# yondonfu/ai-rtc-agent

Measured on NVIDIA H100. Metric: frames/sec at 512x512 SD-Turbo img2img (1-step, stream-batch 1), higher is better.
Workload: dtype f16

## Files before the change

ai-rtc-agent_b200/csrc/capi.cu:

```cuda
#include "../../include/b200sd.h"

#include "attention.cuh"
#include "codec.cuh"
#include "elementwise.cuh"
#include "igemm.cuh"
#include "tconv.cuh"

using namespace b2;

extern "C" {

const char* b2sd_last_error(void) { return b2_last_error(); }
int b2sd_version(void) { return 1; }

static ActView to_view(const b2sd_act_view& v) {
    ActView a;
    a.ptr = reinterpret_cast<const __half*>(v.ptr);
    a.N = v.n; a.H = v.h; a.W = v.w; a.C = v.c; a.ld = v.ld;
    return a;
}

static void to_igemm_desc(const b2sd_igemm_desc* d, IgemmDesc& g) {
    g.nseg = d->nseg;
    for (int s = 0; s < d->nseg && s < IG_MAX_SRC; ++s) {
        g.src[s] = to_view(d->src[s]);
        g.ntap[s] = d->ntap[s];
    }
    g.w = reinterpret_cast<const __half*>(d->w);
    g.w_rows = d->w_rows;
    g.w_ld = d->w_ld;
    g.stride = d->stride;
    g.Nb = d->nb; g.Ho = d->ho; g.Wo = d->wo;
    g.BN = d->bn;
    g.swap = d->swap;
    g.pair = (d->flags & B2SD_IG_PAIR) ? 1 : 0;
    g.splits = d->splits;
    g.partial = nullptr;
    g.dbg_ts = reinterpret_cast<unsigned long long*>(d->partial);
    g.epi.out = reinterpret_cast<__half*>(d->out);
    g.epi.ldc = d->ldc;
    g.epi.colbias = d->colbias;
    g.epi.colbias_bstride = d->colbias_bstride;
    g.epi.res = reinterpret_cast<const __half*>(d->res);
    g.epi.ldr = d->ldr;
    g.epi.acc_scale = d->acc_scale;
    g.epi.res_scale = d->res_scale;
    g.epi.flags = d->flags & (IG_RELU | IG_GEGLU | IG_SILU | IG_PAD0);
    g.epi.n_valid = d->n_valid;
    g.epi.rowstat_out = static_cast<unsigned long long*>(d->rowstat_out);
    g.epi.rowstat_in = static_cast<const unsigned long long*>(d->rowstat_in);
    g.epi.colsum = d->colsum;
    g.epi.ln_inv_c = d->ln_c > 0 ? 1.f / (float)d->ln_c : 0.f;
    g.epi.ln_eps = d->ln_eps;
    g.epi.out2 = reinterpret_cast<__half*>(d->out2);
    g.epi.ld2 = d->ld2;
    g.epi.col2 = d->col2;
}

int b2sd_op_igemm(const b2sd_igemm_desc* d, void* stream) {
    if (!d) {
        b2_set_error("b2sd_op_igemm: null desc");
        return -1;
    }
    IgemmDesc g{};
    to_igemm_desc(d, g);
    if (d->flags & B2SD_IG_TCONV) {
        if (d->flags & B2SD_IG_PAD0) {
            b2_set_error("b2sd_op_igemm: the halo-tile kernel has no tap-origin-0 variant");
            return -1;
        }
        TconvPlan tp;
        if (tconv_plan(g, &tp)) return -1;
        return tconv_launch(tp, reinterpret_cast<cudaStream_t>(stream));
    }
    IgemmPlan plan;
    if (igemm_plan(g, &plan)) return -1;
    return igemm_launch(plan, reinterpret_cast<cudaStream_t>(stream));
}

int b2sd_igemm_plan_dry(const b2sd_igemm_desc* d, int autotile, int allow_swap, b2sd_igemm_plan_info* out) {
    if (!d || !out) {
        b2_set_error("b2sd_igemm_plan_dry: null argument");
        return -1;
    }
    IgemmDesc g{};
    to_igemm_desc(d, g);
    g.dbg_ts = nullptr;
    IgemmPlan plan;
    if (autotile == 2) {
        g.max_splits = 4; g.pair_auto = 1; g.pair_splits = 1;
    }
    igemm_set_dry_run(true);
    const int rc = autotile ? igemm_autotile(g, allow_swap != 0, &plan) : igemm_plan(g, &plan);
    igemm_set_dry_run(false);
    if (rc) return -1;
    out->mode = plan.mode;
    out->swap = plan.p.swap;
    out->bn = plan.p.BN;
    out->splits = plan.splits;
    out->grid_x = (int)plan.grid.x; out->grid_y = (int)plan.grid.y; out->grid_z = (int)plan.grid.z;
    out->num_stages = plan.p.num_stages;
    out->acc_bufs = plan.p.acc_bufs;
    out->total_kb = plan.p.total_kb;
    out->kb_per_split = plan.p.kb_per_split;
    out->tmem_cols = (int)plan.p.tmem_cols;
    out->m_tiles = plan.p.tiles_w * plan.p.tiles_h * plan.p.tiles_n;
    out->smem_bytes = (int64_t)plan.smem;
    out->rows_total = plan.rows_total;
    return 0;
}

int b2sd_groupnorm_plan_dry(int ca, int cb, int groups, int hw, int* cluster, int* threads, int* pixels_per_cta) {
    GroupNormArgs a{};
    a.ca = ca; a.cb = cb; a.lda = ca; a.ldb = cb; a.ldy = ca + cb; a.groups = groups; a.hw = hw; a.nb = 1;
    if (groups <= 0 || hw <= 0 || ca <= 0 || !cluster) {
        b2_set_error("b2sd_groupnorm_plan_dry: bad arguments");
        return -1;
    }
    *cluster = groupnorm_plan(a, threads, pixels_per_cta);
    return 0;
}

uint64_t b2sd_igemm_partial_floats(int splits, int64_t rows_total, int n_valid) {
    return igemm_partial_floats(splits, rows_total, n_valid);
}

int b2sd_op_nv12_to_rgb(const void* y, int y_pitch, const void* uv, int uv_pitch, void* rgb_nhwc, int h, int w, int flags, void* stream) {
    return nv12_to_rgb_u8_launch(static_cast<const uint8_t*>(y), y_pitch, static_cast<const uint8_t*>(uv), uv_pitch,
                                 static_cast<uint8_t*>(rgb_nhwc), h, w, flags, reinterpret_cast<cudaStream_t>(stream));
}
int b2sd_op_rgb_to_nv12(const void* rgb_nchw, void* y, int y_pitch, void* uv, int uv_pitch, int h, int w, int flags, void* stream) {
    return rgb_u8_to_nv12_launch(static_cast<const uint8_t*>(rgb_nchw), static_cast<uint8_t*>(y), y_pitch, static_cast<uint8_t*>(uv),
                                 uv_pitch, h, w, flags, reinterpret_cast<cudaStream_t>(stream));
}
int b2sd_codec_probe(void) { return codec_probe(); }

int b2sd_op_attention(const b2sd_attn_desc* d, void* stream) {
    AttnDesc a{};
    a.q = reinterpret_cast<const __half*>(d->q); a.ldq = d->ldq;
    a.k = reinterpret_cast<const __half*>(d->k); a.ldk = d->ldk; a.k_bstride = d->k_bstride; a.k_rows = d->k_rows;
    a.vt = reinterpret_cast<const __half*>(d->vt); a.ldvt = d->ldvt; a.vt_bstride = d->vt_bstride; a.vt_cols = d->vt_cols;
    a.out = reinterpret_cast<__half*>(d->out); a.ldo = d->ldo;
    a.nb = d->nb; a.heads = d->heads; a.sq = d->sq; a.skv = d->skv; a.d_real = d->d_real; a.dp = d->dp;
    AttnPlan plan;
    if (attn_plan(a, &plan)) return -1;
    return attn_launch(plan, reinterpret_cast<cudaStream_t>(stream));
}

int b2sd_op_groupnorm(const void* xa, int ca, int lda, const void* xb, int cb, int ldb, const float* gamma,
                      const float* beta, void* y, int ldy, int nb, int hw, int groups, float eps, int silu,
                      void* stream) {
    GroupNormArgs a{};
    a.xa = reinterpret_cast<const __half*>(xa); a.ca = ca; a.lda = lda;
    a.xb = reinterpret_cast<const __half*>(xb); a.cb = cb; a.ldb = ldb;
    a.gamma = gamma; a.beta = beta;
    a.y = reinterpret_cast<__half*>(y); a.ldy = ldy;
    a.nb = nb; a.hw = hw; a.groups = groups; a.eps = eps; a.silu = silu;
    static float* scratch = nullptr;
    static size_t scratch_floats = 0;
    const size_t need = groupnorm_partial_floats(nb, groups);
    if (need > scratch_floats) {
        if (scratch) cudaFree(scratch);
        if (cudaMalloc(&scratch, need * sizeof(float)) != cudaSuccess) {
            b2_set_error("b2sd_op_groupnorm: cudaMalloc failed");
            return -1;
        }
        scratch_floats = need;
    }
    a.partial = scratch;
// ... 83 lines not shown
```

ai-rtc-agent_b200/csrc/elementwise.cu:

```cuda
#include "elementwise.cuh"

#include <stdio.h>

#include "igemm.cuh"
#include "launch.cuh"
#include "ptx.cuh"

namespace b2 {

#define B2_PDL_ENTRY()            \
    do {                          \
        pdl_launch_dependents();  \
        pdl_wait();               \
    } while (0)

#define B2_LAUNCHED(name, expr)                                            \
    do {                                                                   \
        cudaError_t e__ = (expr);                                          \
        if (e__ != cudaSuccess) {                                          \
            b2_set_error("%s launch: %s", name, cudaGetErrorString(e__));  \
            return -1;                                                     \
        }                                                                  \
    } while (0)

// ... 846 lines not shown
    const long warp = ((long)blockIdx.x * blockDim.x + threadIdx.x) >> 5;
    const int lane = threadIdx.x & 31;
    if (warp >= (long)nb * n) return;
    const int b = (int)(warp / n), j = (int)(warp % n);
    float acc = 0.f;
    for (int i = lane; i < k; i += 32) {
        float v = in[(long)b * in_ld + i];
        if (silu_in) v = v / (1.0f + expf(-v));
        acc += v * __half2float(w[(long)j * k + i]);
    }
#pragma unroll
    for (int o = 16; o > 0; o >>= 1) acc += __shfl_xor_sync(0xffffffffu, acc, o);
    if (lane == 0) out[(long)b * out_ld + j] = acc + (bias ? bias[j] : 0.f);
}

int small_linear_launch(const float* in, int in_ld, const __half* w, const float* bias, float* out, int out_ld,
                        int nb, int n, int k, int silu_in, cudaStream_t s) {
    const long warps = (long)nb * n;
    small_linear_kernel<<<(unsigned)((warps * 32 + 255) / 256), 256, 0, s>>>(in, in_ld, w, bias, out, out_ld, nb, n, k, silu_in);
    B2_CHECK_LAUNCH("small_linear");
    return 0;
}

__global__ void timestep_embedding_kernel(const float* __restrict__ t, float* __restrict__ out, int nb, int dim) {
    const int half_dim = dim / 2;
    const int i = blockIdx.x * blockDim.x + threadIdx.x;
    if (i >= nb * half_dim) return;
    const int b = i / half_dim, j = i % half_dim;
    const float freq = expf(-logf(10000.0f) * (float)j / (float)half_dim);
    const float arg = t[b] * freq;
    out[(long)b * dim + j] = cosf(arg);
    out[(long)b * dim + half_dim + j] = sinf(arg);
}

int timestep_embedding_launch(const float* t, float* out, int nb, int dim, cudaStream_t s) {
    const int total = nb * (dim / 2);
    timestep_embedding_kernel<<<(total + 127) / 128, 128, 0, s>>>(t, out, nb, dim);
    B2_CHECK_LAUNCH("timestep_embedding");
    return 0;
}

__global__ void cast_f32_f16_kernel(const float* __restrict__ x, __half* __restrict__ y, long n) {
    for (long i = (long)blockIdx.x * blockDim.x + threadIdx.x; i < n; i += (long)gridDim.x * blockDim.x)
        y[i] = __float2half_rn(x[i]);
}
__global__ void cast_f16_f32_kernel(const __half* __restrict__ x, float* __restrict__ y, long n) {
    for (long i = (long)blockIdx.x * blockDim.x + threadIdx.x; i < n; i += (long)gridDim.x * blockDim.x)
        y[i] = __half2float(x[i]);
}
static unsigned grid_for(long n) {
    long b = (n + 255) / 256;
    if (b > IG_SMS * 32) b = IG_SMS * 32;
    if (b < 1) b = 1;
    return (unsigned)b;
}
int cast_f32_to_f16_launch(const float* x, __half* y, long n, cudaStream_t s) {
    cast_f32_f16_kernel<<<grid_for(n), 256, 0, s>>>(x, y, n);
    B2_CHECK_LAUNCH("cast_f32_f16");
    return 0;
}
int cast_f16_to_f32_launch(const __half* x, float* y, long n, cudaStream_t s) {
    cast_f16_f32_kernel<<<grid_for(n), 256, 0, s>>>(x, y, n);
    B2_CHECK_LAUNCH("cast_f16_f32");
    return 0;
}

__global__ void pack_conv_weight_kernel(const __half* __restrict__ w, __half* __restrict__ dst, int dst_ld, int koff,
                                        int o, int i, int taps, int c0, int cn) {
    const long total = (long)o * taps * cn;
    for (long e = (long)blockIdx.x * blockDim.x + threadIdx.x; e < total; e += (long)gridDim.x * blockDim.x) {
        const int c = (int)(e % cn);
        const int tap = (int)((e / cn) % taps);
        const int oo = (int)(e / ((long)cn * taps));
        dst[(long)oo * dst_ld + koff + tap * cn + c] = c0 + c < i ? w[((long)oo * i + (c0 + c)) * taps + tap] : __float2half(0.f);
    }
}
int pack_conv_weight_launch(const __half* w_oihw, __half* dst, int dst_ld, int koff, int o, int i, int taps, int c0,
                            int cn, cudaStream_t s) {
    pack_conv_weight_kernel<<<grid_for((long)o * taps * cn), 256, 0, s>>>(w_oihw, dst, dst_ld, koff, o, i, taps, c0, cn);
    B2_CHECK_LAUNCH("pack_conv_weight");
    return 0;
}

__global__ void gather_rows_kernel(const __half* __restrict__ src, int src_ld, const int* __restrict__ perm,
                                   __half* __restrict__ dst, int dst_ld, int rows, int cols) {
    const long total = (long)rows * cols;
    for (long e = (long)blockIdx.x * blockDim.x + threadIdx.x; e < total; e += (long)gridDim.x * blockDim.x) {
        const int c = (int)(e % cols);
        const int r = (int)(e / cols);
        const int sr = perm ? perm[r] : r;
        dst[(long)r * dst_ld + c] = sr >= 0 ? src[(long)sr * src_ld + c] : __float2half(0.f);
    }
}
int gather_rows_launch(const __half* src, int src_ld, const int* perm, __half* dst, int dst_ld, int rows, int cols,
                       cudaStream_t s) {
    gather_rows_kernel<<<grid_for((long)rows * cols), 256, 0, s>>>(src, src_ld, perm, dst, dst_ld, rows, cols);
    B2_CHECK_LAUNCH("gather_rows");
    return 0;
}

__global__ void scale_cols_kernel(__half* w, long rows, int k, const float* __restrict__ g) {
    const long r = (long)blockIdx.x * (blockDim.x >> 5) + (threadIdx.x >> 5);
    if (r >= rows) return;
    for (int c = threadIdx.x & 31; c < k; c += 32) w[r * k + c] = __float2half_rn(__half2float(w[r * k + c]) * g[c]);
}
__global__ void row_sum_kernel(const __half* __restrict__ w, long rows, int k, float* out) {
    const long r = (long)blockIdx.x * (blockDim.x >> 5) + (threadIdx.x >> 5);
    if (r >= rows) return;
    float a = 0.f;
    for (int c = threadIdx.x & 31; c < k; c += 32) a += __half2float(w[r * k + c]);
    for (int o = 16; o; o >>= 1) a += __shfl_xor_sync(0xffffffffu, a, o);
    if ((threadIdx.x & 31) == 0) out[r] = a;
}
__global__ void row_dot_kernel(const __half* __restrict__ w, long rows, int k, const float* __restrict__ v,
                               const float* __restrict__ bias, float* out) {
    const long r = (long)blockIdx.x * (blockDim.x >> 5) + (threadIdx.x >> 5);
    if (r >= rows) return;
    float a = 0.f;
    for (int c = threadIdx.x & 31; c < k; c += 32) a += __half2float(w[r * k + c]) * v[c];
    for (int o = 16; o; o >>= 1) a += __shfl_xor_sync(0xffffffffu, a, o);
    if ((threadIdx.x & 31) == 0) out[r] = a + (bias ? bias[r] : 0.f);
}
int scale_cols_launch(__half* w, long rows, int k, const float* gamma, cudaStream_t s) {
    scale_cols_kernel<<<(unsigned)((rows + 7) / 8), 256, 0, s>>>(w, rows, k, gamma);
    B2_CHECK_LAUNCH("scale_cols");
    return 0;
}
int row_sum_launch(const __half* w, long rows, int k, float* out, cudaStream_t s) {
    row_sum_kernel<<<(unsigned)((rows + 7) / 8), 256, 0, s>>>(w, rows, k, out);
    B2_CHECK_LAUNCH("row_sum");
    return 0;
}
int row_dot_launch(const __half* w, long rows, int k, const float* v, const float* bias, float* out, cudaStream_t s) {
    row_dot_kernel<<<(unsigned)((rows + 7) / 8), 256, 0, s>>>(w, rows, k, v, bias, out);
    B2_CHECK_LAUNCH("row_dot");
    return 0;
}

__global__ void maxpool2x2_kernel(const __half2* __restrict__ x, __half2* __restrict__ y, int nb, int h, int w, int c2) {
    B2_PDL_ENTRY();
    const int ho = h / 2, wo = w / 2;
    const long total = (long)nb * ho * wo * c2;
    for (long e = (long)blockIdx.x * blockDim.x + threadIdx.x; e < total; e += (long)gridDim.x * blockDim.x) {
        const int cc = (int)(e % c2);
        long p = e / c2;
        const int xo = (int)(p % wo);
        p /= wo;
        const int yo = (int)(p % ho);
        const int n = (int)(p / ho);
        const __half2* src = x + (((long)n * h + 2 * yo) * w + 2 * xo) * c2 + cc;
        const long row = (long)w * c2;
        y[e] = __hmax2(__hmax2(src[0], src[c2]), __hmax2(src[row], src[row + c2]));
    }
}

int maxpool2x2_launch(const __half* x, __half* y, int nb, int h, int w, int c, cudaStream_t s) {
    if ((c & 1) || (h & 1) || (w & 1)) {
        b2_set_error("maxpool2x2: c, h and w must be even (c=%d, %dx%d)", c, h, w);
        return -1;
    }
    const long total = (long)nb * (h / 2) * (w / 2) * (c / 2);
    long blocks = (total + 255) / 256;
    if (blocks > IG_SMS * 16) blocks = IG_SMS * 16;
    B2_LAUNCHED("maxpool2x2", launch_k(maxpool2x2_kernel, dim3((unsigned)blocks), dim3(256), 0, s, 1,
                                       reinterpret_cast<const __half2*>(x), reinterpret_cast<__half2*>(y), nb, h, w, c / 2));
    return 0;
// ... 75 lines not shown
```

ai-rtc-agent_b200/csrc/elementwise.cuh:

```cuda
#pragma once
#include <cuda_fp16.h>
#include <cuda_runtime.h>
#include <stdint.h>

namespace b2 {

struct GroupNormArgs {
    const __half* xa; int ca; int lda;
    const __half* xb; int cb; int ldb;
    const float* gamma; const float* beta;
    __half* y; int ldy;
    int nb, hw, groups;
    float eps;
    int silu;
    float* partial;
    int* counters;
};
int groupnorm_launch(const GroupNormArgs& a, cudaStream_t s);
size_t groupnorm_partial_floats(int nb, int groups);
int groupnorm_plan(const GroupNormArgs& a, int* threads, int* pixels_per_cta);
int groupnorm_last_launch_count();
enum : int { GN_PATH_CLUSTER = 0, GN_PATH_FUSED = 1, GN_PATH_STATS_APPLY = 2 };
int groupnorm_last_path();

int layernorm_launch(const __half* x, int ldx, const float* gamma, const float* beta, __half* y, int ldy,
                     long rows, int c, float eps, cudaStream_t s);

int upsample2x_launch(const __half* x, __half* y, int nb, int h, int w, int c, cudaStream_t s);

enum : int { SC_IN_U8 = 1, SC_IN_TANH3 = 2, SC_OUT_RELU = 4, SC_IN_F32_NCHW = 8, SC_IN_F16_NCHW = 16, SC_OUT_SILU = 32,
             SC_IN_OFFSET = 64 };
struct SmallConvArgs {
    const void* x;
    const float* wt;
    const float* bias;
    __half* y; int ldy;
    int nb, h, w_, cin, cout;
    int in_h, in_w;
    int flags;
    const __half* res;
    int ldr;
    long res_bstride;
    const float* in_off;
};
int smallconv_launch(const SmallConvArgs& a, cudaStream_t s);
int smallconv_prep_launch(const __half* w_oihw, float* wt, int cout, int cin, cudaStream_t s);

int maxpool2x2_launch(const __half* x, __half* y, int nb, int h, int w, int c, cudaStream_t s);
int hed_project_launch(const __half* x, int ldx, int c, long npix, const float* w, const float* bias, float* out, cudaStream_t s);
struct HedFuseArgs {
    const float* maps[5];
    int hs[5], ws[5];
    int levels;
    int h, w;
    uint8_t* out;
    __half* edge_f16;
};
int hed_fuse_launch(const HedFuseArgs& a, cudaStream_t s);

int lcm_step_launch(__half* x, const __half* eps, const __half* noise, const float* coef, __half* out_latent,
                    int T, int hw, int do_add_noise, cudaStream_t s);

int post_u8_launch(const __half* y_nhwc, int ldy, uint8_t* out_nchw, int nb, int h, int w, cudaStream_t s);
int post_f16_launch(const __half* y_nhwc, int ldy, __half* out_nchw, int nb, int h, int w, cudaStream_t s);

int small_linear_launch(const float* in, int in_ld, const __half* w, const float* bias, float* out, int out_ld,
                        int nb, int n, int k, int silu_in, cudaStream_t s);
int timestep_embedding_launch(const float* t, float* out, int nb, int dim, cudaStream_t s);

int cast_f32_to_f16_launch(const float* x, __half* y, long n, cudaStream_t s);
int cast_f16_to_f32_launch(const __half* x, float* y, long n, cudaStream_t s);
int pack_conv_weight_launch(const __half* w_oihw, __half* dst, int dst_ld, int koff, int o, int i, int taps,
                            int c0, int cn, cudaStream_t s);
int gather_rows_launch(const __half* src, int src_ld, const int* perm, __half* dst, int dst_ld, int rows, int cols,
                       cudaStream_t s);

int scale_cols_launch(__half* w, long rows, int k, const float* gamma, cudaStream_t s);
int row_sum_launch(const __half* w, long rows, int k, float* out, cudaStream_t s);
int row_dot_launch(const __half* w, long rows, int k, const float* v, const float* bias, float* out, cudaStream_t s);

}
```

ai-rtc-agent_b200/csrc/engine.cu:

```cuda
#include <cuda_fp16.h>
#include <cuda_runtime.h>
#include <math.h>
#include <stddef.h>
#include <stdio.h>
#include <stdlib.h>
#include <string.h>

#include <atomic>
#include <chrono>
#include <functional>
#include <thread>
#include <map>
#include <memory>
#include <string>
#include <vector>

#include "../../include/b200sd.h"
#include "attention.cuh"
#include "elementwise.cuh"
#include "igemm.cuh"
#include "tconv.cuh"

using namespace b2;

// ... 29 lines not shown
        for (auto s : shape) v *= s;
        return v;
    }
};

class Arena {
  public:
    explicit Arena(size_t slab) : slab_(slab) {}
    ~Arena() { release(); }
    void* alloc(size_t bytes) {
        bytes = (bytes + 1023) & ~size_t(1023);
        if (cur_ < 0 || off_ + bytes > sizes_[cur_]) {
            int next = cur_ + 1;
            while (next < (int)slabs_.size() && sizes_[next] < bytes) ++next;
            if (next >= (int)slabs_.size()) {
                size_t sz = bytes > slab_ ? bytes : slab_;
                void* p = nullptr;
                if (cudaMalloc(&p, sz) != cudaSuccess) return nullptr;
                slabs_.push_back(p);
                sizes_.push_back(sz);
                next = (int)slabs_.size() - 1;
            }
            cur_ = next;
            off_ = 0;
        }
        void* r = static_cast<char*>(slabs_[cur_]) + off_;
        off_ += bytes;
        return r;
    }
    void reset() { cur_ = slabs_.empty() ? -1 : 0; off_ = 0; }
    void release() {
        for (void* p : slabs_) cudaFree(p);
        slabs_.clear();
        sizes_.clear();
        cur_ = -1;
        off_ = 0;
    }

  private:
    size_t slab_;
    std::vector<void*> slabs_;
    std::vector<size_t> sizes_;
    int cur_ = -1;
    size_t off_ = 0;
};

struct Op {
    std::function<int(cudaStream_t)> fn;
    std::string name;
    double flops = 0.0;
    template <class F>
    Op(F f, std::string n = "", double fl = 0.0) : fn(std::move(f)), name(std::move(n)), flops(fl) {}
    int operator()(cudaStream_t s) const { return fn(s); }
};

}

static int igemm_autotile_single(IgemmDesc d, bool allow_swap, IgemmPlan* plan_out);

int igemm_autotile(IgemmDesc d, bool allow_swap, IgemmPlan* plan_out) {
    TRY(igemm_autotile_single(d, allow_swap, plan_out));
    static const char* pair_env = getenv("B2_PAIR");
    static const char* ps_env = getenv("B2_PAIR_SPLITS");
    static const bool pair_single = getenv("B2_PAIR_SINGLE") != nullptr;
    const int pair_mode = pair_env ? atoi(pair_env) : d.pair_auto;
    const int pair_splits = ps_env ? atoi(ps_env) : (d.pair_splits > 0 ? d.pair_splits : 4);
    const IgemmPlan& pl = *plan_out;
    const int m_tiles = pl.p.tiles_w * pl.p.tiles_h * pl.p.tiles_n;
    if (pair_mode <= 0 || pl.p.swap || m_tiles < 2 || (pl.p.BN % 32) != 0 || (d.epi.flags & (IG_SILU | IG_PAD0))) return 0;
    if (pair_mode == 2 && pl.p.total_kb < 20) return 0;
    d.swap = 0; d.BN = pl.p.BN; d.splits = pl.splits > pair_splits ? pair_splits : pl.splits; d.partial = nullptr;
    d.pair = pair_single ? 0 : 1;
    IgemmPlan paired;
    if (igemm_plan(d, &paired)) return 0;
    *plan_out = paired;
    return 0;
}

static int igemm_autotile_single(IgemmDesc d, bool allow_swap, IgemmPlan* plan_out) {
    IgemmPlan& plan = *plan_out;
    const bool geglu = (d.epi.flags & IG_GEGLU) != 0;
    const bool silu = (d.epi.flags & IG_SILU) != 0;
    const bool pad0 = (d.epi.flags & IG_PAD0) != 0;
    const int n_gemm = geglu ? 2 * d.epi.n_valid : d.epi.n_valid;
    static const bool swap_on = getenv("B2_SWAP") != nullptr, swap_off = getenv("B2_NO_SWAP") != nullptr;
    static const bool tuned = getenv("B2_NO_TUNED_TILES") == nullptr;
    static const char* ms_env = getenv("B2_MAX_SPLITS");
    const int max_splits = ms_env ? atoi(ms_env) : (d.max_splits > 0 ? d.max_splits : 8);
    int total_kb = 0;
    for (int sidx = 0; sidx < d.nseg && sidx < IG_MAX_SRC; ++sidx) total_kb += d.ntap[sidx] * (d.src[sidx].C / IG_BK);
    const long rows_all = (long)d.Nb * d.Ho * d.Wo;
    const bool swap_here = allow_swap && !geglu && !pad0 && d.epi.n_valid >= 128 && (d.epi.n_valid & 7) == 0 &&
                           (swap_on || (!swap_off && tuned && rows_all <= 64 && total_kb >= 90));
    if (swap_here) {
        d.swap = 1;
        d.BN = rows_all >= 256 ? 256 : (rows_all >= 128 ? 128 : 64);
        d.splits = 1; d.partial = nullptr;
        TRY(igemm_plan(d, &plan));
        const long ctas = (long)plan.grid.x * plan.grid.y;
        int max_by_k = plan.p.total_kb / 4;
        if (max_by_k < 1) max_by_k = 1;
        if (max_by_k > 8) max_by_k = 8;
        int splits = 1;
        while (splits * 2 <= max_by_k && ctas * splits * 2 <= 192 && splits * 2 <= max_splits) splits *= 2;
        if (splits > 1) {
            d.splits = splits;
            TRY(igemm_plan(d, &plan));
        }
        return 0;
    }
    d.swap = 0;
    auto vt_ok = [&](int bn) { return !d.epi.out2 || d.epi.col2 % bn == 0; };
    if (tuned && !geglu && !silu && !pad0 && n_gemm % 160 == 0 && total_kb >= 40 && vt_ok(160)) {
        d.BN = 160; d.splits = 1; d.partial = nullptr;
        TRY(igemm_plan(d, &plan));
        const int m_tiles = plan.p.tiles_w * plan.p.tiles_h * plan.p.tiles_n;
        const long tiles = (long)m_tiles * (n_gemm / 160);
        int bn = 0, splits = 0;
        if (tiles < 132) {
            if (m_tiles >= 8) { bn = 160; splits = 4; }
            else if (m_tiles >= 2 && n_gemm % 256 == 0 && total_kb >= 180 && vt_ok(256)) { bn = 256; splits = 8; }
        }
        if (bn && splits > max_splits) bn = 0;
        if (bn) {
            d.BN = bn; d.splits = splits;
            TRY(igemm_plan(d, &plan));
            return 0;
        }
    }
    static const int cands[] = {256, 160, 128, 64, 32, 16};
    std::vector<int> valid;
    for (int bn : cands) {
        if (geglu && (bn % 32 != 0 || bn < 64)) continue;
        if (silu && (bn > 128 || bn % 16 || (bn & (bn - 1)))) continue;
        if (pad0 && bn != 64 && bn != 128 && bn != 256) continue;
        if (n_gemm % bn == 0 && vt_ok(bn)) valid.push_back(bn);
    }
    if (valid.empty()) {
        int bn = 16;
        while (bn < n_gemm && bn < 128) bn <<= 1;
        valid.push_back(bn);
    }
    for (int bn : valid) {
        if (bn < 64 && n_gemm >= 64) break;
        d.BN = bn; d.splits = 1; d.partial = nullptr;
        TRY(igemm_plan(d, &plan));
        if (plan.p.acc_bufs == 2 || (long)plan.grid.x * plan.grid.y >= b2_device_sms()) return 0;
    }
    int bn = valid.back();
    for (int v : valid) if (v >= 64) bn = v;
    d.BN = bn; d.splits = 1; d.partial = nullptr;
    TRY(igemm_plan(d, &plan));
    const long ctas = (long)plan.grid.x * plan.grid.y;
    int splits = ctas >= 96 ? 1 : (int)((IG_SMS + ctas - 1) / ctas);
    if (tuned && ctas >= 64 && total_kb <= 12) splits = 1;
    const int max_by_k = plan.p.total_kb / 4 > 0 ? plan.p.total_kb / 4 : 1;
    if (splits > max_by_k) splits = max_by_k;
    if (splits > 8) splits = 8;
    while (splits > max_splits && splits > 1) splits >>= 1;
    if (geglu) splits = 1;
    if (splits > 1) {
        d.splits = splits;
        TRY(igemm_plan(d, &plan));
    }
    return 0;
}

struct WeightStore {
    std::map<std::string, Raw> raw;
    Arena weights{256u << 20};
    Arena raw_only{256u << 20};
    bool raw_released = false;
    bool imported = false;
    std::map<std::string, __half*> packed;
    std::map<std::string, float*> fvec;
    std::map<std::string, size_t> packed_bytes, fvec_bytes;
};

struct b2sd_engine {
    b2sd_config cfg{};
    int lh = 0, lw = 0;
    std::shared_ptr<WeightStore> ws;
    std::map<std::string, Raw>& raw;
    Arena& weights;
    Arena& raw_only;
    bool& raw_released;
    bool& imported;
    std::map<std::string, __half*>& packed;
    std::map<std::string, float*>& fvec;
    std::map<std::string, size_t>& packed_bytes;
    std::map<std::string, size_t>& fvec_bytes;
    Arena state{16u << 20};
    Arena prog{512u << 20};
    explicit b2sd_engine(std::shared_ptr<WeightStore> s)
        : ws(std::move(s)), raw(ws->raw), weights(ws->weights), raw_only(ws->raw_only), raw_released(ws->raw_released),
          imported(ws->imported), packed(ws->packed), fvec(ws->fvec), packed_bytes(ws->packed_bytes), fvec_bytes(ws->fvec_bytes) {}

    Act x_in;
    __half* noise = nullptr;
    float* coef = nullptr;
    float* tsteps = nullptr;
    __half* ctx = nullptr;
    float* temb_sin = nullptr;
    float* temb_h = nullptr;
    float* temb = nullptr;
    float* cn_temb_h = nullptr;
    float* cn_temb = nullptr;
    float* gn_ws = nullptr;
    int* tile_counters = nullptr;
    float coef_host[4][64]{};

    unsigned long long* ln_stats = nullptr;
    size_t ln_stats_cap = 0, ln_stats_used = 0;
    std::vector<Op> prog_frame, prog_prompt, prog_time;
    std::map<std::string, Act> taps;
    SmallConvArgs head{};
    SmallConvArgs cn_head{};
    SmallConvArgs hed_head{};
    Act image;
// ... 17 lines not shown
            if (stage_graph[i]) { cudaGraphDestroy(stage_graph[i]); stage_graph[i] = nullptr; }
        }
    }

    ~b2sd_engine() { drop_graphs(); }

    const Raw* get(const std::string& key) {
        auto it = raw.find(key);
        if (it == raw.end()) {
            b2_set_error("missing weight '%s'", key.c_str());
            return nullptr;
        }
        return &it->second;
    }
    bool has(const std::string& key) const { return raw.count(key) != 0; }

    float* vec(const std::vector<std::string>& keys, const std::vector<int>* perm = nullptr, int pad_to = 0) {
        std::string ck = "v:";
        for (auto& k : keys) ck += k + "+";
        if (perm) ck += "perm";
        auto it = fvec.find(ck);
        if (it != fvec.end()) return it->second;
        std::vector<float> host;
        for (auto& k : keys) {
            const Raw* r = get(k);
            if (!r) return nullptr;
            if (host.empty()) host.assign(r->host.begin(), r->host.end());
            else
                for (size_t i = 0; i < host.size() && i < r->host.size(); ++i) host[i] += r->host[i];
        }
        if (perm) {
            std::vector<float> t(perm->size());
            for (size_t i = 0; i < perm->size(); ++i) t[i] = (*perm)[i] >= 0 ? host[(*perm)[i]] : 0.f;
            host.swap(t);
        }
        if ((int)host.size() < pad_to) host.resize(pad_to, 0.f);
        float* d = static_cast<float*>(weights.alloc(host.size() * sizeof(float)));
        if (!d) return nullptr;
        if (cudaMemcpy(d, host.data(), host.size() * sizeof(float), cudaMemcpyHostToDevice) != cudaSuccess) return nullptr;
        fvec[ck] = d;
        fvec_bytes[ck] = host.size() * sizeof(float);
        return d;
    }

    const float* small_w(const std::string& key, cudaStream_t s) {
        auto it = fvec.find("sw:" + key);
        if (it != fvec.end()) return it->second;
        const Raw* r = get(key);
        if (!r) return nullptr;
        if (!r->p) { b2_set_error("parameter '%s' was released after the first prepare and is not in the packed cache", key.c_str()); return nullptr; }
        const int cout = (int)r->shape[0], cin = (int)r->shape[1];
        float* d = static_cast<float*>(weights.alloc((size_t)cin * 9 * cout * sizeof(float)));
        if (!d || smallconv_prep_launch(r->p, d, cout, cin, s)) return nullptr;
        fvec["sw:" + key] = d;
        fvec_bytes["sw:" + key] = (size_t)cin * 9 * cout * sizeof(float);
        return d;
    }

    struct ConvSeg { std::string key; int c0, cn, taps; };
    __half* pack_conv(const std::string& name, const std::vector<ConvSeg>& segs, int rows, int* k_out,
                      cudaStream_t s) {
        int K = 0;
        for (auto& g : segs) K += g.taps * g.cn;
        *k_out = K;
        auto it = packed.find(name);
        if (it != packed.end()) return it->second;
        const int rows_pad = (rows + 15) / 16 * 16;
        __half* dst = static_cast<__half*>(weights.alloc((size_t)rows_pad * K * 2));
        if (!dst) return nullptr;
        cudaMemsetAsync(dst, 0, (size_t)rows_pad * K * 2, s);
        int koff = 0;
        for (auto& g : segs) {
            const Raw* r = get(g.key);
            if (!r) return nullptr;
            if (!r->p) { b2_set_error("parameter '%s' was released after the first prepare and is not in the packed cache", g.key.c_str()); return nullptr; }
            const int cin_total = (int)r->shape[1];
            if (pack_conv_weight_launch(r->p, dst, K, koff, rows, cin_total, g.taps, g.c0, g.cn, s)) return nullptr;
            koff += g.taps * g.cn;
        }
        packed[name] = dst;
        packed_bytes[name] = (size_t)rows_pad * K * 2;
        return dst;
    }
    __half* pack_rows(const std::string& name, const std::vector<std::pair<std::string, std::vector<int>>>& parts,
                      int K, cudaStream_t s) {
        auto it = packed.find(name);
        if (it != packed.end()) return it->second;
        size_t rows = 0;
        for (auto& p : parts) rows += p.second.size();
        const size_t rows_pad = (rows + 15) / 16 * 16;
        __half* dst = static_cast<__half*>(weights.alloc(rows_pad * K * 2));
        if (!dst) return nullptr;
        cudaMemsetAsync(dst, 0, rows_pad * K * 2, s);
        size_t r0 = 0;
        for (auto& p : parts) {
            const Raw* r = get(p.first);
            if (!r) return nullptr;
            if (!r->p) { b2_set_error("parameter '%s' was released after the first prepare and is not in the packed cache", p.first.c_str()); return nullptr; }
            int* dperm = static_cast<int*>(weights.alloc(p.second.size() * sizeof(int)));
            if (!dperm) return nullptr;
            cudaMemcpyAsync(dperm, p.second.data(), p.second.size() * sizeof(int), cudaMemcpyHostToDevice, s);
            cudaStreamSynchronize(s);
            if (gather_rows_launch(r->p, K, dperm, dst + r0 * K, K, (int)p.second.size(), K, s)) return nullptr;
            r0 += p.second.size();
        }
        packed[name] = dst;
        packed_bytes[name] = rows_pad * K * 2;
        return dst;
    }

    struct LnFold { __half* w = nullptr; const float* colsum = nullptr; const float* bias = nullptr; };
    int fold_ln(const std::string& name, const std::vector<std::pair<std::string, std::vector<int>>>& parts, int K,
                const std::string& ln_prefix, const float* bias_vec, LnFold* out, cudaStream_t s) {
        size_t rows = 0;
        for (auto& p : parts) rows += p.second.size();
        const size_t rows_pad = (rows + 15) / 16 * 16;
        const bool done = packed.count(name) && fvec.count(name + ":cs") && fvec.count(name + ":b");
        __half* w = pack_rows(name, parts, K, s);
        if (!w) return -1;
        if (!done) {
            const float* gamma = vec({ln_prefix + ".weight"});
            const float* beta = vec({ln_prefix + ".bias"});
            float* cs = static_cast<float*>(weights.alloc(rows_pad * sizeof(float)));
            float* bb = static_cast<float*>(weights.alloc(rows_pad * sizeof(float)));
            if (!gamma || !beta || !cs || !bb) return -1;
            cudaMemsetAsync(bb, 0, rows_pad * sizeof(float), s);
            TRY(row_dot_launch(w, (long)rows, K, beta, bias_vec, bb, s));
            TRY(scale_cols_launch(w, (long)rows_pad, K, gamma, s));
            TRY(row_sum_launch(w, (long)rows_pad, K, cs, s));
            fvec[name + ":cs"] = cs; fvec_bytes[name + ":cs"] = rows_pad * sizeof(float);
            fvec[name + ":b"] = bb; fvec_bytes[name + ":b"] = rows_pad * sizeof(float);
        }
        out->w = w;
        out->colsum = fvec[name + ":cs"];
        out->bias = fvec[name + ":b"];
        return 0;
    }
    unsigned long long* alloc_rowstat(long rows) {
        if (ln_stats_used + 2 * (size_t)rows > ln_stats_cap) {
            b2_set_error("LayerNorm statistics slab exhausted");
            return nullptr;
        }
        unsigned long long* p = ln_stats + ln_stats_used;
        ln_stats_used += 2 * (size_t)rows;
        return p;
    }

    Act new_act(int n, int h, int w, int c, int ld = 0) {
        Act a;
        a.n = n; a.h = h; a.w = w; a.c = c; a.ld = ld ? ld : c;
        a.p = static_cast<__half*>(prog.alloc((size_t)a.elems() * 2));
        return a;
    }
    static ActView view(const Act& a) { return ActView{a.p, a.n, a.h, a.w, a.c, a.ld}; }
    static ActView tokens(const Act& a) { return ActView{a.p, 1, 1, a.n * a.h * a.w, a.c, a.ld}; }

    void push_igemm(std::vector<Op>& dst, const IgemmPlan& plan, const std::string& label, double flops) {
        if (&dst == &prog_frame) launches += 1;
        dst.push_back(Op([plan](cudaStream_t s) { return igemm_launch(plan, s); }, label, flops));
    }

    int add_igemm(std::vector<Op>& dst, IgemmDesc d) {
        const bool geglu = (d.epi.flags & IG_GEGLU) != 0;
        const int n_gemm = geglu ? 2 * d.epi.n_valid : d.epi.n_valid;
        const bool extras = d.epi.rowstat_out || d.epi.colsum || d.epi.out2;
        if (concurrency > 1 && d.max_splits == 0) d.max_splits = 4;
        if (concurrency >= 4 && d.pair_auto == 0) { d.pair_auto = 1; d.pair_splits = 1; }
        IgemmPlan plan;
        TRY(igemm_autotile(d, allow_swap && !extras, &plan));
        if (d.epi.out2 && d.epi.col2 % plan.p.BN != 0) {
            b2_set_error("fused q/k/v projection: N tile %d does not divide the V offset %d", plan.p.BN, d.epi.col2);
            return -1;
        }
        char label[256];
        snprintf(label, sizeof(label), "igemm %s rows=%ld n=%d kb=%d bn=%d splits=%d grid=%u,%u,%u %s", cur.c_str(),
                 plan.rows_total, d.epi.n_valid, plan.p.total_kb, plan.p.BN, plan.splits, plan.grid.x, plan.grid.y,
                 plan.grid.z, plan.p.swap ? "swapped" : (plan.pair ? "pairs" : "taps"));
        push_igemm(dst, plan, label, 2.0 * (double)plan.rows_total * n_gemm * plan.p.total_kb * IG_BK);
        return 0;
    }

    int add_groupnorm(const Act& xa, const Act* xb, const std::string& prefix, const Act& y, float eps, int silu) {
        GroupNormArgs a{};
        a.xa = xa.p; a.ca = xa.c; a.lda = xa.ld;
        if (xb) { a.xb = xb->p; a.cb = xb->c; a.ldb = xb->ld; }
        a.gamma = vec({prefix + ".weight"});
        a.beta = vec({prefix + ".bias"});
        if (!a.gamma || !a.beta) return -1;
        a.y = y.p; a.ldy = y.ld;
        a.nb = xa.n; a.hw = xa.h * xa.w; a.groups = cfg.norm_groups; a.eps = eps; a.silu = silu;
        a.partial = gn_ws;
        a.counters = tile_counters;
        launches += 1;
        prog_frame.push_back(Op([a](cudaStream_t s) { return groupnorm_launch(a, s); }, "groupnorm " + prefix));
        return 0;
    }

    int add_layernorm(const Act& x, const std::string& prefix, const Act& y) {
        const float* g = vec({prefix + ".weight"});
        const float* b = vec({prefix + ".bias"});
        if (!g || !b) return -1;
        const long rows = (long)x.n * x.h * x.w;
        const __half* xp = x.p; __half* yp = y.p;
        const int ldx = x.ld, ldy = y.ld, c = x.c;
        ++launches;
        prog_frame.push_back(Op([=](cudaStream_t s) { return layernorm_launch(xp, ldx, g, b, yp, ldy, rows, c, 1e-5f, s); }, "layernorm " + prefix));
        return 0;
    }

    int add_conv(std::vector<Op>& dst, const Act& x, const std::string& wkey, const std::string& bkey, int taps,
                 int stride, const Act& y, int flags, const Act* res, cudaStream_t s, float acc_scale = 1.f,
                 float res_scale = 1.f) {
        const Raw* w = get(wkey);
        if (!w) return -1;
        cur = wkey;
        const int cout = (int)w->shape[0];
        int K = 0;
        __half* wp = pack_conv(wkey, {{wkey, 0, x.c, taps}}, cout, &K, s);
        if (!wp) return -1;
        IgemmDesc d{};
        d.nseg = 1; d.src[0] = view(x); d.ntap[0] = taps;
        d.w = wp; d.w_rows = (cout + 15) / 16 * 16; d.w_ld = K;
        d.stride = stride;
        d.Nb = y.n; d.Ho = y.h; d.Wo = y.w;
        d.epi.out = y.p; d.epi.ldc = y.ld;
        if (!bkey.empty()) {
            d.epi.colbias = vec({bkey}, nullptr, 16);
            if (!d.epi.colbias) return -1;
        }
        d.epi.colbias_bstride = 0;
        if (res) { d.epi.res = res->p; d.epi.ldr = res->ld; }
        d.epi.acc_scale = acc_scale; d.epi.res_scale = res_scale;
        d.epi.flags = flags;
        d.epi.n_valid = cout;
        static const bool no_tconv = getenv("B2_NO_TCONV") != nullptr;
        static const char* tc_min = getenv("B2_TCONV_MIN_TILES");
        const long tiles = (long)y.n * ((y.h + TC_TH - 1) / TC_TH) * ((y.w + TC_TW - 1) / TC_TW);
        if (!no_tconv && stride == 1 && tconv_eligible(d) && tiles >= (tc_min ? atoi(tc_min) : 2 * IG_SMS)) {
            TconvPlan tp;
            TRY(tconv_plan(d, &tp));
            char label[256];
            snprintf(label, sizeof(label), "tconv %s rows=%ld tiles=%d grid=%u nbuf=%d", wkey.c_str(), tp.rows_total, tp.p.num_tiles,
                     tp.grid.x, tp.p.nbuf);
            if (&dst == &prog_frame) launches += 1;
            dst.push_back(Op([tp](cudaStream_t st) { return tconv_launch(tp, st); }, label, 2.0 * (double)tp.rows_total * cout * K));
            return 0;
        }
        return add_igemm(dst, d);
    }

    struct LinExtra {
        unsigned long long* rowstat_out = nullptr;
        const unsigned long long* rowstat_in = nullptr;
        const float* colsum = nullptr;
        int ln_c = 0;
        __half* out2 = nullptr;
        int ld2 = 0, col2 = 0;
    };
    int add_linear(std::vector<Op>& dst, const ActView& x, const __half* w, int n, int k, const float* bias,
                   __half* out, int ldc, const __half* res, int ldr, int flags = 0, int n_valid = -1,
                   const LinExtra* ex = nullptr) {
        IgemmDesc d{};
        if (ex) {
            d.epi.rowstat_out = ex->rowstat_out;
            d.epi.rowstat_in = ex->rowstat_in;
            d.epi.colsum = ex->colsum;
            d.epi.ln_inv_c = ex->ln_c ? 1.f / (float)ex->ln_c : 0.f;
            d.epi.ln_eps = 1e-5f;
            d.epi.out2 = ex->out2; d.epi.ld2 = ex->ld2; d.epi.col2 = ex->col2;
        }
        d.nseg = 1; d.src[0] = x; d.ntap[0] = 1;
        d.w = w; d.w_rows = n; d.w_ld = k;
        d.stride = 1;
        d.Nb = 1; d.Ho = 1; d.Wo = x.W;
        d.epi.out = out; d.epi.ldc = ldc;
        d.epi.colbias = bias; d.epi.colbias_bstride = 0;
        d.epi.res = res; d.epi.ldr = ldr;
        d.epi.acc_scale = 1.f; d.epi.res_scale = 1.f;
        d.epi.flags = flags;
        d.epi.n_valid = n_valid >= 0 ? n_valid : n;
        return add_igemm(dst, d);
    }

    int build_resnet(const std::string& p, const Act& xa, const Act* xb, int cout, const float* emb, Act* out, cudaStream_t s,
                     float eps = 1e-5f);
    int build_vae_attention(const std::string& p, const Act& x, Act* out, cudaStream_t s);
    int build_kl_encoder(Act* out, std::string* latent_conv, cudaStream_t s);
    int build_kl_decoder(const Act& x0, cudaStream_t s);
    std::vector<float> host_copy(const std::string& key);
    int derive(const std::string& name, const std::vector<int64_t>& shape, const std::vector<float>& v);
    const float* const_vec(const std::string& name, const std::vector<float>& v);
    int build_cond_embedding(Act* out, cudaStream_t s);
    int build_hed(const uint8_t** control, cudaStream_t s);
    int build_controlnet(const Act& cond, std::vector<Act>& skips, Act* mid, cudaStream_t s);
    int build_transformer(const std::string& p, const Act& x, int heads, Act* out, cudaStream_t s);
    int build_taesd_block(const std::string& p, const Act& x, Act* out, cudaStream_t s);
    int build_program(cudaStream_t s);
    int run_range(std::vector<Op>& ops, size_t a, size_t b, cudaStream_t s) {
        for (size_t i = a; i < b && i < ops.size(); ++i) TRY(ops[i](s));
        return 0;
    }
    int run(std::vector<Op>& ops, cudaStream_t s) {
        static const bool dbg = getenv("B200SD_DEBUG_SYNC") != nullptr;
        static const char* skip = getenv("B200SD_SKIP");
        static const char* skip_name = getenv("B200SD_SKIP_NAME");
        int idx = 0;
        for (auto& op : ops) {
            if (skip) {
                const std::string kind = op.name.substr(0, op.name.find(' '));
                if (!kind.empty() && std::string(skip).find(kind) != std::string::npos) { ++idx; continue; }
            }
            if (skip_name && op.name.find(skip_name) != std::string::npos) { ++idx; continue; }
            TRY(op(s));
            if (dbg) {
                cudaError_t e = cudaStreamSynchronize(s);
                if (e != cudaSuccess) {
                    b2_set_error("op %d '%s' failed: %s", idx, op.name.c_str(), cudaGetErrorString(e));
                    fprintf(stderr, "b2sd: op %d '%s' failed: %s\n", idx, op.name.c_str(), cudaGetErrorString(e));
                    return -1;
                }
            }
            ++idx;
        }
        return 0;
    }
};

int b2sd_engine::build_resnet(const std::string& p, const Act& xa, const Act* xb, int cout, const float* emb, Act* out,
                              cudaStream_t s, float eps) {
    cur = p;
    allow_swap = true;
// ... 596 lines not shown
            }
            bf[o] = (float)bo;
        }
        TRY(derive(*latent_conv + ".weight", {4, ci, 3, 3}, wf));
        TRY(derive(*latent_conv + ".bias", {4}, bf));
    }
    return 0;
}

int b2sd_engine::build_kl_decoder(const Act& x0, cudaStream_t s) {
    const std::string P = "vae.decoder.";
    allow_swap = false;
    cur = P + "conv_in";
    const float sf = cfg.vae_scaling_factor > 0.f ? cfg.vae_scaling_factor : 0.18215f;
    const std::string wkey = P + "conv_in+post_quant_conv.weight";
    if (!has(wkey)) {
        const Raw* wc = get(P + "conv_in.weight");
        const Raw* wq = get("vae.post_quant_conv.weight");
        if (!wc || !wq) return -1;
        const int co = (int)wc->shape[0];
        if (wc->shape[1] != 4 || wq->numel() != 16) {
            b2_set_error("vae: decoder conv_in takes %ld channels and post_quant_conv has %ld weights (4 and 4x4 expected)",
                         (long)wc->shape[1], wq->numel());
            return -1;
        }
        std::vector<float> w = host_copy(P + "conv_in.weight"), q = host_copy("vae.post_quant_conv.weight");
        if (w.empty() || q.empty()) return -1;
        std::vector<float> wf((size_t)co * 4 * 9, 0.f);
        for (int o = 0; o < co; ++o)
            for (int j = 0; j < 4; ++j)
                for (int t = 0; t < 9; ++t) {
                    double acc = 0.0;
                    for (int i = 0; i < 4; ++i) acc += (double)w[((size_t)o * 4 + i) * 9 + t] * q[i * 4 + j];
                    wf[((size_t)o * 4 + j) * 9 + t] = (float)(acc / sf);
                }
        TRY(derive(wkey, {co, 4, 3, 3}, wf));
    }
    const Raw* rw = get(wkey);
    const Raw* pqb = get("vae.post_quant_conv.bias");
    if (!rw || !pqb || pqb->host.size() != 4) {
        if (rw && pqb) b2_set_error("vae: post_quant_conv.bias must have 4 elements");
        return -1;
    }
    const int cm = (int)rw->shape[0];
    Act bmap = new_act(1, lh, lw, cm), cst = new_act(1, lh, lw, 4), h = new_act(1, lh, lw, cm);
    if (!bmap.p || !cst.p || !h.p) return -1;
    {
        std::vector<__half> c((size_t)lh * lw * 4);
        for (size_t i = 0; i < c.size(); ++i) c[i] = __float2half_rn(pqb->host[i % 4]);
        CUDA_OK(cudaMemcpyAsync(cst.p, c.data(), c.size() * 2, cudaMemcpyHostToDevice, s));
        SmallConvArgs m{};
        m.x = cst.p; m.wt = small_w(P + "conv_in.weight", s); m.bias = vec({P + "conv_in.bias"});
        if (!m.wt || !m.bias) return -1;
        m.y = bmap.p; m.ldy = cm; m.nb = 1; m.h = lh; m.w_ = lw; m.cin = 4; m.cout = cm; m.in_h = lh; m.in_w = lw;
        TRY(smallconv_launch(m, s));
        CUDA_OK(cudaStreamSynchronize(s));
    }
    {
        SmallConvArgs a{};
        a.x = x0.p; a.wt = small_w(wkey, s); a.bias = nullptr;
        if (!a.wt) return -1;
        a.y = h.p; a.ldy = h.ld; a.nb = 1; a.h = lh; a.w_ = lw; a.cin = 4; a.cout = cm; a.in_h = lh; a.in_w = lw;
        a.res = bmap.p; a.ldr = bmap.ld; a.res_bstride = 0;
        ++launches;
        prog_frame.push_back(Op([a](cudaStream_t st) { return smallconv_launch(a, st); }, "smallconv vae.decoder.conv_in"));
    }
    {
        Act o;
        TRY(build_resnet(P + "mid_block.resnets.0.", h, nullptr, h.c, nullptr, &o, s, 1e-6f)); h = o;
        TRY(build_vae_attention(P + "mid_block.attentions.0.", h, &o, s)); h = o;
        TRY(build_resnet(P + "mid_block.resnets.1.", h, nullptr, h.c, nullptr, &o, s, 1e-6f)); h = o;
        taps["vae.dec.mid"] = h;
    }
    for (int i = 0; i < 4; ++i) {
        const std::string bp = P + "up_blocks." + std::to_string(i);
        for (int j = 0; j < 3; ++j) {
            const Raw* w1 = get(bp + ".resnets." + std::to_string(j) + ".conv1.weight");
            if (!w1) return -1;
            Act o;
            TRY(build_resnet(bp + ".resnets." + std::to_string(j) + ".", h, nullptr, (int)w1->shape[0], nullptr, &o, s, 1e-6f));
            h = o;
        }
        if (i < 3) {
            Act up = new_act(1, h.h * 2, h.w * 2, h.c);
            const Act hin = h;
            ++launches;
            prog_frame.push_back(Op([hin, up](cudaStream_t st) { return upsample2x_launch(hin.p, up.p, hin.n, hin.h, hin.w, hin.c, st); }, "upsample2x"));
            Act o = new_act(1, up.h, up.w, h.c);
            TRY(add_conv(prog_frame, up, bp + ".upsamplers.0.conv.weight", bp + ".upsamplers.0.conv.bias", 9, 1, o, 0, nullptr, s));
            h = o;
        }
        taps["vae.dec.up." + std::to_string(i)] = h;
    }
    Act nout = new_act(1, h.h, h.w, h.c);
    TRY(add_groupnorm(h, nullptr, P + "conv_norm_out", nout, 1e-6f, 1));
    const std::string bkey = P + "conv_out.bias+1";
    if (!has(bkey)) {
        const Raw* b = get(P + "conv_out.bias");
        if (!b) return -1;
        std::vector<float> v(b->host);
        for (auto& x : v) x += 1.f;
        TRY(derive(bkey, b->shape, v));
    }
    image = new_act(1, cfg.height, cfg.width, 3, 8);
    return add_conv(prog_frame, nout, P + "conv_out.weight", bkey, 9, 1, image, 0, nullptr, s, 0.5f);
}

int b2sd_engine::build_program(cudaStream_t s) {
    prog.reset();
    prog_frame.clear(); prog_prompt.clear(); prog_time.clear();
    taps.clear();
    launches = 0;
    drop_graphs();
    const int B = cfg.batch, H = cfg.height, W = cfg.width;
    const int* ch = cfg.block_out_channels;
    const int nlev = 4;
    {
        long words = 0;
        for (int i = 0; i < nlev; ++i) {
            const long tokens_i = (long)B * (lh >> i) * (lw >> i);
            int blocks_i = (cfg.down_attn[i] ? cfg.layers_per_block + (cfg.layers_per_block + 1) : 0) + (i == nlev - 1 ? 1 : 0);
            if (cfg.controlnet) blocks_i += (cfg.down_attn[i] ? cfg.layers_per_block : 0) + (i == nlev - 1 ? 1 : 0);
            words += 3 * 2 * tokens_i * blocks_i;
        }
        ln_stats_cap = (size_t)words;
        ln_stats_used = 0;
        ln_stats = static_cast<unsigned long long*>(prog.alloc(ln_stats_cap * sizeof(unsigned long long)));
        if (!ln_stats) return -1;
    }

    allow_swap = false;
    const bool kl = cfg.vae == B2SD_VAE_KL;
    Act e;
    std::string latent_conv;
    int li = 1;
    if (kl) {
        TRY(build_kl_encoder(&e, &latent_conv, s));
    } else {
    e = new_act(1, H, W, 64);
    {
        head = SmallConvArgs{};
        head.wt = small_w("vae.encoder.layers.0.weight", s);
        if (!head.wt) return -1;
        head.bias = vec({"vae.encoder.layers.0.bias"});
        head.y = e.p; head.ldy = e.ld; head.nb = 1; head.h = H; head.w_ = W; head.cin = 3; head.cout = 64;
        head.flags = SC_IN_U8;
        if (!head.bias) return -1;
        ++launches;
    }
    const int enc_blocks[4] = {1, 3, 3, 3};
    for (int st = 0; st < 4; ++st) {
        if (st > 0) {
            Act dwn = new_act(1, e.h / 2, e.w / 2, 64);
            TRY(add_conv(prog_frame, e, "vae.encoder.layers." + std::to_string(li) + ".weight", "", 9, 2, dwn, 0, nullptr, s));
            e = dwn;
            ++li;
        }
        for (int k = 0; k < enc_blocks[st]; ++k) {
            Act o;
            TRY(build_taesd_block("vae.encoder.layers." + std::to_string(li), e, &o, s));
            e = o;
            ++li;
        }
    }
    latent_conv = "vae.encoder.layers." + std::to_string(li);
    }
    Act cond;
    if (cfg.controlnet) TRY(build_cond_embedding(&cond, s));
    {
        Act xt;
        xt.p = x_in.p; xt.n = 1; xt.h = lh; xt.w = lw; xt.c = 4; xt.ld = 4;
        Act nz = xt;
        nz.p = noise;
        const float zscale = kl ? (cfg.vae_scaling_factor > 0.f ? cfg.vae_scaling_factor : 0.18215f) : 1.f;
        idx_enc_end = prog_frame.size();
        TRY(add_conv(prog_frame, e, latent_conv + ".weight", latent_conv + ".bias", 9, 1, xt, 0, &nz, s, coef_host[0][0] * zscale,
                     coef_host[1][0]));
        taps["x_t"] = xt;
    }
    taps["unet_in"] = x_in;

    allow_swap = true;
    Act h = new_act(B, lh, lw, ch[0]);
    {
        SmallConvArgs a{};
        a.wt = small_w("conv_in.weight", s);
        if (!a.wt) return -1;
        a.x = x_in.p; a.bias = vec({"conv_in.bias"});
        a.y = h.p; a.ldy = h.ld; a.nb = B; a.h = lh; a.w_ = lw; a.cin = 4; a.cout = ch[0]; a.in_h = lh; a.in_w = lw;
        if (!a.bias) return -1;
        ++launches;
        prog_frame.push_back(Op([a](cudaStream_t st) { return smallconv_launch(a, st); }, "smallconv"));
    }
    taps["conv_in"] = h;
    std::vector<Act> skips{h};
    for (int i = 0; i < nlev; ++i) {
        for (int j = 0; j < cfg.layers_per_block; ++j) {
            Act o;
            const std::string bp = "down_blocks." + std::to_string(i);
            TRY(build_resnet(bp + ".resnets." + std::to_string(j) + ".", h, nullptr, ch[i], temb, &o, s));
            h = o;
            if (cfg.down_attn[i]) {
                TRY(build_transformer(bp + ".attentions." + std::to_string(j) + ".", h, cfg.heads[i], &o, s));
                h = o;
            }
            skips.push_back(h);
            taps["down." + std::to_string(i) + "." + std::to_string(j)] = h;
        }
        if (i != nlev - 1) {
            Act o = new_act(B, h.h / 2, h.w / 2, ch[i]);
            const std::string k = "down_blocks." + std::to_string(i) + ".downsamplers.0.conv.";
            TRY(add_conv(prog_frame, h, k + "weight", k + "bias", 9, 2, o, 0, nullptr, s));
            h = o;
            skips.push_back(h);
        }
    }
    {
        Act o;
        TRY(build_resnet("mid_block.resnets.0.", h, nullptr, ch[nlev - 1], temb, &o, s)); h = o;
        TRY(build_transformer("mid_block.attentions.0.", h, cfg.heads[nlev - 1], &o, s)); h = o;
        TRY(build_resnet("mid_block.resnets.1.", h, nullptr, ch[nlev - 1], temb, &o, s)); h = o;
        taps["mid"] = h;
    }
    if (cfg.controlnet) TRY(build_controlnet(cond, skips, &h, s));
    for (int i = 0; i < nlev; ++i) {
        const int co = ch[nlev - 1 - i];
        const int hd = cfg.heads[nlev - 1 - i];
        const bool attn = cfg.down_attn[nlev - 1 - i] != 0;
        for (int j = 0; j < cfg.layers_per_block + 1; ++j) {
            Act sk = skips.back();
            skips.pop_back();
            Act o;
            const std::string bp = "up_blocks." + std::to_string(i);
            TRY(build_resnet(bp + ".resnets." + std::to_string(j) + ".", h, &sk, co, temb, &o, s));
            h = o;
            if (attn) {
                TRY(build_transformer(bp + ".attentions." + std::to_string(j) + ".", h, hd, &o, s));
                h = o;
            }
            taps["up." + std::to_string(i) + "." + std::to_string(j)] = h;
        }
        if (i != nlev - 1) {
            Act up = new_act(B, h.h * 2, h.w * 2, co);
            const Act hin = h;
            ++launches;
            prog_frame.push_back(Op([hin, up](cudaStream_t st) { return upsample2x_launch(hin.p, up.p, hin.n, hin.h, hin.w, hin.c, st); }, "upsample2x"));
            Act o = new_act(B, up.h, up.w, co);
            const std::string k = "up_blocks." + std::to_string(i) + ".upsamplers.0.conv.";
            TRY(add_conv(prog_frame, up, k + "weight", k + "bias", 9, 1, o, 0, nullptr, s));
            h = o;
        }
    }
    Act nout = new_act(B, lh, lw, ch[0]);
    TRY(add_groupnorm(h, nullptr, "conv_norm_out", nout, 1e-5f, 1));
    Act eps = new_act(B, lh, lw, 4);
    TRY(add_conv(prog_frame, nout, "conv_out.weight", "conv_out.bias", 9, 1, eps, 0, nullptr, s));
    taps["eps"] = eps;
    Act x0 = new_act(1, lh, lw, 4);
    {
        __half* xp = x_in.p; const __half* ep = eps.p; const __half* np_ = noise; const float* cf = coef; __half* op = x0.p;
        const int T = B, hw = lh * lw, dan = cfg.do_add_noise;
        ++launches;
        prog_frame.push_back(Op([=](cudaStream_t st) { return lcm_step_launch(xp, ep, np_, cf, op, T, hw, dan, st); }, "lcm_step"));
        idx_unet_end = prog_frame.size();
    }
    taps["x0"] = x0;
    allow_swap = false;
    if (kl) {
        TRY(build_kl_decoder(x0, s));
    } else {
    Act dcur = new_act(1, lh, lw, 64);
    {
        SmallConvArgs a{};
        a.wt = small_w("vae.decoder.layers.0.weight", s);
        if (!a.wt) return -1;
        a.x = x0.p; a.bias = vec({"vae.decoder.layers.0.bias"});
        a.y = dcur.p; a.ldy = dcur.ld; a.nb = 1; a.h = lh; a.w_ = lw; a.cin = 4; a.cout = 64; a.in_h = lh; a.in_w = lw;
        a.flags = SC_IN_TANH3 | SC_OUT_RELU;
        if (!a.bias) return -1;
        ++launches;
        prog_frame.push_back(Op([a](cudaStream_t st) { return smallconv_launch(a, st); }, "smallconv"));
    }
    li = 2;
    const int dec_blocks[4] = {3, 3, 3, 1};
    for (int st = 0; st < 4; ++st) {
        for (int k = 0; k < dec_blocks[st]; ++k) {
            Act o;
            TRY(build_taesd_block("vae.decoder.layers." + std::to_string(li), dcur, &o, s));
            dcur = o;
            ++li;
        }
        if (st != 3) {
            Act up = new_act(1, dcur.h * 2, dcur.w * 2, 64);
            const Act hin = dcur;
            ++launches;
            prog_frame.push_back(Op([hin, up](cudaStream_t s2) { return upsample2x_launch(hin.p, up.p, hin.n, hin.h, hin.w, hin.c, s2); }, "upsample2x"));
            ++li;
            Act o = new_act(1, up.h, up.w, 64);
            TRY(add_conv(prog_frame, up, "vae.decoder.layers." + std::to_string(li) + ".weight", "", 9, 1, o, 0, nullptr, s));
            dcur = o;
            ++li;
        } else {
            image = new_act(1, H, W, 3, 8);
            const std::string k = "vae.decoder.layers." + std::to_string(li);
            TRY(add_conv(prog_frame, dcur, k + ".weight", k + ".bias", 9, 1, image, 0, nullptr, s));
        }
    }
    }
    taps["image"] = image;
    ++launches;
    if (ln_stats_used) {
        unsigned long long* sp = ln_stats;
        const size_t bytes = ln_stats_used * sizeof(unsigned long long);
        prog_frame.insert(prog_frame.begin() + idx_enc_end, Op([sp, bytes](cudaStream_t st) {
            if (cudaMemsetAsync(sp, 0, bytes, st) != cudaSuccess) { b2_set_error("memset of the LayerNorm statistics failed"); return -1; }
            return 0; }, "memset ln_stats"));
        idx_unet_end += 1;
    }
    CUDA_OK(cudaStreamSynchronize(s));
    built = true;
    return 0;
}

extern "C" {

static int create_engine(const b2sd_config* cfg, std::shared_ptr<WeightStore> store, b2sd_handle* out);

int b2sd_create(const b2sd_config* cfg, b2sd_handle* out) { return create_engine(cfg, std::make_shared<WeightStore>(), out); }

int b2sd_create_lane(b2sd_handle parent, const b2sd_config* cfg, b2sd_handle* out) {
    if (!parent) {
        b2_set_error("b2sd_create_lane: null parent");
        return -1;
    }
    b2sd_config c = cfg ? *cfg : parent->cfg;
    c.controlnet = parent->cfg.controlnet;
    c.control_processor = parent->cfg.control_processor;
    c.vae = parent->cfg.vae;
    c.vae_scaling_factor = parent->cfg.vae_scaling_factor;
    for (int i = 0; i < 4; ++i)
        if (c.block_out_channels[i] != parent->cfg.block_out_channels[i] || c.heads[i] != parent->cfg.heads[i] ||
            c.down_attn[i] != parent->cfg.down_attn[i]) {
            b2_set_error("b2sd_create_lane: the lane's architecture differs from its parent's");
            return -1;
        }
    if (create_engine(&c, parent->ws, out)) return -1;
    (*out)->concurrency = parent->concurrency > 1 ? parent->concurrency : 2;
    return 0;
}

static int create_engine(const b2sd_config* cfg, std::shared_ptr<WeightStore> store, b2sd_handle* out) {
    if (!cfg || !out) {
        b2_set_error("b2sd_create: null argument");
        return -1;
    }
    if (cfg->height % 64 || cfg->width % 64 || cfg->batch < 1 || cfg->batch > 16) {
        b2_set_error("b2sd_create: height/width must be multiples of 64, 1 <= batch <= 16 (got %dx%d, %d)",
                     cfg->height, cfg->width, cfg->batch);
        return -1;
    }
    for (int i = 0; i < 4; ++i) {
        if (cfg->block_out_channels[i] % 64 || cfg->heads[i] < 1 || cfg->block_out_channels[i] % cfg->heads[i]) {
            b2_set_error("b2sd_create: block_out_channels must be multiples of 64 and divisible by heads");
            return -1;
        }
    }
    if (cfg->cross_attention_dim % 64) {
        b2_set_error("b2sd_create: cross_attention_dim must be a multiple of 64");
        return -1;
    }
    if (cfg->controlnet != 0 && cfg->controlnet != 1) {
        b2_set_error("b2sd_create: controlnet must be 0 or 1 (got %d)", cfg->controlnet);
        return -1;
    }
    if (cfg->control_processor != B2SD_CONTROL_FRAME && (cfg->control_processor != B2SD_CONTROL_HED || !cfg->controlnet)) {
        b2_set_error("b2sd_create: control_processor must be 0 (the frame) or 1 (HED, with a ControlNet) (got %d)", cfg->control_processor);
        return -1;
    }
    if (cfg->vae != B2SD_VAE_TINY && cfg->vae != B2SD_VAE_KL) {
        b2_set_error("b2sd_create: vae must be 0 (TAESD) or 1 (AutoencoderKL) (got %d)", cfg->vae);
        return -1;
    }
// ... 125 lines not shown
        const Raw* w2 = h->get(p + "time_embedding.linear_2.weight");
        const float* b1 = h->vec({p + "time_embedding.linear_1.bias"});
        const float* b2v = h->vec({p + "time_embedding.linear_2.bias"});
        if (!w1 || !w2 || !b1 || !b2v) return -1;
        TRY(small_linear_launch(h->temb_sin, C0, w1->p, b1, hid, TD, B, TD, C0, 0, s));
        return small_linear_launch(hid, TD, w2->p, b2v, out, TD, B, TD, TD, 1, s);
    };
    TRY(embed("", h->temb_h, h->temb));
    if (h->cfg.controlnet) TRY(embed("controlnet.", h->cn_temb_h, h->cn_temb));
    return h->run(h->prog_time, s);
}

int b2sd_prepare(b2sd_handle h, const void* prompt_embeds, const float* timesteps, const float* coef,
                 const void* init_noise, void* stream) {
    if (!h || !prompt_embeds || !timesteps || !coef || !init_noise) {
        b2_set_error("b2sd_prepare: null argument");
        return -1;
    }
    cudaStream_t s = reinterpret_cast<cudaStream_t>(stream);
    const int B = h->cfg.batch, lh = h->lh, lw = h->lw;
    for (int k = 0; k < 4; ++k)
        for (int i = 0; i < B; ++i) h->coef_host[k][i] = coef[k * B + i];
    CUDA_OK(cudaMemcpyAsync(h->coef, coef, 4 * B * sizeof(float), cudaMemcpyHostToDevice, s));
    CUDA_OK(cudaMemcpyAsync(h->tsteps, timesteps, B * sizeof(float), cudaMemcpyHostToDevice, s));
    CUDA_OK(cudaMemcpyAsync(h->ctx, prompt_embeds, (size_t)h->cfg.ctx_tokens * h->cfg.cross_attention_dim * 2,
                            cudaMemcpyHostToDevice, s));
    {
        const __half* src = static_cast<const __half*>(init_noise);
        std::vector<__half> nhwc((size_t)B * lh * lw * 4);
        for (int b = 0; b < B; ++b)
            for (int c = 0; c < 4; ++c)
                for (int y = 0; y < lh; ++y)
                    for (int x = 0; x < lw; ++x)
                        nhwc[(((size_t)b * lh + y) * lw + x) * 4 + c] = src[(((size_t)b * 4 + c) * lh + y) * lw + x];
        CUDA_OK(cudaMemcpyAsync(h->noise, nhwc.data(), nhwc.size() * 2, cudaMemcpyHostToDevice, s));
        CUDA_OK(cudaStreamSynchronize(s));
    }
    CUDA_OK(cudaMemsetAsync(h->x_in.p, 0, (size_t)h->x_in.elems() * 2, s));
    TRY(h->build_program(s));
    TRY(h->run(h->prog_prompt, s));
    TRY(refresh_time(h, s));
    CUDA_OK(cudaStreamSynchronize(s));
    static const bool keep_raw = getenv("B2_KEEP_RAW") != nullptr;
    if (!keep_raw && !h->raw_released) {
        for (auto& kv : h->raw)
            if (kv.second.pack_only) kv.second.p = nullptr;
        h->raw_only.release();
        h->raw_released = true;
    }
    return 0;
}

extern "C++" {
namespace {
struct BlobWriter {
    FILE* f;
    bool ok = true;
    void put(const void* p, size_t n) { if (ok && n && fwrite(p, 1, n, f) != n) ok = false; }
    template <class T> void pod(const T& v) { put(&v, sizeof(T)); }
    void str(const std::string& v) { pod((uint32_t)v.size()); put(v.data(), v.size()); }
};
struct BlobReader {
    FILE* f;
    bool ok = true;
    void get(void* p, size_t n) { if (ok && n && fread(p, 1, n, f) != n) ok = false; }
    template <class T> T pod() { T v{}; get(&v, sizeof(T)); return v; }
    std::string str() { uint32_t n = pod<uint32_t>(); if (!ok || n > 4096) { ok = false; return ""; } std::string v(n, 0); get(&v[0], n); return v; }
};
}
}

int b2sd_export_packed(b2sd_handle h, const char* path) {
    if (!h || !h->built || !path) {
        b2_set_error("b2sd_export_packed: call b2sd_prepare first");
        return -1;
    }
    FILE* f = fopen(path, "wb");
    if (!f) {
        b2_set_error("b2sd_export_packed: cannot open %s", path);
        return -1;
    }
    BlobWriter w{f};
    w.put("B2SDPACK", 8);
    w.pod((uint32_t)3);
    b2sd_config cfg = h->cfg;
    cfg.batch = 0; cfg.height = 0; cfg.width = 0; cfg.use_cuda_graph = 0; cfg.do_add_noise = 0;
    w.pod(cfg);
    w.pod((uint32_t)(h->raw.size() + h->packed_bytes.size() + h->fvec_bytes.size()));
    std::vector<char> host;
    auto payload = [&](const void* dptr, size_t bytes) {
        w.pod((uint64_t)bytes);
        if (!bytes) return true;
        host.resize(bytes);
        if (cudaMemcpy(host.data(), dptr, bytes, cudaMemcpyDeviceToHost) != cudaSuccess) return false;
        w.put(host.data(), bytes);
        return true;
    };
    bool copy_ok = true;
    for (auto& kv : h->raw) {
        const Raw& r = kv.second;
        w.pod((uint8_t)0); w.str(kv.first);
        w.pod((uint32_t)r.shape.size());
        for (auto d : r.shape) w.pod((int64_t)d);
        copy_ok &= payload(r.p, (r.pack_only || !r.p) ? 0 : (size_t)r.numel() * 2);
    }
    for (auto& kv : h->packed_bytes) {
        w.pod((uint8_t)1); w.str(kv.first); w.pod((uint32_t)0);
        copy_ok &= payload(h->packed[kv.first], kv.second);
    }
    for (auto& kv : h->fvec_bytes) {
        w.pod((uint8_t)2); w.str(kv.first); w.pod((uint32_t)0);
        copy_ok &= payload(h->fvec[kv.first], kv.second);
    }
    const bool ok = w.ok && copy_ok && fclose(f) == 0;
    if (!ok) {
        b2_set_error("b2sd_export_packed: write to %s failed", path);
        remove(path);
        return -1;
    }
    return 0;
}

int b2sd_import_packed(b2sd_handle h, const char* path) {
    if (!h || !path) {
        b2_set_error("b2sd_import_packed: null argument");
        return -1;
    }
    if (!h->raw.empty()) {
        b2_set_error("b2sd_import_packed: the engine already holds parameters");
        return -1;
    }
    FILE* f = fopen(path, "rb");
    if (!f) {
        b2_set_error("b2sd_import_packed: cannot open %s", path);
        return -1;
    }
    BlobReader rd{f};
    char magic[8];
    rd.get(magic, 8);
    const uint32_t version = rd.pod<uint32_t>();
    b2sd_config cfg{};
    if (version == 1) rd.get(&cfg, offsetof(b2sd_config, controlnet));
    else if (version == 2) rd.get(&cfg, offsetof(b2sd_config, vae));
    else cfg = rd.pod<b2sd_config>();
    bool same = rd.ok && memcmp(magic, "B2SDPACK", 8) == 0 && version >= 1 && version <= 3 && cfg.cross_attention_dim == h->cfg.cross_attention_dim &&
                cfg.layers_per_block == h->cfg.layers_per_block && cfg.norm_groups == h->cfg.norm_groups && cfg.ctx_tokens == h->cfg.ctx_tokens &&
                cfg.controlnet == h->cfg.controlnet && cfg.control_processor == h->cfg.control_processor && cfg.vae == h->cfg.vae &&
                (cfg.vae != B2SD_VAE_KL || cfg.vae_scaling_factor == h->cfg.vae_scaling_factor);
    for (int i = 0; i < 4 && same; ++i)
        same = cfg.block_out_channels[i] == h->cfg.block_out_channels[i] && cfg.heads[i] == h->cfg.heads[i] && cfg.down_attn[i] == h->cfg.down_attn[i];
    if (!same) {
        fclose(f);
        b2_set_error("b2sd_import_packed: %s is not a packed-weight blob of this architecture", path);
        return -1;
    }
    const uint32_t count = rd.pod<uint32_t>();
    std::vector<char> host;
    for (uint32_t i = 0; i < count && rd.ok; ++i) {
        const uint8_t kind = rd.pod<uint8_t>();
        const std::string name = rd.str();
        const uint32_t ndim = rd.pod<uint32_t>();
        Raw r;
        for (uint32_t d = 0; d < ndim && d < 8; ++d) r.shape.push_back(rd.pod<int64_t>());
        const uint64_t bytes = rd.pod<uint64_t>();
        if (!rd.ok || bytes > ((uint64_t)1 << 32)) { rd.ok = false; break; }
        void* dptr = nullptr;
        if (bytes) {
            host.resize(bytes);
            rd.get(host.data(), bytes);
            dptr = h->weights.alloc(bytes);
            if (!rd.ok || !dptr || cudaMemcpy(dptr, host.data(), bytes, cudaMemcpyHostToDevice) != cudaSuccess) { rd.ok = false; break; }
        }
        if (kind == 0) {
            r.p = static_cast<__half*>(dptr);
            r.pack_only = bytes == 0;
            if (ndim == 1 && bytes) {
                const __half* hp = reinterpret_cast<const __half*>(host.data());
                r.host.resize(bytes / 2);
                for (size_t k = 0; k < r.host.size(); ++k) r.host[k] = __half2float(hp[k]);
            }
            h->raw[name] = std::move(r);
        } else if (kind == 1) {
            h->packed[name] = static_cast<__half*>(dptr);
            h->packed_bytes[name] = bytes;
        } else if (kind == 2) {
            h->fvec[name] = static_cast<float*>(dptr);
            h->fvec_bytes[name] = bytes;
        } else {
            rd.ok = false;
        }
    }
    fclose(f);
    if (!rd.ok) {
        b2_set_error("b2sd_import_packed: %s is truncated or corrupt", path);
        return -1;
    }
    h->raw_released = true;
    h->imported = true;
    h->built = false;
    return 0;
}

int b2sd_set_prompt_embeds(b2sd_handle h, const void* prompt_embeds, void* stream) {
    if (!h || !h->built) {
        b2_set_error("b2sd_set_prompt_embeds: call b2sd_prepare first");
        return -1;
    }
    cudaStream_t s = reinterpret_cast<cudaStream_t>(stream);
    CUDA_OK(cudaMemcpyAsync(h->ctx, prompt_embeds, (size_t)h->cfg.ctx_tokens * h->cfg.cross_attention_dim * 2,
                            cudaMemcpyHostToDevice, s));
    CUDA_OK(cudaStreamSynchronize(s));
    return h->run(h->prog_prompt, s);
}

int b2sd_set_timesteps(b2sd_handle h, const float* timesteps, void* stream) {
    if (!h || !h->built) {
        b2_set_error("b2sd_set_timesteps: call b2sd_prepare first");
        return -1;
    }
    cudaStream_t s = reinterpret_cast<cudaStream_t>(stream);
    CUDA_OK(cudaMemcpyAsync(h->tsteps, timesteps, h->cfg.batch * sizeof(float), cudaMemcpyHostToDevice, s));
    CUDA_OK(cudaStreamSynchronize(s));
    return refresh_time(h, s);
}

int b2sd_step(b2sd_handle h, const void* frame_in, int in_h, int in_w, void* frame_out, void* stream) {
    return b2sd_step_ex(h, frame_in, B2SD_IN_U8_NHWC, in_h, in_w, frame_out, B2SD_OUT_U8_NCHW, stream);
}
// ... 252 lines not shown
```

ai-rtc-agent_b200/csrc/igemm.cu:

```cuda
#include "igemm.cuh"

#include <cudaTypedefs.h>
#include <stdarg.h>
#include <stdio.h>
#include <stdlib.h>
#include <string.h>

#include "epilogue.cuh"
#include "launch.cuh"
#include "ptx.cuh"

namespace b2 {

#ifdef B2_TIMELINE
#define B2_TS(stmt) stmt
#else
#define B2_TS(stmt)
#endif

static thread_local char g_err[1024] = "";
const char* b2_last_error() { return g_err; }
void b2_set_error(const char* fmt, ...) {
    va_list ap;
    va_start(ap, fmt);
// ... 25 lines not shown
        if (item >= npix * 16) continue;
        const int pl = item >> 4, q = item & 15;
        const int j = j0 + pl;
        const int wi = j & (tw - 1);
        const int hi = (j >> p.tw_log2) & (th - 1);
        const int ni = j >> (p.tw_log2 + p.th_log2);
        const int n = n0 + ni, h = h0 + hi, w = w0 + wi;
        const int cout0 = ntile * IG_BM + q * 8;
        if (ni >= p.tn || n >= p.Nb || h >= p.Ho || w >= p.Wo || cout0 >= e.n_valid) continue;
        const long orow = ((long)n * p.Ho + h) * p.Wo + w;
        pre.orow[k] = orow;
        if (e.colbias) {
            const float4* bp = reinterpret_cast<const float4*>(e.colbias + (long)n * e.colbias_bstride + cout0);
            pre.b0[k] = __ldg(bp);
            pre.b1[k] = __ldg(bp + 1);
        }
        if (e.res) pre.res[k] = __ldg(reinterpret_cast<const uint4*>(e.res + orow * e.ldr + cout0));
    }
}

template <bool SILU>
__device__ __forceinline__ void swap_store_chunk(const IgemmParams& p, const SwapPre& pre, const float* T, int ntile, int t) {
    const IgEpilogue& e = p.epi;
#pragma unroll
    for (int k = 0; k < SWAP_ITEMS; ++k) {
        if (pre.orow[k] < 0) continue;
        const int item = t + IG_CONS * k;
        const int pl = item >> 4, q = item & 15;
        const int cout0 = ntile * IG_BM + q * 8;
        const float4 a0 = *reinterpret_cast<const float4*>(T + pl * IG_BM + q * 8);
        const float4 a1 = *reinterpret_cast<const float4*>(T + pl * IG_BM + q * 8 + 4);
        const float4 b0 = pre.b0[k], b1 = pre.b1[k];
        float v[8] = {a0.x + b0.x, a0.y + b0.y, a0.z + b0.z, a0.w + b0.w, a1.x + b1.x, a1.y + b1.y, a1.z + b1.z, a1.w + b1.w};
#pragma unroll
        for (int i = 0; i < 8; ++i) v[i] *= e.acc_scale;
        if (e.res) {
            const __half2* rh = reinterpret_cast<const __half2*>(&pre.res[k]);
#pragma unroll
            for (int i = 0; i < 4; ++i) {
                const float2 f = __half22float2(rh[i]);
                v[2 * i] += e.res_scale * f.x;
                v[2 * i + 1] += e.res_scale * f.y;
            }
        }
        if (e.flags & IG_RELU) {
#pragma unroll
            for (int i = 0; i < 8; ++i) v[i] = fmaxf(v[i], 0.f);
        }
        if (SILU && (e.flags & IG_SILU)) {
#pragma unroll
            for (int i = 0; i < 8; ++i) v[i] = silu_f(v[i]);
        }
        uint4 o;
        __half2* oh = reinterpret_cast<__half2*>(&o);
#pragma unroll
        for (int i = 0; i < 4; ++i) oh[i] = __floats2half2_rn(v[2 * i], v[2 * i + 1]);
        *reinterpret_cast<uint4*>(e.out + pre.orow[k] * e.ldc + cout0) = o;
    }
}

template <int SPL>
__device__ __forceinline__ void splitk_sum16(uint32_t stg_local, int cc, int row, float (&acc)[16], int rank_mul = 1, int rank_add = 0) {
#pragma unroll
    for (int i = 0; i < 16; ++i) acc[i] = 0.f;
    constexpr int G = SPL < 4 ? SPL : 4;
#pragma unroll
    for (int s0 = 0; s0 < SPL; s0 += G) {
        float4 v[G][4];
#pragma unroll
        for (int s = 0; s < G; ++s) {
            const uint32_t peer = dsmem_map(stg_local, (uint32_t)((s0 + s) * rank_mul + rank_add));
#pragma unroll
            for (int i = 0; i < 4; ++i) v[s][i] = dsmem_ld_f4(peer + (uint32_t)(((cc * 4 + i) * IG_BM + row) * 16));
        }
#pragma unroll
        for (int s = 0; s < G; ++s)
#pragma unroll
            for (int i = 0; i < 4; ++i) {
                acc[4 * i] += v[s][i].x; acc[4 * i + 1] += v[s][i].y; acc[4 * i + 2] += v[s][i].z; acc[4 * i + 3] += v[s][i].w;
            }
    }
}

template <int BN, bool PAIR, bool SILU, bool PAD0 = false>
__device__ __forceinline__ void igemm_body(const IgemmParams& p) {
    extern __shared__ uint8_t smem_raw[];
    uint8_t* smem = reinterpret_cast<uint8_t*>((reinterpret_cast<uintptr_t>(smem_raw) + 1023) &
                                               ~static_cast<uintptr_t>(1023));
    const int warp = threadIdx.x >> 5;
    const int lane = threadIdx.x & 31;
    constexpr uint32_t A_BYTES = IG_BM * IG_BK * 2;
    constexpr uint32_t stage_bytes = A_BYTES + (uint32_t)BN * IG_BK * 2;
    uint64_t* full_bar = reinterpret_cast<uint64_t*>(smem + (size_t)p.num_stages * stage_bytes);
    uint64_t* empty_bar = full_bar + IG_MAX_STAGES;
    const int cr = PAIR ? (int)(blockIdx.x & 1) : 0;
    const int mt_first = (int)blockIdx.x;
    const int mt_step = (int)gridDim.x;
    const int mt_guard = PAIR ? cr : 0;

    const int num_mtiles = p.tiles_w * p.tiles_h * p.tiles_n;
    const int ntile = blockIdx.y;
    const int kb_begin = blockIdx.z * p.kb_per_split;
    const int kb_end = min(p.total_kb, kb_begin + p.kb_per_split);
    [[maybe_unused]] unsigned long long* ts = p.dbg_ts ? p.dbg_ts + ((size_t)(blockIdx.z * gridDim.y + blockIdx.y) * gridDim.x + blockIdx.x) * 8 : nullptr;
    B2_TS(if (ts && threadIdx.x == 0) ts[0] = globaltimer_ns();)

    if (threadIdx.x == IG_CONS) {
        for (int s = 0; s < p.nseg; ++s) tma_prefetch_desc(&p.tmA[s]);
        tma_prefetch_desc(&p.tmB);
        for (int s = 0; s < p.num_stages; ++s) {
            mbar_init(&full_bar[s], 1);
            mbar_init(&empty_bar[s], (PAIR ? 2 : 1) * (IG_CONS / 32));
        }
        fence_mbar_init();
    }
    if (PAIR) {
        cluster_arrive_relaxed();
        cluster_wait();
    }
    __syncthreads();

    pdl_launch_dependents();
    pdl_wait();
    B2_TS(if (ts && threadIdx.x == 0) ts[1] = globaltimer_ns();)

    if (warp == IG_CONS / 32) {
        if (lane == 0) {
            [[maybe_unused]] const uint16_t pair_mask = PAIR ? (uint16_t)(3u << (cluster_ctarank() & ~1u)) : (uint16_t)0;
            int stage = 0;
            uint32_t phase = 0;
            for (int mt = mt_first; mt - mt_guard < num_mtiles; mt += mt_step) {
                const int w0 = (mt % p.tiles_w) * p.tw, h0 = ((mt / p.tiles_w) % p.tiles_h) * p.th;
                const int n0 = (mt / (p.tiles_w * p.tiles_h)) * p.tn;
                int seg = 0, base = 0;
                while (seg < p.nseg - 1 && kb_begin >= base + p.seg_ntap[seg] * p.seg_cblocks[seg]) {
                    base += p.seg_ntap[seg] * p.seg_cblocks[seg];
                    ++seg;
                }
                int tap = (kb_begin - base) / p.seg_cblocks[seg];
                int cb = (kb_begin - base) % p.seg_cblocks[seg];
                for (int kb = kb_begin; kb < kb_end; ++kb) {
                    mbar_wait(&empty_bar[stage], phase ^ 1);
#ifdef B2_BOUND_STUDY
                    if (p.dbg_mode == 1 && kb >= kb_begin + p.num_stages) {
                        mbar_arrive(&full_bar[stage]);
                        if (++stage == p.num_stages) { stage = 0; phase ^= 1; }
                        continue;
                    }
#endif
                    mbar_expect_tx(&full_bar[stage], p.a_bytes + p.b_bytes);
                    uint8_t* sa = smem + (size_t)stage * stage_bytes;
                    uint8_t* sb = sa + A_BYTES;
                    int dy = 0, dx = 0;
                    if (p.seg_ntap[seg] == 9) {
                        dy = tap / 3 - (PAD0 ? 0 : 1);
                        dx = tap % 3 - (PAD0 ? 0 : 1);
                    }
                    tma_load_4d(p.swap ? sb : sa, &p.tmA[seg], &full_bar[stage], p.seg_c0[seg] + cb * IG_BK,
                                w0 * p.stride + dx, h0 * p.stride + dy, n0);
                    if (PAIR)
                        tma_load_2d_mc(sb + cr * (BN / 2) * 128, &p.tmB, &full_bar[stage], kb * IG_BK, ntile * BN + cr * (BN / 2), pair_mask);
                    else
                        tma_load_2d(p.swap ? sa : sb, &p.tmB, &full_bar[stage], kb * IG_BK, ntile * (p.swap ? IG_BM : BN));
                    B2_TS(if (ts && mt == (int)blockIdx.x && kb == kb_begin) ts[2] = globaltimer_ns();)
                    if (++cb == p.seg_cblocks[seg]) {
                        cb = 0;
                        if (++tap == p.seg_ntap[seg]) {
                            tap = 0;
                            ++seg;
                        }
                    }
                    if (++stage == p.num_stages) {
                        stage = 0;
                        phase ^= 1;
                    }
                }
            }
        }
    } else {
        const int wg = warp >> 2;
        const int r0 = wg * 64 + (warp & 3) * 16 + (lane >> 2);
        [[maybe_unused]] const uint32_t peer_empty = PAIR ? dsmem_map(smem_u32(empty_bar), cluster_ctarank() ^ 1u) : 0u;
        const IgEpilogue& e = p.epi;
        const bool ln_fma = e.colsum && !p.swap && !(e.flags & IG_SPLITK) && (e.ldc & 7) == 0 && (e.n_valid & 15) == 0;
        const uint32_t smem_base = smem_u32(smem);
        auto release = [&](int s) {
            if (lane == 0) {
                mbar_arrive(&empty_bar[s]);
                if (PAIR) mbar_arrive_remote(peer_empty + (uint32_t)s * 8u);
            }
        };
        int stage = 0;
        uint32_t phase = 0;
        int it = 0;
        for (int mt = mt_first; mt - mt_guard < num_mtiles; mt += mt_step, ++it) {
            float acc[BN / 2];
#pragma unroll
            for (int i = 0; i < BN / 2; ++i) acc[i] = 0.f;
            int prev = -1;
            for (int kb = kb_begin; kb < kb_end; ++kb) {
                mbar_wait(&full_bar[stage], phase);
                B2_TS(if (ts && it == 0 && kb == kb_begin && threadIdx.x == 0) ts[3] = globaltimer_ns();)
                const uint32_t sa = smem_base + (uint32_t)stage * stage_bytes;
                const uint64_t da = make_kmajor_sw128_desc(sa + (uint32_t)wg * (64 * 128));
                const uint64_t db = make_kmajor_sw128_desc(sa + A_BYTES);
#ifdef B2_BOUND_STUDY
                if (p.dbg_mode != 2)
#endif
                {
                    wgmma_fence_regs(acc);
                    wgmma_fence();
#pragma unroll
                    for (int k = 0; k < 4; ++k) Wgmma<BN>::ss(acc, da + 2 * k, db + 2 * k, 1u);
                    wgmma_commit();
                    wgmma_wait<1>();
                    wgmma_fence_regs(acc);
                }
                if (prev >= 0) release(prev);
                prev = stage;
                if (++stage == p.num_stages) {
                    stage = 0;
                    phase ^= 1;
                }
            }
            wgmma_wait<0>();
            wgmma_fence_regs(acc);
            if (prev >= 0) release(prev);
            B2_TS(if (ts && it == 0 && threadIdx.x == 0) ts[4] = globaltimer_ns();)

            const int w0 = (mt % p.tiles_w) * p.tw, h0 = ((mt / p.tiles_w) % p.tiles_h) * p.th;
            const int n0 = (mt / (p.tiles_w * p.tiles_h)) * p.tn;
            if (p.swap || (e.flags & IG_SPLITK)) {
                float* stg = reinterpret_cast<float*>(smem);
                cons_bar_sync();
                if (e.flags & IG_SPLITK) {
                    frag_to_smem<BN>(stg, acc, r0, lane, 0, BN, false);
                } else {
                    for (int c = 0; c < BN; c += SWAP_CH) {
                        SwapPre pre;
                        swap_prefetch(p, pre, SWAP_CH, c, ntile, n0, h0, w0, threadIdx.x);
                        frag_to_smem<BN>(stg, acc, r0, lane, c, SWAP_CH, true);
                        cons_bar_sync();
                        swap_store_chunk<SILU>(p, pre, stg, ntile, threadIdx.x);
                        cons_bar_sync();
                    }
                }
            } else {
                EpiRow rw[2];
#pragma unroll
                for (int h = 0; h < 2; ++h) {
                    const int r = r0 + 8 * h;
                    const int wi = r % p.tw, hi = (r / p.tw) % p.th, ni = r / (p.tw * p.th);
                    const int n = n0 + ni, hh = h0 + hi, ww = w0 + wi;
                    rw[h].ok = (ni < p.tn) && (n < p.Nb) && (hh < p.Ho) && (ww < p.Wo);
                    rw[h].orow = ((long)n * p.Ho + hh) * p.Wo + ww;
                    rw[h].b = n;
                    ln_row_stats(e, rw[h].orow, rw[h].ok, rw[h].mu, rw[h].rstd);
                }
                epi_frag<BN, SILU>(e, acc, rw, ntile, ln_fma, lane);
            }
            B2_TS(if (ts && it == 0 && threadIdx.x == 0) ts[5] = globaltimer_ns();)
        }
    }
    if (p.epi.flags & IG_SPLITK) {
        const int mt = blockIdx.x;
        const int w0 = (mt % p.tiles_w) * p.tw, h0 = ((mt / p.tiles_w) % p.tiles_h) * p.th;
        const int n0 = (mt / (p.tiles_w * p.tiles_h)) * p.tn;
        const int splits = (int)gridDim.z;
        const int rk_mul = PAIR ? 2 : 1, rk_add = cr;
        cluster_sync_all();
        B2_TS(if (ts && threadIdx.x == 0) ts[6] = globaltimer_ns();)
        if (warp < IG_CONS / 32 && p.swap) {
            const int rank = (int)cluster_ctarank();
            const int cols_per = BN / splits;
            const int ch = cols_per < SWAP_CH ? cols_per : SWAP_CH;
            const int t = threadIdx.x & (IG_BM - 1);
            const int half = threadIdx.x >> 7;
            const uint32_t stg_local = smem_u32(smem);
            float* T = reinterpret_cast<float*>(smem + (size_t)BN * IG_BM * 4);
            for (int c = rank * cols_per; c < (rank + 1) * cols_per; c += ch) {
                SwapPre pre;
                swap_prefetch(p, pre, ch, c, ntile, n0, h0, w0, threadIdx.x);
                if (ch >= 16) {
                    for (int g = 4 * half; g < (ch >> 2); g += 8) {
                        float acc[16];
                        const int cc = ((c >> 2) + g) >> 2;
                        switch (splits) {
                            case 2: splitk_sum16<2>(stg_local, cc, t, acc); break;
                            case 4: splitk_sum16<4>(stg_local, cc, t, acc); break;
                            default: splitk_sum16<8>(stg_local, cc, t, acc); break;
                        }
#pragma unroll
                        for (int i = 0; i < 16; ++i) T[(4 * g + i) * IG_BM + t] = acc[i];
                    }
                } else {
                    const int gg = half;
                    float4 v[8];
#pragma unroll
                    for (int sidx = 0; sidx < 8; ++sidx)
                        v[sidx] = dsmem_ld_f4(dsmem_map(stg_local, (uint32_t)sidx) + (uint32_t)((((c >> 2) + gg) * IG_BM + t) * 16));
                    float4 a = make_float4(0.f, 0.f, 0.f, 0.f);
#pragma unroll
                    for (int sidx = 0; sidx < 8; ++sidx) { a.x += v[sidx].x; a.y += v[sidx].y; a.z += v[sidx].z; a.w += v[sidx].w; }
                    T[(4 * gg + 0) * IG_BM + t] = a.x;
                    T[(4 * gg + 1) * IG_BM + t] = a.y;
                    T[(4 * gg + 2) * IG_BM + t] = a.z;
                    T[(4 * gg + 3) * IG_BM + t] = a.w;
                }
                cons_bar_sync();
                swap_store_chunk<SILU>(p, pre, T, ntile, threadIdx.x);
                cons_bar_sync();
            }
        } else if (warp < IG_CONS / 32) {
            const int rank = (int)cluster_ctarank() / rk_mul;
            const int rows_per = IG_BM / splits;
            const int t = threadIdx.x;
            const int chunks = BN >> 4;
            const uint32_t stg_local = smem_u32(smem);
            for (int item = t; item < rows_per * chunks; item += IG_CONS) {
                const int rl = item % rows_per;
                const int cc = item / rows_per;
                const int r = rank * rows_per + rl;
                const int wi = r % p.tw, hi = (r / p.tw) % p.th, ni = r / (p.tw * p.th);
                const int n = n0 + ni, h = h0 + hi, w = w0 + wi;
                const bool ok = (ni < p.tn) && (n < p.Nb) && (h < p.Ho) && (w < p.Wo);
                float acc[16];
                switch (splits) {
                    case 2: splitk_sum16<2>(stg_local, cc, r, acc, rk_mul, rk_add); break;
                    case 4: splitk_sum16<4>(stg_local, cc, r, acc, rk_mul, rk_add); break;
                    default: splitk_sum16<8>(stg_local, cc, r, acc, rk_mul, rk_add); break;
                }
                if (ok) {
                    const long orow = ((long)n * p.Ho + h) * p.Wo + w;
                    float mu, rstd;
                    ln_row_stats(p.epi, orow, true, mu, rstd);
                    epi_store16<0, 16, float, SILU>(p.epi, acc, n, orow, ntile * BN + cc * 16, mu, rstd);
                }
            }
        }
        B2_TS(if (ts && threadIdx.x == 0) ts[7] = globaltimer_ns();)
        cluster_sync_all();
    }
    if (PAIR) {
        cluster_arrive_relaxed();
        cluster_wait();
    }
}

template <int BN, bool PAIR, bool SILU = false>
__global__ void __launch_bounds__(IG_THREADS, 1) igemm_kernel(const __grid_constant__ IgemmParams p) { igemm_body<BN, PAIR, SILU>(p); }
template <int BN>
__global__ void __launch_bounds__(IG_THREADS, 1) igemm_pad0_kernel(const __grid_constant__ IgemmParams p) { igemm_body<BN, false, false, true>(p); }

using IgemmFn = void (*)(IgemmParams);
template <bool PAIR>
static IgemmFn igemm_fn(int bn) {
    switch (bn) {
#define B2_IG_CASE(N) case N: if constexpr (PAIR && (N % 32)) return nullptr; else return igemm_kernel<N, PAIR>;
        B2_IG_CASE(16) B2_IG_CASE(32) B2_IG_CASE(48) B2_IG_CASE(64) B2_IG_CASE(80) B2_IG_CASE(96) B2_IG_CASE(112) B2_IG_CASE(128)
        B2_IG_CASE(144) B2_IG_CASE(160) B2_IG_CASE(176) B2_IG_CASE(192) B2_IG_CASE(208) B2_IG_CASE(224) B2_IG_CASE(240) B2_IG_CASE(256)
#undef B2_IG_CASE
        default: return nullptr;
    }
}
static IgemmFn igemm_select(int bn, bool pair, bool silu, bool pad0 = false) {
    if (pad0) {
        if (pair || silu) return nullptr;
        switch (bn) {
            case 64: return igemm_pad0_kernel<64>;
            case 128: return igemm_pad0_kernel<128>;
            case 256: return igemm_pad0_kernel<256>;
            default: return nullptr;
        }
    }
    if (!silu) return pair ? igemm_fn<true>(bn) : igemm_fn<false>(bn);
    if (pair) return nullptr;
    switch (bn) {
        case 16: return igemm_kernel<16, false, true>;
        case 32: return igemm_kernel<32, false, true>;
        case 64: return igemm_kernel<64, false, true>;
        case 128: return igemm_kernel<128, false, true>;
        default: return nullptr;
    }
}

static PFN_cuTensorMapEncodeTiled_v12000 get_encode() {
    static PFN_cuTensorMapEncodeTiled_v12000 fn = nullptr;
    if (fn) return fn;
    void* p = nullptr;
    cudaDriverEntryPointQueryResult qres;
    cudaError_t err = cudaGetDriverEntryPoint("cuTensorMapEncodeTiled", &p, cudaEnableDefault, &qres);
    if (err != cudaSuccess || qres != cudaDriverEntryPointSuccess || !p) {
        b2_set_error("cudaGetDriverEntryPoint(cuTensorMapEncodeTiled) failed: %s",
                     cudaGetErrorString(err));
        return nullptr;
    }
    fn = reinterpret_cast<PFN_cuTensorMapEncodeTiled_v12000>(p);
    return fn;
}

static thread_local bool g_plan_dry = false;
void igemm_set_dry_run(bool on) { g_plan_dry = on; }

static int encode_act_map(CUtensorMap* m, const ActView& a, int box_c, int box_w, int box_h, int box_n,
                          int estride) {
    if (g_plan_dry) return 0;
    auto enc = get_encode();
    if (!enc) return -1;
    cuuint64_t dims[4] = {(cuuint64_t)a.C, (cuuint64_t)a.W, (cuuint64_t)a.H, (cuuint64_t)a.N};
    cuuint64_t strides[3] = {(cuuint64_t)a.ld * 2, (cuuint64_t)a.W * a.ld * 2,
                             (cuuint64_t)a.H * a.W * a.ld * 2};
    cuuint32_t box[4] = {(cuuint32_t)box_c, (cuuint32_t)box_w, (cuuint32_t)box_h, (cuuint32_t)box_n};
    cuuint32_t es[4] = {1, (cuuint32_t)estride, (cuuint32_t)estride, 1};
    CUresult r = enc(m, CU_TENSOR_MAP_DATA_TYPE_FLOAT16, 4, const_cast<__half*>(a.ptr), dims, strides,
                     box, es, CU_TENSOR_MAP_INTERLEAVE_NONE, CU_TENSOR_MAP_SWIZZLE_128B,
                     CU_TENSOR_MAP_L2_PROMOTION_L2_256B, CU_TENSOR_MAP_FLOAT_OOB_FILL_NONE);
    if (r != CUDA_SUCCESS) {
        b2_set_error("cuTensorMapEncodeTiled(act) failed: %d (ptr %p dims %d,%d,%d,%d ld %d box "
                     "%d,%d,%d,%d es %d)",
                     (int)r, a.ptr, a.C, a.W, a.H, a.N, a.ld, box_c, box_w, box_h, box_n, estride);
        return -1;
    }
    return 0;
}

static int encode_w_map(CUtensorMap* m, const __half* w, int rows, int ld, int box_rows) {
    if (g_plan_dry) return 0;
    auto enc = get_encode();
    if (!enc) return -1;
    cuuint64_t dims[2] = {(cuuint64_t)ld, (cuuint64_t)rows};
    cuuint64_t strides[1] = {(cuuint64_t)ld * 2};
    cuuint32_t box[2] = {IG_BK, (cuuint32_t)box_rows};
    cuuint32_t es[2] = {1, 1};
    CUresult r = enc(m, CU_TENSOR_MAP_DATA_TYPE_FLOAT16, 2, const_cast<__half*>(w), dims, strides, box,
                     es, CU_TENSOR_MAP_INTERLEAVE_NONE, CU_TENSOR_MAP_SWIZZLE_128B,
                     CU_TENSOR_MAP_L2_PROMOTION_L2_256B, CU_TENSOR_MAP_FLOAT_OOB_FILL_NONE);
    if (r != CUDA_SUCCESS) {
        b2_set_error("cuTensorMapEncodeTiled(weights) failed: %d (rows %d ld %d box %d)", (int)r, rows,
                     ld, box_rows);
        return -1;
    }
    return 0;
}

size_t igemm_partial_floats(int splits, long rows_total, int n_valid) {
    long n_pad = ((n_valid + 255) / 256 + 1) * 256;
    return (size_t)splits * rows_total * n_pad;
}

static int plan_swap(const IgemmDesc& d, IgemmPlan* plan) {
    IgemmParams& p = plan->p;
    if ((d.epi.flags & (IG_GEGLU | IG_PAD0)) || d.nseg < 1 || d.nseg > IG_MAX_SRC || d.epi.rowstat_out || d.epi.colsum || d.epi.out2) {
        b2_set_error("igemm(swap): unsupported (GEGLU / tap origin 0 / LayerNorm fold / row statistics / transposed V / nseg %d)", d.nseg);
        return -1;
    }
    int BN = d.BN;
    const long rows_total = (long)d.Nb * d.Ho * d.Wo;
    if (BN <= 0) BN = rows_total >= 256 ? 256 : (rows_total >= 128 ? 128 : 64);
    if (BN != 64 && BN != 128 && BN != 256) {
        b2_set_error("igemm(swap): BN %d must be 64, 128 or 256", BN);
        return -1;
    }
    p.swap = 1;
    { static const char* dm = getenv("B2_DBG_MODE"); p.dbg_mode = dm ? atoi(dm) : 0; }
    p.acc_bufs = 1;
    p.BN = BN;
    auto lg = [](int v) { int l = 0; while ((1 << l) < v) ++l; return l; };
    int tw, th, tn;
    if (d.Ho == 1 && d.Nb == 1) { tw = BN; th = 1; tn = 1; }
    else if (d.Wo >= 16) { tw = 16; th = BN / 16; tn = 1; }
    else { tw = 8; th = 8; tn = BN / 64; }
    p.tw = tw; p.th = th; p.tn = tn;
    p.tw_log2 = lg(tw); p.th_log2 = lg(th);
    p.tiles_w = (d.Wo + tw - 1) / tw;
    p.tiles_h = (d.Ho + th - 1) / th;
    p.tiles_n = (d.Nb + tn - 1) / tn;
    p.Wo = d.Wo; p.Ho = d.Ho; p.Nb = d.Nb;
    p.stride = d.stride < 1 ? 1 : d.stride;
    p.nseg = d.nseg;
    int total_kb = 0;
    for (int s = 0; s < d.nseg; ++s) {
        const ActView& a = d.src[s];
        if (a.C % IG_BK != 0 || (a.ld % 8) != 0 || (reinterpret_cast<uintptr_t>(a.ptr) & 15) || (d.ntap[s] != 1 && d.ntap[s] != 9)) {
            b2_set_error("igemm(swap): bad source %d", s);
            return -1;
        }
        p.seg_ntap[s] = d.ntap[s];
        p.seg_cblocks[s] = a.C / IG_BK;
        p.seg_c0[s] = 0;
        total_kb += d.ntap[s] * p.seg_cblocks[s];
        if (encode_act_map(&p.tmA[s], a, IG_BK, tw * p.stride, th * p.stride, tn, p.stride)) return -1;
    }
    p.total_kb = total_kb;
    if (d.w_ld < total_kb * IG_BK || (d.w_ld % 8) != 0 || (reinterpret_cast<uintptr_t>(d.w) & 15)) {
        b2_set_error("igemm(swap): weight ld %d < K %d or misaligned", d.w_ld, total_kb * IG_BK);
        return -1;
    }
    if (encode_w_map(&p.tmB, d.w, d.w_rows, d.w_ld, IG_BM)) return -1;
    p.a_bytes = IG_BM * IG_BK * 2;
    p.b_bytes = (uint32_t)BN * IG_BK * 2;
    int splits = d.splits < 1 ? 1 : d.splits;
    if (splits > total_kb) splits = total_kb;
    if (splits >= 8) splits = 8; else if (splits >= 4) splits = 4; else if (splits >= 2) splits = 2;
    p.kb_per_split = (total_kb + splits - 1) / splits;
    while (splits > 1 && (total_kb + p.kb_per_split - 1) / p.kb_per_split != splits) {
        splits >>= 1;
        p.kb_per_split = (total_kb + splits - 1) / splits;
    }
    plan->splits = splits;
    plan->rows_total = rows_total;
    p.epi = d.epi;
    p.dbg_ts = d.dbg_ts;
    if (splits > 1) p.epi.flags |= IG_SPLITK;
    const int c_tiles = (d.epi.n_valid + IG_BM - 1) / IG_BM;
    p.n_pad = c_tiles * IG_BM;
    if ((d.epi.n_valid & 7) || (d.epi.ldc & 7) || (d.epi.res && (d.epi.ldr & 7)) || (d.epi.colbias && (d.epi.colbias_bstride & 3)) ||
        (reinterpret_cast<uintptr_t>(d.epi.out) & 15) || (reinterpret_cast<uintptr_t>(d.epi.res) & 15) ||
        (reinterpret_cast<uintptr_t>(d.epi.colbias) & 15)) {
        b2_set_error("igemm(swap): epilogue needs n_valid/ldc/ldr multiples of 8 and 16-byte aligned pointers");
        return -1;
    }
    const size_t stage_bytes = (size_t)IG_BM * IG_BK * 2 + (size_t)BN * IG_BK * 2;
    static const char* sw_stage_env = getenv("B2_SWAP_STAGE_KB");
    int stages = (int)(((size_t)(sw_stage_env ? atoi(sw_stage_env) : (d.ring_kb > 0 ? d.ring_kb : 200)) * 1024) / stage_bytes);
    if (stages < 2) stages = 2;
    if (stages > IG_MAX_STAGES) stages = IG_MAX_STAGES;
    if (stages > p.kb_per_split) stages = p.kb_per_split < 2 ? 2 : p.kb_per_split;
    size_t pipe_bytes = stages * stage_bytes;
    {
        const int cols_per = BN / splits;
        const size_t need = (splits > 1 ? (size_t)BN * IG_BM * 4 : 0) + (size_t)(cols_per < SWAP_CH ? cols_per : SWAP_CH) * IG_BM * 4;
        if (need > pipe_bytes) {
            stages = (int)((need + stage_bytes - 1) / stage_bytes);
            if (stages > IG_MAX_STAGES) {
                b2_set_error("igemm(swap): split-K staging does not fit (BN %d)", BN);
                return -1;
            }
            pipe_bytes = stages * stage_bytes;
        }
    }
    p.num_stages = stages;
    plan->smem = pipe_bytes + 1024 + 512;
    uint32_t cols = 32;
    while (cols < (uint32_t)BN) cols <<= 1;
    p.tmem_cols = cols;
    plan->grid = dim3(p.tiles_w * p.tiles_h * p.tiles_n, c_tiles, splits);
    plan->mode = 0;
    return 0;
}

int b2_device_sms() {
    static int sms = 0;
    if (sms == 0) {
        int dev = 0, n = 0;
        if (cudaGetDevice(&dev) == cudaSuccess && cudaDeviceGetAttribute(&n, cudaDevAttrMultiProcessorCount, dev) == cudaSuccess && n > 0)
            sms = n;
        else
            sms = IG_SMS;
        cudaGetLastError();
    }
    return sms;
}

static int igemm_ctas_per_sm(int bn, bool pair, bool silu, bool pad0) {
    if (g_plan_dry) return 1;
    IgemmFn fn = igemm_select(bn, pair, silu, pad0);
    int n = 0;
    if (fn && cudaOccupancyMaxActiveBlocksPerMultiprocessor(&n, fn, IG_THREADS, 0) == cudaSuccess && n > 0) return n;
    cudaGetLastError();
    return 1;
}

int igemm_plan(const IgemmDesc& d, IgemmPlan* plan) {
    *plan = IgemmPlan{};
    if (d.swap) return plan_swap(d, plan);
    IgemmParams& p = plan->p;
    if (d.nseg < 1 || d.nseg > IG_MAX_SRC) {
        b2_set_error("igemm: bad nseg %d", d.nseg);
        return -1;
    }
    const bool geglu = (d.epi.flags & IG_GEGLU) != 0;
    const int n_gemm = geglu ? d.epi.n_valid * 2 : d.epi.n_valid;
    int BN = d.BN;
    if (BN <= 0) {
        if (n_gemm <= 256 && n_gemm % 16 == 0) BN = n_gemm;
        else if (n_gemm < 16) BN = 16;
        else if (n_gemm % 128 == 0) BN = 128;
        else if (n_gemm % 160 == 0) BN = 160;
        else if (n_gemm % 64 == 0) BN = 64;
        else BN = 128;
    }
    if (BN % 16 != 0 || BN < 16 || BN > 256 || (geglu && (BN % 32 != 0 || n_gemm % BN != 0))) {
        b2_set_error("igemm: unsupported BN %d (n %d)", BN, n_gemm);
        return -1;
    }
    const bool pair = d.pair != 0;
    if ((d.epi.flags & IG_SILU) && !igemm_select(BN, pair, true)) {
        b2_set_error("igemm: no SiLU-epilogue kernel for BN %d%s (16/32/64/128, single CTAs)", BN, pair ? " (CTA pair)" : "");
        return -1;
    }
    if ((d.epi.flags & IG_PAD0) && !igemm_select(BN, pair, (d.epi.flags & IG_SILU) != 0, true)) {
        b2_set_error("igemm: no tap-origin-0 kernel for BN %d%s (64/128/256, single CTAs, no SiLU)", BN, pair ? " (CTA pair)" : "");
        return -1;
    }
    if (pair && BN % 32 != 0) {
        b2_set_error("igemm(pair): BN %d must be a multiple of 32", BN);
        return -1;
    }
    p.BN = BN;
    { static const char* dm = getenv("B2_DBG_MODE"); p.dbg_mode = dm ? atoi(dm) : 0; }
    const int n_tiles = (n_gemm + BN - 1) / BN;
    if (d.w_rows < n_gemm) {
        if (d.w_rows <= 0) {
            b2_set_error("igemm: w_rows %d", d.w_rows);
            return -1;
        }
    }
    int tw, th, tn;
    if (d.Ho == 1 && d.Nb == 1) {
        tw = IG_BM; th = 1; tn = 1;
    } else {
        if (d.Wo <= 16) tw = d.Wo;
        else if (d.Wo % 16 == 0) tw = 16;
        else if (d.Wo % 8 == 0) tw = 8;
        else tw = 16;
        th = IG_BM / tw;
        if (th > d.Ho) th = d.Ho;
        tn = IG_BM / (tw * th);
        if (tn > d.Nb) tn = d.Nb;
        if (tn < 1) tn = 1;
    }
    p.tw = tw; p.th = th; p.tn = tn;
    p.tiles_w = (d.Wo + tw - 1) / tw;
    p.tiles_h = (d.Ho + th - 1) / th;
    p.tiles_n = (d.Nb + tn - 1) / tn;
    p.Wo = d.Wo; p.Ho = d.Ho; p.Nb = d.Nb;
    p.stride = d.stride < 1 ? 1 : d.stride;
    if (p.stride > 2) {
        b2_set_error("igemm: stride %d", p.stride);
        return -1;
    }
    p.nseg = d.nseg;
    int total_kb = 0;
    for (int s = 0; s < d.nseg; ++s) {
        const ActView& a = d.src[s];
        if (a.C % IG_BK != 0 || (a.ld % 8) != 0 || (reinterpret_cast<uintptr_t>(a.ptr) & 15)) {
            b2_set_error("igemm: source %d: C=%d must be a multiple of 64, ld=%d multiple of 8, ptr "
                         "16B aligned",
                         s, a.C, a.ld);
            return -1;
        }
        if (d.ntap[s] != 1 && d.ntap[s] != 9) {
            b2_set_error("igemm: ntap %d", d.ntap[s]);
            return -1;
        }
        p.seg_ntap[s] = d.ntap[s];
        p.seg_cblocks[s] = a.C / IG_BK;
        p.seg_c0[s] = 0;
        total_kb += d.ntap[s] * p.seg_cblocks[s];
        if (encode_act_map(&p.tmA[s], a, IG_BK, tw * p.stride, th * p.stride, tn, p.stride)) return -1;
    }
    p.total_kb = total_kb;
    if (d.w_ld < total_kb * IG_BK || (d.w_ld % 8) != 0 || (reinterpret_cast<uintptr_t>(d.w) & 15)) {
        b2_set_error("igemm: weight ld %d < K %d or misaligned", d.w_ld, total_kb * IG_BK);
        return -1;
    }
    const int b_rows = pair ? BN / 2 : BN;
    if (encode_w_map(&p.tmB, d.w, d.w_rows, d.w_ld, b_rows)) return -1;
    p.a_bytes = (uint32_t)(tw * th * tn) * IG_BK * 2;
    p.b_bytes = (uint32_t)BN * IG_BK * 2;
    int splits = d.splits < 1 ? 1 : d.splits;
    if (splits > total_kb) splits = total_kb;
    if (pair && splits > 4) splits = 4;
    if (splits >= 8) splits = 8;
    else if (splits >= 4) splits = 4;
    else if (splits >= 2) splits = 2;
    p.kb_per_split = (total_kb + splits - 1) / splits;
    while (splits > 1 && (total_kb + p.kb_per_split - 1) / p.kb_per_split != splits) {
        splits >>= 1;
        p.kb_per_split = (total_kb + splits - 1) / splits;
    }
    plan->splits = splits;
    plan->rows_total = (long)d.Nb * d.Ho * d.Wo;
    p.epi = d.epi;
    p.dbg_ts = d.dbg_ts;
    p.n_pad = n_tiles * BN;
    if (splits > 1) {
        if (geglu) {
            b2_set_error("igemm: split-K cannot be combined with GEGLU");
            return -1;
        }
        p.epi.flags |= IG_SPLITK;
    }
    const size_t stage_bytes = (size_t)IG_BM * IG_BK * 2 + (size_t)BN * IG_BK * 2;
    const int per_sm = igemm_ctas_per_sm(BN, pair, (d.epi.flags & IG_SILU) != 0, (d.epi.flags & IG_PAD0) != 0);
    const long resident = (long)per_sm * b2_device_sms();
    static const char* pc_env = getenv("B2_PERSIST_CTAS");
    const long persist_ctas = pc_env ? atoi(pc_env) : resident;
    const long all_tiles = (long)p.tiles_w * p.tiles_h * p.tiles_n * n_tiles;
    static const bool no_persist_e = getenv("B2_NO_PERSIST") != nullptr;
    const bool will_persist = !no_persist_e && splits == 1 && all_tiles > resident && 2 * BN <= 512;
    const long total_ctas = will_persist ? persist_ctas : all_tiles * splits;
    static const char* stage_env = getenv("B2_STAGE_KB");
    const size_t ring_budget = stage_env ? (size_t)atoi(stage_env) * 1024
                                         : (d.ring_kb > 0 ? (size_t)d.ring_kb * 1024
                                                          : (size_t)((per_sm >= 2 && total_ctas > b2_device_sms() ? 100 : 200) * 1024));
    int stages = (int)(ring_budget / stage_bytes);
    if (stages < 2) stages = 2;
    if (stages > IG_MAX_STAGES) stages = IG_MAX_STAGES;
    if (stages > p.kb_per_split) stages = p.kb_per_split < 2 ? 2 : p.kb_per_split;
    p.num_stages = stages;
    size_t pipe_bytes = stages * stage_bytes;
    if (splits > 1) {
        const size_t stg = (size_t)BN * IG_BM * 4;
        if (stg > pipe_bytes) {
            stages = (int)((stg + stage_bytes - 1) / stage_bytes);
            if (stages > IG_MAX_STAGES) {
                b2_set_error("igemm: split-K staging does not fit (BN %d)", BN);
                return -1;
            }
            p.num_stages = stages;
            pipe_bytes = stages * stage_bytes;
        }
    }
    plan->smem = pipe_bytes + 1024  + 512 ;
    const int m_tiles = p.tiles_w * p.tiles_h * p.tiles_n;
    int grid_x = m_tiles;
    p.acc_bufs = 1;
    if (will_persist) {
        grid_x = (int)(persist_ctas / n_tiles);
        if (grid_x < 1) grid_x = 1;
        if (grid_x > m_tiles) grid_x = m_tiles;
        p.acc_bufs = 2;
    }
    if (pair) {
        grid_x = (p.acc_bufs == 2 && grid_x > 2) ? (grid_x & ~1) : ((grid_x + 1) & ~1);
    }
    uint32_t cols = 32;
    while (cols < (uint32_t)(BN * p.acc_bufs)) cols <<= 1;
    p.tmem_cols = cols;
    plan->grid = dim3(grid_x, n_tiles, splits);
    plan->mode = pair ? 1 : 0;
    plan->pair = pair ? 1 : 0;
    return 0;
}

int igemm_encode_act_map(CUtensorMap* m, const ActView& a, int box_c, int box_w, int box_h, int box_n, int estride) {
    return encode_act_map(m, a, box_c, box_w, box_h, box_n, estride);
}
int igemm_encode_w_map(CUtensorMap* m, const __half* w, int rows, int ld, int box_rows) { return encode_w_map(m, w, rows, ld, box_rows); }

int igemm_init() {
    static bool attr_set = false;
    if (!attr_set) {
        for (int bn = 16; bn <= 256; bn += 16) {
            for (int pair = 0; pair < 4; ++pair) {
                IgemmFn fn = igemm_select(bn, pair == 1, pair == 2, pair == 3);
                if (!fn) continue;
                cudaError_t e = cudaFuncSetAttribute(fn, cudaFuncAttributeMaxDynamicSharedMemorySize, 227 * 1024);
                if (e != cudaSuccess) {
                    b2_set_error("cudaFuncSetAttribute(igemm BN %d%s): %s", bn, pair ? " pair" : "", cudaGetErrorString(e));
                    return -1;
                }
            }
        }
        if (!get_encode()) return -1;
        attr_set = true;
    }
    return 0;
}

int igemm_launch(const IgemmPlan& plan, cudaStream_t stream) {
    if (igemm_init()) return -1;
    const int cz = plan.splits > 1 ? plan.splits : 1;
    IgemmFn fn = igemm_select(plan.p.BN, plan.pair, (plan.p.epi.flags & IG_SILU) != 0, (plan.p.epi.flags & IG_PAD0) != 0);
    if (!fn) {
        b2_set_error("igemm launch: no kernel for BN %d%s%s%s", plan.p.BN, plan.pair ? " (CTA pair)" : "",
                     (plan.p.epi.flags & IG_SILU) ? " with the SiLU epilogue" : "", (plan.p.epi.flags & IG_PAD0) ? " with tap origin 0" : "");
        return -1;
    }
    cudaError_t e = plan.pair ? launch_kc(fn, plan.grid, dim3(IG_THREADS), plan.smem, stream, 2, cz, plan.p)
                              : launch_k(fn, plan.grid, dim3(IG_THREADS), plan.smem, stream, cz, plan.p);
    if (e != cudaSuccess) {
        b2_set_error("igemm launch: %s", cudaGetErrorString(e));
        return -1;
    }
    return 0;
}

}
```

ai-rtc-agent_b200/csrc/igemm.cuh:

```cuda
#pragma once
#include <cuda.h>
#include <cuda_fp16.h>
#include <cuda_runtime.h>
#include <stdint.h>

namespace b2 {

constexpr int IG_BM = 128;
constexpr int IG_BK = 64;
constexpr int IG_MAX_SRC = 3;
constexpr int IG_MAX_STAGES = 8;
constexpr int IG_CONS = 256;
constexpr int IG_THREADS = IG_CONS + 32;
constexpr int IG_SMS = 132;

enum : int {
    IG_RELU = 1,
    IG_GEGLU = 2,
    IG_SPLITK = 4,
    IG_SILU = 8,
    IG_PAD0 = 16,
};

struct IgEpilogue {
    __half* out;
    int ldc;
    const float* colbias;
    int colbias_bstride;
    const __half* res;
    int ldr;
    float acc_scale;
    float res_scale;
    int flags;
    int n_valid;
    unsigned long long* rowstat_out;
    const unsigned long long* rowstat_in;
    const float* colsum;
    float ln_inv_c, ln_eps;
    __half* out2;
    int ld2, col2;
};

constexpr float IG_STAT_SCALE = 1048576.f;

struct IgemmParams {
    CUtensorMap tmA[IG_MAX_SRC];
    CUtensorMap tmB;
    int seg_ntap[IG_MAX_SRC];
    int seg_cblocks[IG_MAX_SRC];
    int seg_c0[IG_MAX_SRC];
    int nseg;
    int total_kb;
    int kb_per_split;
    int tw, th, tn;
    int tiles_w, tiles_h, tiles_n;
    int Wo, Ho, Nb;
    int stride;
    int BN;
    int num_stages;
    int acc_bufs;
    uint32_t a_bytes;
    uint32_t b_bytes;
    uint32_t tmem_cols;
    unsigned long long* dbg_ts;
    int n_pad;
    int swap;
    int tw_log2, th_log2;
    int dbg_mode;
    IgEpilogue epi;
};

struct ActView {
    const __half* ptr;
    int N, H, W, C;
    int ld;
};

struct IgemmDesc {
    ActView src[IG_MAX_SRC];
    int ntap[IG_MAX_SRC];
    int nseg;
    const __half* w;
    int w_rows;
    int w_ld;
    int stride;
    int Nb, Ho, Wo;
    int BN;
    int swap;
    int splits;
    int ring_kb;
    int max_splits;
    int pair_auto;
    int pair_splits;
    int pair;
    unsigned long long* dbg_ts;
    float* partial;
    int* tile_counters;
    IgEpilogue epi;
};

struct IgemmPlan {
    int mode;
    IgemmParams p;
    dim3 grid;
// ... 19 lines not shown
```

ai-rtc-agent_b200/host/capi.py:

```python
from __future__ import annotations

import ctypes as C
import os

_HERE = os.path.dirname(os.path.abspath(__file__))
LIB_PATH = os.environ.get("B200SD_LIB") or os.path.join(os.path.dirname(_HERE), "libb200sd.so")


class B2Error(RuntimeError):
    pass


class ActView(C.Structure):
    _fields_ = [("ptr", C.c_void_p), ("n", C.c_int), ("h", C.c_int), ("w", C.c_int), ("c", C.c_int),
                ("ld", C.c_int)]


class IgemmDesc(C.Structure):
    _fields_ = [
        ("src", ActView * 3), ("ntap", C.c_int * 3), ("nseg", C.c_int),
        ("w", C.c_void_p), ("w_rows", C.c_int), ("w_ld", C.c_int), ("stride", C.c_int),
        ("nb", C.c_int), ("ho", C.c_int), ("wo", C.c_int),
        ("bn", C.c_int), ("splits", C.c_int), ("partial", C.c_void_p),
        ("out", C.c_void_p), ("ldc", C.c_int),
        ("colbias", C.c_void_p), ("colbias_bstride", C.c_int),
        ("res", C.c_void_p), ("ldr", C.c_int),
        ("acc_scale", C.c_float), ("res_scale", C.c_float),
        ("flags", C.c_int), ("n_valid", C.c_int), ("swap", C.c_int),
        ("rowstat_out", C.c_void_p), ("rowstat_in", C.c_void_p), ("colsum", C.c_void_p), ("ln_c", C.c_int), ("ln_eps", C.c_float),
        ("out2", C.c_void_p), ("ld2", C.c_int), ("col2", C.c_int),
    ]


class IgemmPlanInfo(C.Structure):
    _fields_ = [
        ("mode", C.c_int), ("swap", C.c_int), ("bn", C.c_int), ("splits", C.c_int),
        ("grid_x", C.c_int), ("grid_y", C.c_int), ("grid_z", C.c_int),
        ("num_stages", C.c_int), ("acc_bufs", C.c_int), ("total_kb", C.c_int), ("kb_per_split", C.c_int),
        ("tmem_cols", C.c_int), ("m_tiles", C.c_int),
        ("smem_bytes", C.c_int64), ("rows_total", C.c_int64),
    ]


class AttnDesc(C.Structure):
    _fields_ = [
        ("q", C.c_void_p), ("ldq", C.c_int),
        ("k", C.c_void_p), ("ldk", C.c_int), ("k_bstride", C.c_int64), ("k_rows", C.c_int64),
        ("vt", C.c_void_p), ("ldvt", C.c_int), ("vt_bstride", C.c_int64), ("vt_cols", C.c_int64),
        ("out", C.c_void_p), ("ldo", C.c_int),
        ("nb", C.c_int), ("heads", C.c_int), ("sq", C.c_int), ("skv", C.c_int), ("d_real", C.c_int),
        ("dp", C.c_int),
    ]


class EngineConfig(C.Structure):
    _fields_ = [
        ("block_out_channels", C.c_int * 4), ("heads", C.c_int * 4), ("down_attn", C.c_int * 4),
        ("cross_attention_dim", C.c_int), ("layers_per_block", C.c_int), ("norm_groups", C.c_int),
        ("ctx_tokens", C.c_int), ("batch", C.c_int), ("height", C.c_int), ("width", C.c_int),
        ("do_add_noise", C.c_int), ("use_cuda_graph", C.c_int), ("controlnet", C.c_int), ("control_processor", C.c_int),
        ("vae", C.c_int), ("vae_scaling_factor", C.c_float),
    ]


IN_U8_NHWC, IN_F32_NCHW, IN_F16_NCHW = 0, 1, 2
OUT_U8_NCHW, OUT_F16_NCHW = 0, 1
IG_RELU = 1
IG_GEGLU = 2
IG_SILU = 8
IG_PAD0 = 16
SC_IN_U8, SC_IN_TANH3, SC_OUT_RELU, SC_OUT_SILU, SC_IN_OFFSET = 1, 2, 4, 32, 64
CONTROL_FRAME, CONTROL_HED = 0, 1
VAE_TINY, VAE_KL = 0, 1
IG_TCONV = 64
IG_PAIR = 128

_lib = None


def lib() -> C.CDLL:
    global _lib
    if _lib is None:
        if not os.path.exists(LIB_PATH):
            raise B2Error(f"{LIB_PATH} not found: build it with `make -C ai-rtc-agent_b200/csrc` "
                          "(or __graft_entry__.build()); there is no CPU fallback")
        _lib = C.CDLL(LIB_PATH)
        _lib.b2sd_last_error.restype = C.c_char_p
        _lib.b2sd_version.restype = C.c_int
        _lib.b2sd_op_igemm.argtypes = [C.POINTER(IgemmDesc), C.c_void_p]
        _lib.b2sd_op_igemm.restype = C.c_int
        _lib.b2sd_igemm_plan_dry.argtypes = [C.POINTER(IgemmDesc), C.c_int, C.c_int, C.POINTER(IgemmPlanInfo)]
        _lib.b2sd_igemm_plan_dry.restype = C.c_int
        _lib.b2sd_groupnorm_plan_dry.argtypes = [C.c_int, C.c_int, C.c_int, C.c_int, C.POINTER(C.c_int), C.POINTER(C.c_int), C.POINTER(C.c_int)]
        _lib.b2sd_groupnorm_plan_dry.restype = C.c_int
        _lib.b2sd_igemm_partial_floats.argtypes = [C.c_int, C.c_int64, C.c_int]
        _lib.b2sd_igemm_partial_floats.restype = C.c_uint64
        vp, ci, cf, i64 = C.c_void_p, C.c_int, C.c_float, C.c_int64
        _lib.b2sd_op_attention.argtypes = [C.POINTER(AttnDesc), vp]
        _lib.b2sd_op_groupnorm.argtypes = [vp, ci, ci, vp, ci, ci, vp, vp, vp, ci, ci, ci, ci, cf, ci, vp]
        _lib.b2sd_groupnorm_last_path.argtypes = []
        _lib.b2sd_groupnorm_last_path.restype = C.c_int
        _lib.b2sd_op_layernorm.argtypes = [vp, ci, vp, vp, vp, ci, i64, ci, cf, vp]
        _lib.b2sd_op_upsample2x.argtypes = [vp, vp, ci, ci, ci, ci, vp]
        _lib.b2sd_op_smallconv.argtypes = [vp, vp, vp, vp, ci, ci, ci, ci, ci, ci, ci, ci, ci, vp]
        _lib.b2sd_op_smallconv_ex.argtypes = [vp, vp, vp, vp, ci, ci, ci, ci, ci, ci, ci, ci, ci, vp, ci, i64, vp, vp]
        _lib.b2sd_op_maxpool2x2.argtypes = [vp, vp, ci, ci, ci, ci, vp]
        _lib.b2sd_op_hed_project.argtypes = [vp, ci, ci, i64, vp, vp, vp, vp]
        _lib.b2sd_op_hed_fuse.argtypes = [C.POINTER(vp), C.POINTER(ci), C.POINTER(ci), ci, ci, ci, vp, vp, vp]
        _lib.b2sd_op_lcm_step.argtypes = [vp, vp, vp, vp, vp, ci, ci, ci, vp]
        _lib.b2sd_op_post_u8.argtypes = [vp, ci, vp, ci, ci, ci, vp]
        _lib.b2sd_op_nv12_to_rgb.argtypes = [vp, ci, vp, ci, vp, ci, ci, ci, vp]
        _lib.b2sd_op_rgb_to_nv12.argtypes = [vp, vp, ci, vp, ci, ci, ci, ci, vp]
        _lib.b2sd_codec_probe.restype = C.c_int
        _lib.b2sd_create.argtypes = [C.POINTER(EngineConfig), C.POINTER(vp)]
        _lib.b2sd_destroy.argtypes = [vp]
        _lib.b2sd_create_lane.argtypes = [vp, C.POINTER(EngineConfig), C.POINTER(vp)]
        _lib.b2sd_load_tensor.argtypes = [vp, C.c_char_p, vp, ci, C.POINTER(i64), ci]
        _lib.b2sd_prepare.argtypes = [vp, vp, vp, vp, vp, vp]
        _lib.b2sd_export_packed.argtypes = [vp, C.c_char_p]
        _lib.b2sd_import_packed.argtypes = [vp, C.c_char_p]
        _lib.b2sd_set_prompt_embeds.argtypes = [vp, vp, vp]
        _lib.b2sd_set_timesteps.argtypes = [vp, vp, vp]
        _lib.b2sd_step.argtypes = [vp, vp, ci, ci, vp, vp]
        _lib.b2sd_step_ex.argtypes = [vp, vp, ci, ci, ci, vp, ci, vp]
        _lib.b2sd_get_tensor.argtypes = [vp, C.c_char_p, vp, i64, C.POINTER(i64), C.POINTER(ci), vp]
        _lib.b2sd_launches_per_step.argtypes = [vp]
        _lib.b2sd_share_stream_state.argtypes = [vp, vp]
        _lib.b2sd_share_stream_state.restype = C.c_int
        _lib.b2sd_set_concurrency.argtypes = [vp, ci]
        _lib.b2sd_set_concurrency.restype = C.c_int
        _lib.b2sd_profile.argtypes = [vp, vp, ci, ci, vp, ci, C.c_char_p, i64, vp]
        _lib.b2sd_profile.restype = C.c_int
        _lib.b2sd_profile_kind.argtypes = [vp, C.c_char_p, ci, C.POINTER(C.c_double), C.POINTER(ci), C.POINTER(C.c_double), vp]
        _lib.b2sd_profile_kind.restype = C.c_int
        _lib.b2sd_profile_gate.argtypes = [ci]
        _lib.b2sd_profile_gate.restype = C.c_int
        for name in ("create", "create_lane", "destroy", "load_tensor", "prepare", "export_packed", "import_packed", "set_prompt_embeds", "set_timesteps", "step",
                     "step_ex", "get_tensor", "launches_per_step"):
            getattr(_lib, "b2sd_" + name).restype = C.c_int
        for name in ("attention", "groupnorm", "layernorm", "upsample2x", "smallconv", "smallconv_ex", "maxpool2x2", "hed_project", "hed_fuse", "lcm_step", "post_u8", "nv12_to_rgb", "rgb_to_nv12"):
            getattr(_lib, "b2sd_op_" + name).restype = C.c_int
    return _lib


def check(rc: int, what: str = "") -> None:
    if rc != 0:
        raise B2Error(f"{what}: {lib().b2sd_last_error().decode(errors='replace')}")


def current_stream_ptr() -> int:
    import torch
    return torch.cuda.current_stream().cuda_stream
```

ai-rtc-agent_b200/host/ops.py:

```python
from __future__ import annotations

import ctypes as C
from typing import Optional, Sequence, Tuple

import torch

from . import capi


_SCRATCH = {}


def pack_conv_weight(w_oihw: torch.Tensor) -> torch.Tensor:
    o, i, kh, kw = w_oihw.shape
    return w_oihw.permute(0, 2, 3, 1).reshape(o, kh * kw * i).contiguous().to(torch.float16)


def _view(t: torch.Tensor) -> capi.ActView:
    assert t.dtype == torch.float16 and t.is_cuda and t.dim() == 4
    n, h, w, c = t.shape
    assert t.stride(3) == 1 and t.stride(2) % 8 == 0
    ld = t.stride(2)
    assert t.stride(1) == w * ld and t.stride(0) == h * w * ld, "NHWC view must be dense in n,h,w"
    return capi.ActView(t.data_ptr(), n, h, w, c, ld)


def igemm(srcs: Sequence[Tuple[torch.Tensor, int]], w: torch.Tensor, out: torch.Tensor, *,
          stride: int = 1, colbias: Optional[torch.Tensor] = None, res: Optional[torch.Tensor] = None,
          acc_scale: float = 1.0, res_scale: float = 1.0, relu: bool = False, geglu: bool = False, silu: bool = False,
          bn: int = 0, splits: int = 1, n_valid: Optional[int] = None, timeline: Optional[torch.Tensor] = None, swap: bool = False,
          tconv: bool = False, pair: bool = False, pad0: bool = False,
          rowstat_out: Optional[torch.Tensor] = None, rowstat_in: Optional[torch.Tensor] = None,
          colsum: Optional[torch.Tensor] = None, ln_c: int = 0, ln_eps: float = 1e-5,
          out2: Optional[torch.Tensor] = None, col2: int = 0) -> torch.Tensor:
    d = _igemm_desc(srcs, w, out, stride=stride, colbias=colbias, res=res, acc_scale=acc_scale, res_scale=res_scale, relu=relu,
                    geglu=geglu, silu=silu, bn=bn, splits=splits, n_valid=n_valid, timeline=timeline, swap=swap, tconv=tconv, pair=pair,
                    pad0=pad0,
                    rowstat_out=rowstat_out, rowstat_in=rowstat_in, colsum=colsum, ln_c=ln_c, ln_eps=ln_eps, out2=out2, col2=col2)
    capi.check(capi.lib().b2sd_op_igemm(C.byref(d), capi.current_stream_ptr()), "b2sd_op_igemm")
    return out


def igemm_engine_plan(srcs, w, out, *, autotile: int = 1, allow_swap: bool = True, **kw) -> capi.IgemmPlanInfo:
    d = _igemm_desc(srcs, w, out, **kw)
    info = capi.IgemmPlanInfo()
    capi.check(capi.lib().b2sd_igemm_plan_dry(C.byref(d), autotile, int(allow_swap), C.byref(info)), "b2sd_igemm_plan_dry")
    return info


def _igemm_desc(srcs, w, out, *, stride=1, colbias=None, res=None, acc_scale=1.0, res_scale=1.0, relu=False, geglu=False,
                silu=False, bn=0, splits=1, n_valid=None, timeline=None, swap=False, tconv=False, pair=False, pad0=False, rowstat_out=None,
                rowstat_in=None, colsum=None, ln_c=0, ln_eps=1e-5, out2=None, col2=0) -> capi.IgemmDesc:
    d = capi.IgemmDesc()
    d.nseg = len(srcs)
    for i, (t, ntap) in enumerate(srcs):
        d.src[i] = _view(t)
        d.ntap[i] = ntap
    assert w.dtype == torch.float16 and w.is_contiguous()
    d.w, d.w_rows, d.w_ld = w.data_ptr(), w.shape[0], w.shape[1]
    d.stride = stride
    nb, ho, wo, _ = out.shape
    d.nb, d.ho, d.wo = nb, ho, wo
    d.bn, d.splits = bn, splits
    d.swap = int(swap)
    d.out, d.ldc = out.data_ptr(), out.stride(2)
    nv = n_valid if n_valid is not None else out.shape[3]
    d.n_valid = nv
    if timeline is not None:
        d.partial = timeline.data_ptr()
    if colbias is not None:
        assert colbias.dtype == torch.float32 and colbias.is_contiguous()
        d.colbias = colbias.data_ptr()
        d.colbias_bstride = colbias.shape[1] if colbias.dim() == 2 and colbias.shape[0] > 1 else 0
    if res is not None:
        assert res.dtype == torch.float16
        d.res, d.ldr = res.data_ptr(), res.stride(2)
    d.acc_scale, d.res_scale = acc_scale, res_scale
    d.flags = (capi.IG_RELU if relu else 0) | (capi.IG_GEGLU if geglu else 0) | (capi.IG_TCONV if tconv else 0) | (capi.IG_PAIR if pair else 0) \
        | (capi.IG_SILU if silu else 0) | (capi.IG_PAD0 if pad0 else 0)
    if rowstat_out is not None:
        assert rowstat_out.dtype == torch.int64 and rowstat_out.is_contiguous()
        d.rowstat_out = rowstat_out.data_ptr()
    if rowstat_in is not None:
        assert rowstat_in.dtype == torch.int64 and colsum is not None and colsum.dtype == torch.float32 and ln_c > 0
        d.rowstat_in, d.colsum, d.ln_c, d.ln_eps = rowstat_in.data_ptr(), colsum.data_ptr(), ln_c, ln_eps
    if out2 is not None:
        assert out2.dtype == torch.float16 and out2.dim() == 2 and out2.stride(1) == 1
        d.out2, d.ld2, d.col2 = out2.data_ptr(), out2.stride(0), col2
    return d


def _sp():
    return capi.current_stream_ptr()


def attention(q, k, vt, out, *, nb, heads, sq, skv, d_real, dp, k_bstride, vt_bstride):
    d = capi.AttnDesc()
    d.q, d.ldq = q.data_ptr(), q.stride(0)
    d.k, d.ldk, d.k_bstride, d.k_rows = k.data_ptr(), k.stride(0), k_bstride, k.shape[0]
    d.vt, d.ldvt, d.vt_bstride, d.vt_cols = vt.data_ptr(), vt.stride(0), vt_bstride, vt.shape[1]
    d.out, d.ldo = out.data_ptr(), out.stride(0)
    d.nb, d.heads, d.sq, d.skv, d.d_real, d.dp = nb, heads, sq, skv, d_real, dp
    capi.check(capi.lib().b2sd_op_attention(C.byref(d), _sp()), "b2sd_op_attention")
    return out


GN_PATHS = {0: "cluster", 1: "fused", 2: "stats+apply"}


def groupnorm(xa, xb, gamma, beta, y, *, groups=32, eps=1e-5, silu=True, return_path=False):
    nb, h, w, ca = xa.shape
    cb = 0 if xb is None else xb.shape[3]
    capi.check(capi.lib().b2sd_op_groupnorm(
        xa.data_ptr(), ca, xa.stride(2), 0 if xb is None else xb.data_ptr(), cb, 0 if xb is None else xb.stride(2),
        gamma.data_ptr(), beta.data_ptr(), y.data_ptr(), y.stride(2), nb, h * w, groups, eps, int(silu), _sp()),
        "b2sd_op_groupnorm")
    if return_path:
        return y, GN_PATHS[capi.lib().b2sd_groupnorm_last_path()]
    return y


def layernorm(x, gamma, beta, y, eps=1e-5):
    rows, c = x.shape
    capi.check(capi.lib().b2sd_op_layernorm(x.data_ptr(), x.stride(0), gamma.data_ptr(), beta.data_ptr(),
                                            y.data_ptr(), y.stride(0), rows, c, eps, _sp()), "b2sd_op_layernorm")
    return y


def upsample2x(x, y):
    nb, h, w, c = x.shape
    capi.check(capi.lib().b2sd_op_upsample2x(x.data_ptr(), y.data_ptr(), nb, h, w, c, _sp()), "b2sd_op_upsample2x")
    return y


def smallconv(x, w_oihw, bias, y, *, flags=0):
    nb, in_h, in_w, cin = x.shape
    _, h, w, cout = y.shape
    capi.check(capi.lib().b2sd_op_smallconv(x.data_ptr(), w_oihw.data_ptr(), 0 if bias is None else bias.data_ptr(),
                                            y.data_ptr(), y.stride(2), nb, h, w, cin, cout, in_h, in_w, flags, _sp()),
               "b2sd_op_smallconv")
    return y


def smallconv_ex(x, w_oihw, bias, y, *, flags=0, res=None, res_bstride=None, in_off=None):
    nb, in_h, in_w, cin = x.shape
    _, h, w, _ = y.shape
    cout = w_oihw.shape[0]
    rp, ldr, bs = 0, 0, 0
    if res is not None:
        assert res.dtype == torch.float16 and res.stride(3) == 1
        rp, ldr = res.data_ptr(), res.stride(2)
        bs = res.stride(0) if res_bstride is None else res_bstride
    capi.check(capi.lib().b2sd_op_smallconv_ex(x.data_ptr(), w_oihw.data_ptr(), bias.data_ptr() if bias is not None else None,
                                               y.data_ptr(), y.stride(2), nb, h, w, cin, cout, in_h, in_w, flags, rp, ldr, bs,
                                               in_off.data_ptr() if in_off is not None else None, _sp()), "b2sd_op_smallconv_ex")
    return y


def maxpool2x2(x, y):
    nb, h, w, c = x.shape
    capi.check(capi.lib().b2sd_op_maxpool2x2(x.data_ptr(), y.data_ptr(), nb, h, w, c, _sp()), "b2sd_op_maxpool2x2")
    return y
# ... 31 lines not shown
```

ai-rtc-agent_b200/host/stream.py:

```python
from __future__ import annotations

import ctypes as C
import os
from typing import Callable, Dict, List, Optional

import numpy as np
import torch

from . import capi
from .arch import UNetArch

NUM_TRAIN_TIMESTEPS = 1000
LCM_ORIGINAL_INFERENCE_STEPS = 50
LCM_TIMESTEP_SCALING = 10.0
LCM_SIGMA_DATA = 0.5


def scaled_linear_alphas_cumprod(beta_start: float = 0.00085, beta_end: float = 0.012) -> torch.Tensor:
    betas = torch.linspace(beta_start ** 0.5, beta_end ** 0.5, NUM_TRAIN_TIMESTEPS, dtype=torch.float32) ** 2
    return torch.cumprod(1.0 - betas, dim=0)


def lcm_timestep_table(num_inference_steps: int) -> List[int]:
    stride_train = NUM_TRAIN_TIMESTEPS // LCM_ORIGINAL_INFERENCE_STEPS
    origin = [(i + 1) * stride_train - 1 for i in range(LCM_ORIGINAL_INFERENCE_STEPS)]
    if num_inference_steps > LCM_ORIGINAL_INFERENCE_STEPS:
        raise ValueError("num_inference_steps cannot exceed the 50 LCM origin steps")
    step = LCM_ORIGINAL_INFERENCE_STEPS // num_inference_steps
    return list(reversed(origin))[::step][:num_inference_steps]


def lcm_boundary_scalings(timestep: int):
    scaled = timestep * LCM_TIMESTEP_SCALING
    denom = scaled * scaled + LCM_SIGMA_DATA * LCM_SIGMA_DATA
    return LCM_SIGMA_DATA * LCM_SIGMA_DATA / denom, scaled / denom ** 0.5


class ImageProcessor:

    def __init__(self, vae_scale_factor: int = 8):
        self.vae_scale_factor = vae_scale_factor

    def preprocess(self, image, height: Optional[int] = None, width: Optional[int] = None) -> torch.Tensor:
        from PIL import Image
        if isinstance(image, Image.Image):
            if height and width and image.size != (width, height):
                image = image.resize((width, height), Image.LANCZOS)
            arr = np.asarray(image.convert("RGB"), dtype=np.float32) / 255.0
            image = torch.from_numpy(arr).permute(2, 0, 1)
        if isinstance(image, np.ndarray):
            image = torch.from_numpy(image)
        if image.dim() == 3:
            image = image.unsqueeze(0)
        if height and width and (image.shape[-2] != height or image.shape[-1] != width):
            image = torch.nn.functional.interpolate(image, size=(height, width))
        return image if image.min() < 0 else 2.0 * image - 1.0


class StreamDiffusion:
    def __init__(self, arch: UNetArch, unet_sd: Dict[str, torch.Tensor], vae_sd: Dict[str, torch.Tensor],
                 t_index_list: List[int], prompt_encoder: Callable[[str], torch.Tensor],
                 torch_dtype: torch.dtype = torch.float16, width: int = 512, height: int = 512,
                 do_add_noise: bool = True, use_denoising_batch: bool = True, frame_buffer_size: int = 1,
                 cfg_type: str = "self", device: str = "cuda", use_cuda_graph: bool = True,
                 packed_blob: Optional[str] = None, parent: Optional["StreamDiffusion"] = None,
                 controlnet_sd: Optional[Dict[str, torch.Tensor]] = None,
                 hed_sd: Optional[Dict[str, torch.Tensor]] = None, use_tiny_vae: bool = True,
                 vae_scaling_factor: float = 0.18215):
        if hed_sd is not None and controlnet_sd is None:
            raise ValueError("the HED processor needs a ControlNet")
        if frame_buffer_size != 1:
            raise NotImplementedError("frame_buffer_size > 1 is not on the reference's path (lib/pipeline.py:28)")
        if not use_denoising_batch:
            raise NotImplementedError("img2img mode must use denoising batch for now.")
        if torch_dtype != torch.float16:
            raise NotImplementedError("the sm_90a kernels compute in fp16 (fp32 accumulate) like the reference engines")
        self.arch = arch
        self.device = torch.device(device)
        self.dtype = torch_dtype
        self.generator = None
        self.height, self.width = height, width
        self.latent_height, self.latent_width = height // 8, width // 8
        self.frame_bff_size = frame_buffer_size
        self.denoising_steps_num = len(t_index_list)
        self.cfg_type = cfg_type
        self.use_denoising_batch = use_denoising_batch
        self.batch_size = self.denoising_steps_num * frame_buffer_size
        self.trt_unet_batch_size = self.batch_size
        self.t_list = list(t_index_list)
        self.do_add_noise = do_add_noise
        self.similar_image_filter = False
        self.prev_image_result = None
        self.inference_time_ema = 0.0
        self._ev = None
        self.image_processor = ImageProcessor(8)
        self.prompt_encoder = prompt_encoder
        self.text_encoder = prompt_encoder
        self.unet = self
        self.vae = self
        self._handle = C.c_void_p()
        self._prepared = False
        self._lib = capi.lib()
        cfg = capi.EngineConfig()
        for i in range(4):
            cfg.block_out_channels[i] = arch.block_out_channels[i]
            cfg.heads[i] = arch.heads[i]
            cfg.down_attn[i] = arch.down_attn[i]
        cfg.cross_attention_dim = arch.cross_attention_dim
        cfg.layers_per_block = arch.layers_per_block
        cfg.norm_groups = arch.norm_groups
        cfg.ctx_tokens = arch.ctx_tokens
        cfg.batch = self.batch_size
        cfg.height, cfg.width = height, width
        cfg.do_add_noise = int(do_add_noise)
        cfg.use_cuda_graph = int(use_cuda_graph)
        cfg.controlnet = int(controlnet_sd is not None)
        cfg.control_processor = capi.CONTROL_HED if hed_sd is not None else capi.CONTROL_FRAME
        cfg.vae = capi.VAE_TINY if use_tiny_vae else capi.VAE_KL
        cfg.vae_scaling_factor = 0.0 if use_tiny_vae else float(vae_scaling_factor)
        if not torch.cuda.is_available():
            raise capi.B2Error("no CUDA device: the H100 pipeline has no CPU fallback")
        if self.device.index is None:
            self.device = torch.device("cuda", torch.cuda.current_device())
        torch.cuda.set_device(self.device)
        self._ctor = dict(torch_dtype=torch_dtype, width=width, height=height, do_add_noise=do_add_noise,
                          use_denoising_batch=use_denoising_batch, frame_buffer_size=frame_buffer_size, cfg_type=cfg_type,
                          device=device, use_cuda_graph=use_cuda_graph, use_tiny_vae=use_tiny_vae,
                          vae_scaling_factor=vae_scaling_factor)
        self.lanes: List["StreamDiffusion"] = []
        self._parent = parent
        if parent is not None:
            capi.check(self._lib.b2sd_create_lane(parent._handle, C.byref(cfg), C.byref(self._handle)), "b2sd_create_lane")
            return
        capi.check(self._lib.b2sd_create(C.byref(cfg), C.byref(self._handle)), "b2sd_create")
        if packed_blob is not None:
            capi.check(self._lib.b2sd_import_packed(self._handle, os.fsencode(packed_blob)), f"b2sd_import_packed({packed_blob})")
        else:
            self._load("", unet_sd)
            self._load("vae.", vae_sd)
            self._load("controlnet.", controlnet_sd or {})
            self._load("hed.", hed_sd or {})

    def set_concurrency(self, frames_in_flight: int) -> None:
        capi.check(self._lib.b2sd_set_concurrency(self._handle, int(frames_in_flight)), "b2sd_set_concurrency")
        self._prepared = False

    def export_packed(self, path: str) -> None:
        self._check()
        tmp = f"{path}.tmp{os.getpid()}"
        capi.check(self._lib.b2sd_export_packed(self._handle, os.fsencode(tmp)), f"b2sd_export_packed({path})")
        os.replace(tmp, path)

    def __del__(self):
        try:
            if getattr(self, "_handle", None) and self._handle.value:
                self._lib.b2sd_destroy(self._handle)
                self._handle = C.c_void_p()
        except Exception:
            pass

    def _load(self, prefix: str, sd: Dict[str, torch.Tensor]) -> None:
        for key, t in sd.items():
            t = t.detach()
            if t.dtype not in (torch.float16, torch.float32):
                t = t.float()
            t = t.contiguous()
            shape = (C.c_int64 * t.dim())(*t.shape)
            capi.check(self._lib.b2sd_load_tensor(self._handle, (prefix + key).encode(), t.data_ptr(),
                                                  0 if t.dtype == torch.float16 else 1, shape, t.dim()),
                       f"b2sd_load_tensor({prefix + key})")

    def _stream(self) -> int:
        return torch.cuda.current_stream(self.device).cuda_stream

    @torch.no_grad()
    def prepare(self, prompt: str, negative_prompt: str = "", num_inference_steps: int = 50,
                guidance_scale: float = 1.2, delta: float = 1.0,
                generator: Optional[torch.Generator] = None, seed: int = 2) -> None:
        self.generator = generator if generator is not None else torch.Generator()
        self.generator.manual_seed(seed)
        self.guidance_scale = 1.0 if self.cfg_type == "none" else guidance_scale
        if self.guidance_scale > 1.0:
            raise NotImplementedError("classifier-free guidance (guidance_scale > 1) is not on the reference's path "
                                      "(lib/pipeline.py:14 passes 0.0)")
        self.delta = delta
        T = self.denoising_steps_num
        self.prompt_embeds = self._encode(prompt).repeat(self.batch_size, 1, 1)
        self.timesteps = lcm_timestep_table(num_inference_steps)
        self.sub_timesteps = [self.timesteps[t] for t in self.t_list]
        self.sub_timesteps_tensor = torch.tensor(self.sub_timesteps, dtype=torch.long, device=self.device)
        self.sub_timesteps_tensor = torch.repeat_interleave(self.sub_timesteps_tensor, repeats=self.frame_bff_size, dim=0)
        self.init_noise = torch.randn((self.batch_size, 4, self.latent_height, self.latent_width),
                                      generator=self.generator).to(dtype=self.dtype)
        self.stock_noise = torch.zeros_like(self.init_noise)
        scal = [lcm_boundary_scalings(t) for t in self.sub_timesteps]
        ac = scaled_linear_alphas_cumprod()
        f16 = lambda v: torch.tensor(v, dtype=torch.float32).to(self.dtype)
        self.c_skip = f16([s[0] for s in scal]).view(T, 1, 1, 1)
        self.c_out = f16([s[1] for s in scal]).view(T, 1, 1, 1)
        self.alpha_prod_t_sqrt = torch.stack([ac[t].sqrt() for t in self.sub_timesteps]).to(self.dtype).view(T, 1, 1, 1)
        self.beta_prod_t_sqrt = torch.stack([(1 - ac[t]).sqrt() for t in self.sub_timesteps]).to(self.dtype).view(T, 1, 1, 1)
        self._engine_prepare()
        for lane in self.lanes:
            lane._prepare_like(self)

    _SCHEDULE_ATTRS = ("generator", "guidance_scale", "delta", "prompt_embeds", "timesteps", "sub_timesteps", "sub_timesteps_tensor",
                       "init_noise", "stock_noise", "c_skip", "c_out", "alpha_prod_t_sqrt", "beta_prod_t_sqrt")

    def _engine_prepare(self) -> None:
        coef = torch.stack([self.alpha_prod_t_sqrt.flatten(), self.beta_prod_t_sqrt.flatten(),
                            self.c_skip.flatten(), self.c_out.flatten()]).float().contiguous()
        tsteps = torch.tensor(self.sub_timesteps, dtype=torch.float32)
        emb = self.prompt_embeds[0].to(torch.float16).cpu().contiguous()
        noise = self.init_noise.cpu().contiguous()
        capi.check(self._lib.b2sd_prepare(self._handle, emb.data_ptr(), tsteps.data_ptr(), coef.data_ptr(),
                                          noise.data_ptr(), self._stream()), "b2sd_prepare")
        self._prepared = True

    def _prepare_like(self, other: "StreamDiffusion") -> None:
        for name in self._SCHEDULE_ATTRS:
            setattr(self, name, getattr(other, name))
        self.t_list = list(other.t_list)
        self._engine_prepare()

    def add_lane(self, share_state: bool = False) -> "StreamDiffusion":
        self._check()
        lane = StreamDiffusion(self.arch, {}, {}, self.t_list, self.prompt_encoder, parent=self, **self._ctor)
        if share_state:
            capi.check(self._lib.b2sd_share_stream_state(lane._handle, self._handle), "b2sd_share_stream_state")
            self._engine_prepare()
        lane._prepare_like(self)
        self.lanes.append(lane)
        return lane

    def _encode(self, prompt: str) -> torch.Tensor:
# ... 121 lines not shown
```

include/b200sd.h:

```cpp
#ifndef B200SD_H
#define B200SD_H

#include <stdint.h>

#ifdef __cplusplus
extern "C" {
#endif

const char* b2sd_last_error(void);
int b2sd_version(void);


typedef struct {
    const void* ptr;
    int n, h, w, c;
    int ld;
} b2sd_act_view;

enum {
    B2SD_IG_RELU = 1,
    B2SD_IG_GEGLU = 2,
    B2SD_IG_SILU = 8,
    B2SD_IG_PAD0 = 16,
    B2SD_IG_TCONV = 64,
    B2SD_IG_PAIR = 128
};

typedef struct {
    b2sd_act_view src[3];
    int ntap[3];
    int nseg;
    const void* w;
    int w_rows, w_ld;
    int stride;
    int nb, ho, wo;
    int bn;
    int splits;
    void* partial;
    void* out;
    int ldc;
    const float* colbias;
    int colbias_bstride;
    const void* res;
    int ldr;
    float acc_scale, res_scale;
    int flags;
    int n_valid;
    int swap;
    void* rowstat_out;
    const void* rowstat_in;
    const float* colsum;
    int ln_c;
    float ln_eps;
    void* out2;
    int ld2, col2;
} b2sd_igemm_desc;

int b2sd_op_igemm(const b2sd_igemm_desc* d, void* stream);

typedef struct {
    int mode;
    int swap, bn, splits;
    int grid_x, grid_y, grid_z;
    int num_stages;
    int acc_bufs;
    int total_kb, kb_per_split;
    int tmem_cols;
    int m_tiles;
    int64_t smem_bytes, rows_total;
} b2sd_igemm_plan_info;
int b2sd_igemm_plan_dry(const b2sd_igemm_desc* d, int autotile, int allow_swap, b2sd_igemm_plan_info* out);

int b2sd_groupnorm_plan_dry(int ca, int cb, int groups, int hw, int* cluster, int* threads, int* pixels_per_cta);
uint64_t b2sd_igemm_partial_floats(int splits, int64_t rows_total, int n_valid);

typedef struct {
    const void* q; int ldq;
    const void* k; int ldk; int64_t k_bstride; int64_t k_rows;
    const void* vt; int ldvt; int64_t vt_bstride; int64_t vt_cols;
    void* out; int ldo;
    int nb, heads, sq, skv, d_real, dp;
} b2sd_attn_desc;
int b2sd_op_attention(const b2sd_attn_desc* d, void* stream);

int b2sd_op_groupnorm(const void* xa, int ca, int lda, const void* xb, int cb, int ldb, const float* gamma,
                      const float* beta, void* y, int ldy, int nb, int hw, int groups, float eps, int silu,
                      void* stream);
int b2sd_groupnorm_last_path(void);
int b2sd_op_layernorm(const void* x, int ldx, const float* gamma, const float* beta, void* y, int ldy,
                      int64_t rows, int c, float eps, void* stream);
int b2sd_op_upsample2x(const void* x, void* y, int nb, int h, int w, int c, void* stream);
int b2sd_op_smallconv(const void* x, const void* w_oihw, const float* bias, void* y, int ldy, int nb, int h,
                      int w, int cin, int cout, int in_h, int in_w, int flags, void* stream);
int b2sd_op_smallconv_ex(const void* x, const void* w_oihw, const float* bias, void* y, int ldy, int nb, int h, int w,
                         int cin, int cout, int in_h, int in_w, int flags, const void* res, int ldr, int64_t res_bstride,
                         const float* in_off, void* stream);
int b2sd_op_maxpool2x2(const void* x, void* y, int nb, int h, int w, int c, void* stream);
int b2sd_op_hed_project(const void* x, int ldx, int c, int64_t npix, const float* w, const float* bias, float* out, void* stream);
int b2sd_op_hed_fuse(const float* const* maps, const int* hs, const int* ws, int levels, int h, int w, void* out_u8,
                     void* edge_f16, void* stream);
int b2sd_op_lcm_step(void* x, const void* eps, const void* noise, const float* coef, void* out_latent, int T,
                     int hw, int do_add_noise, void* stream);
enum { B2SD_CSC_BT601 = 1, B2SD_CSC_FULL_RANGE = 2 };
int b2sd_op_nv12_to_rgb(const void* y, int y_pitch, const void* uv, int uv_pitch, void* rgb_nhwc, int h, int w, int flags, void* stream);
int b2sd_op_rgb_to_nv12(const void* rgb_nchw, void* y, int y_pitch, void* uv, int uv_pitch, int h, int w, int flags, void* stream);
int b2sd_codec_probe(void);
int b2sd_op_post_u8(const void* y_nhwc, int ldy, void* out_nchw_u8, int nb, int h, int w, void* stream);

typedef struct b2sd_engine* b2sd_handle;

typedef struct {
    int block_out_channels[4];
    int heads[4];
    int down_attn[4];
    int cross_attention_dim;
    int layers_per_block;
    int norm_groups;
    int ctx_tokens;
    int batch;
    int height, width;
    int do_add_noise;
    int use_cuda_graph;
    int controlnet;
    int control_processor;
    int vae;
    float vae_scaling_factor;
} b2sd_config;
enum { B2SD_CONTROL_FRAME = 0, B2SD_CONTROL_HED = 1 };
enum { B2SD_VAE_TINY = 0, B2SD_VAE_KL = 1 };

int b2sd_create(const b2sd_config* cfg, b2sd_handle* out);
int b2sd_destroy(b2sd_handle h);
int b2sd_create_lane(b2sd_handle parent, const b2sd_config* cfg, b2sd_handle* out);

int b2sd_load_tensor(b2sd_handle h, const char* key, const void* ptr, int dtype, const int64_t* shape, int ndim);

int b2sd_export_packed(b2sd_handle h, const char* path);
int b2sd_import_packed(b2sd_handle h, const char* path);

int b2sd_prepare(b2sd_handle h, const void* prompt_embeds, const float* timesteps, const float* coef,
                 const void* init_noise, void* stream);
// ... 26 lines not shown
```

Measured before the change: 175.3.

## Fold nearest-2x upsample into following 3x3 conv via sub-pixel 2x2 weights

New measurement: 175.8, median of 6. Within noise of the previous version (+0.3%).

```diff
diff --git a/ai-rtc-agent_b200/csrc/capi.cu b/ai-rtc-agent_b200/csrc/capi.cu
--- a/ai-rtc-agent_b200/csrc/capi.cu
+++ b/ai-rtc-agent_b200/csrc/capi.cu
@@ -20,7 +20,7 @@
     return a;
 }
 
-static void to_igemm_desc(const b2sd_igemm_desc* d, IgemmDesc& g) {
+static int to_igemm_desc(const b2sd_igemm_desc* d, IgemmDesc& g) {
     g.nseg = d->nseg;
     for (int s = 0; s < d->nseg && s < IG_MAX_SRC; ++s) {
         g.src[s] = to_view(d->src[s]);
@@ -31,6 +31,13 @@
     g.w_ld = d->w_ld;
     g.stride = d->stride;
     g.Nb = d->nb; g.Ho = d->ho; g.Wo = d->wo;
+    if (d->flags & B2SD_IG_UP2) {
+        if ((d->ho | d->wo) & 1) {
+            b2_set_error("B2SD_IG_UP2: output extents %d x %d must be even", d->ho, d->wo);
+            return -1;
+        }
+        g.Ho = d->ho / 2; g.Wo = d->wo / 2;
+    }
     g.BN = d->bn;
     g.swap = d->swap;
     g.pair = (d->flags & B2SD_IG_PAIR) ? 1 : 0;
@@ -45,7 +52,7 @@
     g.epi.ldr = d->ldr;
     g.epi.acc_scale = d->acc_scale;
     g.epi.res_scale = d->res_scale;
-    g.epi.flags = d->flags & (IG_RELU | IG_GEGLU | IG_SILU | IG_PAD0);
+    g.epi.flags = d->flags & (IG_RELU | IG_GEGLU | IG_SILU | IG_PAD0 | IG_UP2);
     g.epi.n_valid = d->n_valid;
     g.epi.rowstat_out = static_cast<unsigned long long*>(d->rowstat_out);
     g.epi.rowstat_in = static_cast<const unsigned long long*>(d->rowstat_in);
@@ -55,6 +62,7 @@
     g.epi.out2 = reinterpret_cast<__half*>(d->out2);
     g.epi.ld2 = d->ld2;
     g.epi.col2 = d->col2;
+    return 0;
 }
 
 int b2sd_op_igemm(const b2sd_igemm_desc* d, void* stream) {
@@ -63,10 +71,10 @@
         return -1;
     }
     IgemmDesc g{};
-    to_igemm_desc(d, g);
+    if (to_igemm_desc(d, g)) return -1;
     if (d->flags & B2SD_IG_TCONV) {
-        if (d->flags & B2SD_IG_PAD0) {
-            b2_set_error("b2sd_op_igemm: the halo-tile kernel has no tap-origin-0 variant");
+        if (d->flags & (B2SD_IG_PAD0 | B2SD_IG_UP2)) {
+            b2_set_error("b2sd_op_igemm: the halo-tile kernel has no tap-origin-0 or sub-pixel upsampling variant");
             return -1;
         }
         TconvPlan tp;
@@ -78,13 +86,27 @@
     return igemm_launch(plan, reinterpret_cast<cudaStream_t>(stream));
 }
 
+int b2sd_fold_up2_weights(const void* w_oihw, int cout, int cin, void* out) {
+    if (!w_oihw || !out || cout <= 0 || cin <= 0) {
+        b2_set_error("b2sd_fold_up2_weights: bad arguments");
+        return -1;
+    }
+    const __half* w = static_cast<const __half*>(w_oihw);
+    __half* dst = static_cast<__half*>(out);
+    for (int row = 0; row < 4 * cout; ++row)
+        for (int tap = 0; tap < 4; ++tap)
+            for (int c = 0; c < cin; ++c)
+                dst[((long)row * 4 + tap) * cin + c] = up2_fold_weight(w, cin, row % cout, c, row / cout, tap);
+    return 0;
+}
+
 int b2sd_igemm_plan_dry(const b2sd_igemm_desc* d, int autotile, int allow_swap, b2sd_igemm_plan_info* out) {
     if (!d || !out) {
         b2_set_error("b2sd_igemm_plan_dry: null argument");
         return -1;
     }
     IgemmDesc g{};
-    to_igemm_desc(d, g);
+    if (to_igemm_desc(d, g)) return -1;
     g.dbg_ts = nullptr;
     IgemmPlan plan;
     if (autotile == 2) {
diff --git a/ai-rtc-agent_b200/csrc/elementwise.cu b/ai-rtc-agent_b200/csrc/elementwise.cu
--- a/ai-rtc-agent_b200/csrc/elementwise.cu
+++ b/ai-rtc-agent_b200/csrc/elementwise.cu
@@ -952,6 +952,21 @@
     return 0;
 }
 
+__global__ void pack_up2_weight_kernel(const __half* __restrict__ w, __half* __restrict__ dst, int o, int i) {
+    const long total = 16L * o * i;
+    for (long e = (long)blockIdx.x * blockDim.x + threadIdx.x; e < total; e += (long)gridDim.x * blockDim.x) {
+        const int c = (int)(e % i);
+        const int tap = (int)((e / i) & 3);
+        const long row = e / (4L * i);
+        dst[e] = up2_fold_weight(w, i, (int)(row % o), c, (int)(row / o), tap);
+    }
+}
+int pack_up2_weight_launch(const __half* w_oihw, __half* dst, int o, int i, cudaStream_t s) {
+    pack_up2_weight_kernel<<<grid_for(16L * o * i), 256, 0, s>>>(w_oihw, dst, o, i);
+    B2_CHECK_LAUNCH("pack_up2_weight");
+    return 0;
+}
+
 __global__ void gather_rows_kernel(const __half* __restrict__ src, int src_ld, const int* __restrict__ perm,
                                    __half* __restrict__ dst, int dst_ld, int rows, int cols) {
     const long total = (long)rows * cols;
diff --git a/ai-rtc-agent_b200/csrc/elementwise.cuh b/ai-rtc-agent_b200/csrc/elementwise.cuh
--- a/ai-rtc-agent_b200/csrc/elementwise.cuh
+++ b/ai-rtc-agent_b200/csrc/elementwise.cuh
@@ -72,6 +72,17 @@
 int cast_f16_to_f32_launch(const __half* x, float* y, long n, cudaStream_t s);
 int pack_conv_weight_launch(const __half* w_oihw, __half* dst, int dst_ld, int koff, int o, int i, int taps,
                             int c0, int cn, cudaStream_t s);
+__host__ __device__ inline __half up2_fold_weight(const __half* w_oihw, int cin, int co, int c, int phase, int tap) {
+    const int py = phase >> 1, px = phase & 1, ty = tap >> 1, tx = tap & 1;
+    const int r_lo = ty ? 1 + py : 0, r_hi = ty ? 2 : py;
+    const int c_lo = tx ? 1 + px : 0, c_hi = tx ? 2 : px;
+    const __half* k = w_oihw + ((long)co * cin + c) * 9;
+    float acc = 0.f;
+    for (int r = r_lo; r <= r_hi; ++r)
+        for (int q = c_lo; q <= c_hi; ++q) acc += __half2float(k[r * 3 + q]);
+    return __float2half_rn(acc);
+}
+int pack_up2_weight_launch(const __half* w_oihw, __half* dst, int o, int i, cudaStream_t s);
 int gather_rows_launch(const __half* src, int src_ld, const int* perm, __half* dst, int dst_ld, int rows, int cols,
                        cudaStream_t s);
 
diff --git a/ai-rtc-agent_b200/csrc/engine.cu b/ai-rtc-agent_b200/csrc/engine.cu
--- a/ai-rtc-agent_b200/csrc/engine.cu
+++ b/ai-rtc-agent_b200/csrc/engine.cu
@@ -135,7 +135,8 @@
     const bool geglu = (d.epi.flags & IG_GEGLU) != 0;
     const bool silu = (d.epi.flags & IG_SILU) != 0;
     const bool pad0 = (d.epi.flags & IG_PAD0) != 0;
-    const int n_gemm = geglu ? 2 * d.epi.n_valid : d.epi.n_valid;
+    const bool up2 = (d.epi.flags & IG_UP2) != 0;
+    const int n_gemm = up2 ? 4 * d.epi.n_valid : (geglu ? 2 * d.epi.n_valid : d.epi.n_valid);
     static const bool swap_on = getenv("B2_SWAP") != nullptr, swap_off = getenv("B2_NO_SWAP") != nullptr;
     static const bool tuned = getenv("B2_NO_TUNED_TILES") == nullptr;
     static const char* ms_env = getenv("B2_MAX_SPLITS");
@@ -143,7 +144,7 @@
     int total_kb = 0;
     for (int sidx = 0; sidx < d.nseg && sidx < IG_MAX_SRC; ++sidx) total_kb += d.ntap[sidx] * (d.src[sidx].C / IG_BK);
     const long rows_all = (long)d.Nb * d.Ho * d.Wo;
-    const bool swap_here = allow_swap && !geglu && !pad0 && d.epi.n_valid >= 128 && (d.epi.n_valid & 7) == 0 &&
+    const bool swap_here = allow_swap && !geglu && !pad0 && !up2 && d.epi.n_valid >= 128 && (d.epi.n_valid & 7) == 0 &&
                            (swap_on || (!swap_off && tuned && rows_all <= 64 && total_kb >= 90));
     if (swap_here) {
         d.swap = 1;
@@ -163,8 +164,10 @@
         return 0;
     }
     d.swap = 0;
-    auto vt_ok = [&](int bn) { return !d.epi.out2 || d.epi.col2 % bn == 0; };
-    if (tuned && !geglu && !silu && !pad0 && n_gemm % 160 == 0 && total_kb >= 40 && vt_ok(160)) {
+    auto tile_ok = [&](int bn) {
+        return (!d.epi.out2 || d.epi.col2 % bn == 0) && (!up2 || ((bn == 64 || bn == 128 || bn == 160) && d.epi.n_valid % bn == 0));
+    };
+    if (tuned && !geglu && !silu && !pad0 && n_gemm % 160 == 0 && total_kb >= 40 && tile_ok(160)) {
         d.BN = 160; d.splits = 1; d.partial = nullptr;
         TRY(igemm_plan(d, &plan));
         const int m_tiles = plan.p.tiles_w * plan.p.tiles_h * plan.p.tiles_n;
@@ -172,7 +175,7 @@
         int bn = 0, splits = 0;
         if (tiles < 132) {
             if (m_tiles >= 8) { bn = 160; splits = 4; }
-            else if (m_tiles >= 2 && n_gemm % 256 == 0 && total_kb >= 180 && vt_ok(256)) { bn = 256; splits = 8; }
+            else if (m_tiles >= 2 && n_gemm % 256 == 0 && total_kb >= 180 && tile_ok(256)) { bn = 256; splits = 8; }
         }
         if (bn && splits > max_splits) bn = 0;
         if (bn) {
@@ -187,7 +190,7 @@
         if (geglu && (bn % 32 != 0 || bn < 64)) continue;
         if (silu && (bn > 128 || bn % 16 || (bn & (bn - 1)))) continue;
         if (pad0 && bn != 64 && bn != 128 && bn != 256) continue;
-        if (n_gemm % bn == 0 && vt_ok(bn)) valid.push_back(bn);
+        if (n_gemm % bn == 0 && tile_ok(bn)) valid.push_back(bn);
     }
     if (valid.empty()) {
         int bn = 16;
@@ -371,6 +374,20 @@
         packed_bytes[name] = (size_t)rows_pad * K * 2;
         return dst;
     }
+    __half* pack_up2(const std::string& wkey, int cout, int cin, cudaStream_t s) {
+        const std::string name = wkey + ":up2";
+        auto it = packed.find(name);
+        if (it != packed.end()) return it->second;
+        const Raw* r = get(wkey);
+        if (!r) return nullptr;
+        if (!r->p) { b2_set_error("parameter '%s' was released after the first prepare and is not in the packed cache", wkey.c_str()); return nullptr; }
+        const size_t bytes = (size_t)16 * cout * cin * 2;
+        __half* dst = static_cast<__half*>(weights.alloc(bytes));
+        if (!dst || pack_up2_weight_launch(r->p, dst, cout, cin, s)) return nullptr;
+        packed[name] = dst;
+        packed_bytes[name] = bytes;
+        return dst;
+    }
     __half* pack_rows(const std::string& name, const std::vector<std::pair<std::string, std::vector<int>>>& parts,
                       int K, cudaStream_t s) {
         auto it = packed.find(name);
@@ -451,7 +468,7 @@
 
     int add_igemm(std::vector<Op>& dst, IgemmDesc d) {
         const bool geglu = (d.epi.flags & IG_GEGLU) != 0;
-        const int n_gemm = geglu ? 2 * d.epi.n_valid : d.epi.n_valid;
+        const int n_gemm = (d.epi.flags & IG_UP2) ? 4 * d.epi.n_valid : (geglu ? 2 * d.epi.n_valid : d.epi.n_valid);
         const bool extras = d.epi.rowstat_out || d.epi.colsum || d.epi.out2;
         if (concurrency > 1 && d.max_splits == 0) d.max_splits = 4;
         if (concurrency >= 4 && d.pair_auto == 0) { d.pair_auto = 1; d.pair_splits = 1; }
@@ -536,6 +553,34 @@
             return 0;
         }
         return add_igemm(dst, d);
+    }
+
+    int add_up2_conv(const Act& x, const std::string& wkey, const std::string& bkey, const Act& y, cudaStream_t s) {
+        const Raw* w = get(wkey);
+        if (!w) return -1;
+        cur = wkey;
+        const int cout = (int)w->shape[0], cin = (int)w->shape[1];
+        if (cin != x.c || w->shape.size() != 4 || w->shape[2] != 3 || w->shape[3] != 3 || y.n != x.n || y.h != 2 * x.h ||
+            y.w != 2 * x.w || y.c != cout) {
+            b2_set_error("%s: not a 3x3 conv from %d channels at %dx%d to %d channels at %dx%d", wkey.c_str(), x.c, x.h, x.w, y.c, y.h, y.w);
+            return -1;
+        }
+        __half* wp = pack_up2(wkey, cout, cin, s);
+        if (!wp) return -1;
+        IgemmDesc d{};
+        d.nseg = 1; d.src[0] = view(x); d.ntap[0] = 4;
+        d.w = wp; d.w_rows = 4 * cout; d.w_ld = 4 * cin;
+        d.stride = 1;
+        d.Nb = x.n; d.Ho = x.h; d.Wo = x.w;
+        d.epi.out = y.p; d.epi.ldc = y.ld;
+        if (!bkey.empty()) {
+            d.epi.colbias = vec({bkey}, nullptr, 16);
+            if (!d.epi.colbias) return -1;
+        }
+        d.epi.acc_scale = 1.f; d.epi.res_scale = 1.f;
+        d.epi.flags = IG_UP2;
+        d.epi.n_valid = cout;
+        return add_igemm(prog_frame, d);
     }
 
     struct LinExtra {
@@ -1298,12 +1343,8 @@
             h = o;
         }
         if (i < 3) {
-            Act up = new_act(1, h.h * 2, h.w * 2, h.c);
-            const Act hin = h;
-            ++launches;
-            prog_frame.push_back(Op([hin, up](cudaStream_t st) { return upsample2x_launch(hin.p, up.p, hin.n, hin.h, hin.w, hin.c, st); }, "upsample2x"));
-            Act o = new_act(1, up.h, up.w, h.c);
-            TRY(add_conv(prog_frame, up, bp + ".upsamplers.0.conv.weight", bp + ".upsamplers.0.conv.bias", 9, 1, o, 0, nullptr, s));
+            Act o = new_act(1, h.h * 2, h.w * 2, h.c);
+            TRY(add_up2_conv(h, bp + ".upsamplers.0.conv.weight", bp + ".upsamplers.0.conv.bias", o, s));
             h = o;
         }
         taps["vae.dec.up." + std::to_string(i)] = h;
@@ -1457,13 +1498,9 @@
             taps["up." + std::to_string(i) + "." + std::to_string(j)] = h;
         }
         if (i != nlev - 1) {
-            Act up = new_act(B, h.h * 2, h.w * 2, co);
-            const Act hin = h;
-            ++launches;
-            prog_frame.push_back(Op([hin, up](cudaStream_t st) { return upsample2x_launch(hin.p, up.p, hin.n, hin.h, hin.w, hin.c, st); }, "upsample2x"));
-            Act o = new_act(B, up.h, up.w, co);
+            Act o = new_act(B, h.h * 2, h.w * 2, co);
             const std::string k = "up_blocks." + std::to_string(i) + ".upsamplers.0.conv.";
-            TRY(add_conv(prog_frame, up, k + "weight", k + "bias", 9, 1, o, 0, nullptr, s));
+            TRY(add_up2_conv(h, k + "weight", k + "bias", o, s));
             h = o;
         }
     }
@@ -1507,13 +1544,9 @@
             ++li;
         }
         if (st != 3) {
-            Act up = new_act(1, dcur.h * 2, dcur.w * 2, 64);
-            const Act hin = dcur;
-            ++launches;
-            prog_frame.push_back(Op([hin, up](cudaStream_t s2) { return upsample2x_launch(hin.p, up.p, hin.n, hin.h, hin.w, hin.c, s2); }, "upsample2x"));
             ++li;
-            Act o = new_act(1, up.h, up.w, 64);
-            TRY(add_conv(prog_frame, up, "vae.decoder.layers." + std::to_string(li) + ".weight", "", 9, 1, o, 0, nullptr, s));
+            Act o = new_act(1, dcur.h * 2, dcur.w * 2, 64);
+            TRY(add_up2_conv(dcur, "vae.decoder.layers." + std::to_string(li) + ".weight", "", o, s));
             dcur = o;
             ++li;
         } else {
@@ -1805,7 +1838,7 @@
     }
     BlobWriter w{f};
     w.put("B2SDPACK", 8);
-    w.pod((uint32_t)3);
+    w.pod((uint32_t)4);
     b2sd_config cfg = h->cfg;
     cfg.batch = 0; cfg.height = 0; cfg.width = 0; cfg.use_cuda_graph = 0; cfg.do_add_noise = 0;
     w.pod(cfg);
@@ -1862,11 +1895,14 @@
     char magic[8];
     rd.get(magic, 8);
     const uint32_t version = rd.pod<uint32_t>();
-    b2sd_config cfg{};
-    if (version == 1) rd.get(&cfg, offsetof(b2sd_config, controlnet));
-    else if (version == 2) rd.get(&cfg, offsetof(b2sd_config, vae));
-    else cfg = rd.pod<b2sd_config>();
-    bool same = rd.ok && memcmp(magic, "B2SDPACK", 8) == 0 && version >= 1 && version <= 3 && cfg.cross_attention_dim == h->cfg.cross_attention_dim &&
+    if (rd.ok && memcmp(magic, "B2SDPACK", 8) == 0 && version <= 3) {
+        fclose(f);
+        b2_set_error("b2sd_import_packed: %s is a format-%u blob without the folded upsampler weights (format 4); re-pack it from "
+                     "the checkpoint", path, version);
+        return -1;
+    }
+    const b2sd_config cfg = rd.pod<b2sd_config>();
+    bool same = rd.ok && memcmp(magic, "B2SDPACK", 8) == 0 && version == 4 && cfg.cross_attention_dim == h->cfg.cross_attention_dim &&
                 cfg.layers_per_block == h->cfg.layers_per_block && cfg.norm_groups == h->cfg.norm_groups && cfg.ctx_tokens == h->cfg.ctx_tokens &&
                 cfg.controlnet == h->cfg.controlnet && cfg.control_processor == h->cfg.control_processor && cfg.vae == h->cfg.vae &&
                 (cfg.vae != B2SD_VAE_KL || cfg.vae_scaling_factor == h->cfg.vae_scaling_factor);
diff --git a/ai-rtc-agent_b200/csrc/igemm.cu b/ai-rtc-agent_b200/csrc/igemm.cu
--- a/ai-rtc-agent_b200/csrc/igemm.cu
+++ b/ai-rtc-agent_b200/csrc/igemm.cu
@@ -131,7 +131,7 @@
     }
 }
 
-template <int BN, bool PAIR, bool SILU, bool PAD0 = false>
+template <int BN, bool PAIR, bool SILU, bool PAD0 = false, bool UP2 = false>
 __device__ __forceinline__ void igemm_body(const IgemmParams& p) {
     extern __shared__ uint8_t smem_raw[];
     uint8_t* smem = reinterpret_cast<uint8_t*>((reinterpret_cast<uintptr_t>(smem_raw) + 1023) &
@@ -151,6 +151,8 @@
     const int ntile = blockIdx.y;
     const int kb_begin = blockIdx.z * p.kb_per_split;
     const int kb_end = min(p.total_kb, kb_begin + p.kb_per_split);
+    [[maybe_unused]] const int up_phase = UP2 ? ntile * BN / p.epi.n_valid : 0;
+    [[maybe_unused]] const int up_ntile = UP2 ? ntile - up_phase * (p.epi.n_valid / BN) : ntile;
     [[maybe_unused]] unsigned long long* ts = p.dbg_ts ? p.dbg_ts + ((size_t)(blockIdx.z * gridDim.y + blockIdx.y) * gridDim.x + blockIdx.x) * 8 : nullptr;
     B2_TS(if (ts && threadIdx.x == 0) ts[0] = globaltimer_ns();)
 
@@ -201,7 +203,10 @@
                     uint8_t* sa = smem + (size_t)stage * stage_bytes;
                     uint8_t* sb = sa + A_BYTES;
                     int dy = 0, dx = 0;
-                    if (p.seg_ntap[seg] == 9) {
+                    if constexpr (UP2) {
+                        dy = (up_phase >> 1) + (tap >> 1) - 1;
+                        dx = (up_phase & 1) + (tap & 1) - 1;
+                    } else if (p.seg_ntap[seg] == 9) {
                         dy = tap / 3 - (PAD0 ? 0 : 1);
                         dx = tap % 3 - (PAD0 ? 0 : 1);
                     }
@@ -302,11 +307,14 @@
                     const int wi = r % p.tw, hi = (r / p.tw) % p.th, ni = r / (p.tw * p.th);
                     const int n = n0 + ni, hh = h0 + hi, ww = w0 + wi;
                     rw[h].ok = (ni < p.tn) && (n < p.Nb) && (hh < p.Ho) && (ww < p.Wo);
-                    rw[h].orow = ((long)n * p.Ho + hh) * p.Wo + ww;
+                    if constexpr (UP2)
+                        rw[h].orow = ((long)n * 2 * p.Ho + 2 * hh + (up_phase >> 1)) * (2 * p.Wo) + 2 * ww + (up_phase & 1);
+                    else
+                        rw[h].orow = ((long)n * p.Ho + hh) * p.Wo + ww;
                     rw[h].b = n;
                     ln_row_stats(e, rw[h].orow, rw[h].ok, rw[h].mu, rw[h].rstd);
                 }
-                epi_frag<BN, SILU>(e, acc, rw, ntile, ln_fma, lane);
+                epi_frag<BN, SILU>(e, acc, rw, up_ntile, ln_fma, lane);
             }
             B2_TS(if (ts && it == 0 && threadIdx.x == 0) ts[5] = globaltimer_ns();)
         }
@@ -380,10 +388,14 @@
                     default: splitk_sum16<8>(stg_local, cc, r, acc, rk_mul, rk_add); break;
                 }
                 if (ok) {
-                    const long orow = ((long)n * p.Ho + h) * p.Wo + w;
+                    long orow;
+                    if constexpr (UP2)
+                        orow = ((long)n * 2 * p.Ho + 2 * h + (up_phase >> 1)) * (2 * p.Wo) + 2 * w + (up_phase & 1);
+                    else
+                        orow = ((long)n * p.Ho + h) * p.Wo + w;
                     float mu, rstd;
                     ln_row_stats(p.epi, orow, true, mu, rstd);
-                    epi_store16<0, 16, float, SILU>(p.epi, acc, n, orow, ntile * BN + cc * 16, mu, rstd);
+                    epi_store16<0, 16, float, SILU>(p.epi, acc, n, orow, up_ntile * BN + cc * 16, mu, rstd);
                 }
             }
         }
@@ -400,6 +412,8 @@
 __global__ void __launch_bounds__(IG_THREADS, 1) igemm_kernel(const __grid_constant__ IgemmParams p) { igemm_body<BN, PAIR, SILU>(p); }
 template <int BN>
 __global__ void __launch_bounds__(IG_THREADS, 1) igemm_pad0_kernel(const __grid_constant__ IgemmParams p) { igemm_body<BN, false, false, true>(p); }
+template <int BN, bool PAIR>
+__global__ void __launch_bounds__(IG_THREADS, 1) igemm_up2_kernel(const __grid_constant__ IgemmParams p) { igemm_body<BN, PAIR, false, false, true>(p); }
 
 using IgemmFn = void (*)(IgemmParams);
 template <bool PAIR>
@@ -412,7 +426,16 @@
         default: return nullptr;
     }
 }
-static IgemmFn igemm_select(int bn, bool pair, bool silu, bool pad0 = false) {
+static IgemmFn igemm_select(int bn, bool pair, bool silu, bool pad0 = false, bool up2 = false) {
+    if (up2) {
+        if (silu || pad0) return nullptr;
+        switch (bn) {
+            case 64: return pair ? igemm_up2_kernel<64, true> : igemm_up2_kernel<64, false>;
+            case 128: return pair ? igemm_up2_kernel<128, true> : igemm_up2_kernel<128, false>;
+            case 160: return pair ? igemm_up2_kernel<160, true> : igemm_up2_kernel<160, false>;
+            default: return nullptr;
+        }
+    }
     if (pad0) {
         if (pair || silu) return nullptr;
         switch (bn) {
@@ -499,6 +522,10 @@
 
 static int plan_swap(const IgemmDesc& d, IgemmPlan* plan) {
     IgemmParams& p = plan->p;
+    if (d.epi.flags & IG_UP2) {
+        b2_set_error("igemm(swap): no swapped orientation for the sub-pixel upsampling convolution (IG_UP2)");
+        return -1;
+    }
     if ((d.epi.flags & (IG_GEGLU | IG_PAD0)) || d.nseg < 1 || d.nseg > IG_MAX_SRC || d.epi.rowstat_out || d.epi.colsum || d.epi.out2) {
         b2_set_error("igemm(swap): unsupported (GEGLU / tap origin 0 / LayerNorm fold / row statistics / transposed V / nseg %d)", d.nseg);
         return -1;
@@ -611,9 +638,9 @@
     return sms;
 }
 
-static int igemm_ctas_per_sm(int bn, bool pair, bool silu, bool pad0) {
+static int igemm_ctas_per_sm(int bn, bool pair, bool silu, bool pad0, bool up2) {
     if (g_plan_dry) return 1;
-    IgemmFn fn = igemm_select(bn, pair, silu, pad0);
+    IgemmFn fn = igemm_select(bn, pair, silu, pad0, up2);
     int n = 0;
     if (fn && cudaOccupancyMaxActiveBlocksPerMultiprocessor(&n, fn, IG_THREADS, 0) == cudaSuccess && n > 0) return n;
     cudaGetLastError();
@@ -629,10 +656,26 @@
         return -1;
     }
     const bool geglu = (d.epi.flags & IG_GEGLU) != 0;
-    const int n_gemm = geglu ? d.epi.n_valid * 2 : d.epi.n_valid;
+    const bool up2 = (d.epi.flags & IG_UP2) != 0;
+    if (up2) {
+        const char* bad = (d.epi.flags & IG_GEGLU) ? "GEGLU" : (d.epi.flags & IG_SILU) ? "SiLU" : (d.epi.flags & IG_PAD0) ? "tap origin 0"
+                        : d.epi.colsum || d.epi.rowstat_in ? "LayerNorm fold" : d.epi.rowstat_out ? "row statistics"
+                        : d.epi.out2 ? "transposed V" : d.epi.res ? "residual" : d.stride > 1 ? "stride 2"
+                        : (d.nseg != 1 || d.ntap[0] != 4) ? "a source other than one 4-tap segment" : nullptr;
+        if (bad) {
+            b2_set_error("igemm(IG_UP2): the sub-pixel upsampling convolution does not support %s", bad);
+            return -1;
+        }
+        if (d.epi.n_valid <= 0 || d.epi.n_valid % 16 != 0) {
+            b2_set_error("igemm(IG_UP2): output channels %d must be a positive multiple of 16", d.epi.n_valid);
+            return -1;
+        }
+    }
+    const int n_gemm = up2 ? d.epi.n_valid * 4 : (geglu ? d.epi.n_valid * 2 : d.epi.n_valid);
     int BN = d.BN;
     if (BN <= 0) {
-        if (n_gemm <= 256 && n_gemm % 16 == 0) BN = n_gemm;
+        if (up2) BN = d.epi.n_valid % 128 == 0 ? 128 : (d.epi.n_valid % 160 == 0 ? 160 : 64);
+        else if (n_gemm <= 256 && n_gemm % 16 == 0) BN = n_gemm;
         else if (n_gemm < 16) BN = 16;
         else if (n_gemm % 128 == 0) BN = 128;
         else if (n_gemm % 160 == 0) BN = 160;
@@ -650,6 +693,10 @@
     }
     if ((d.epi.flags & IG_PAD0) && !igemm_select(BN, pair, (d.epi.flags & IG_SILU) != 0, true)) {
         b2_set_error("igemm: no tap-origin-0 kernel for BN %d%s (64/128/256, single CTAs, no SiLU)", BN, pair ? " (CTA pair)" : "");
+        return -1;
+    }
+    if (up2 && (d.epi.n_valid % BN != 0 || !igemm_select(BN, pair, false, false, true))) {
+        b2_set_error("igemm(IG_UP2): BN %d must divide the output channels %d and be 64 / 128 / 160", BN, d.epi.n_valid);
         return -1;
     }
     if (pair && BN % 32 != 0) {
@@ -699,7 +746,7 @@
                          s, a.C, a.ld);
             return -1;
         }
-        if (d.ntap[s] != 1 && d.ntap[s] != 9) {
+        if (d.ntap[s] != 1 && d.ntap[s] != 9 && !(up2 && d.ntap[s] == 4)) {
             b2_set_error("igemm: ntap %d", d.ntap[s]);
             return -1;
         }
@@ -742,7 +789,7 @@
         p.epi.flags |= IG_SPLITK;
     }
     const size_t stage_bytes = (size_t)IG_BM * IG_BK * 2 + (size_t)BN * IG_BK * 2;
-    const int per_sm = igemm_ctas_per_sm(BN, pair, (d.epi.flags & IG_SILU) != 0, (d.epi.flags & IG_PAD0) != 0);
+    const int per_sm = igemm_ctas_per_sm(BN, pair, (d.epi.flags & IG_SILU) != 0, (d.epi.flags & IG_PAD0) != 0, up2);
     const long resident = (long)per_sm * b2_device_sms();
     static const char* pc_env = getenv("B2_PERSIST_CTAS");
     const long persist_ctas = pc_env ? atoi(pc_env) : resident;
@@ -803,8 +850,8 @@
     static bool attr_set = false;
     if (!attr_set) {
         for (int bn = 16; bn <= 256; bn += 16) {
-            for (int pair = 0; pair < 4; ++pair) {
-                IgemmFn fn = igemm_select(bn, pair == 1, pair == 2, pair == 3);
+            for (int pair = 0; pair < 6; ++pair) {
+                IgemmFn fn = igemm_select(bn, pair == 1 || pair == 5, pair == 2, pair == 3, pair >= 4);
                 if (!fn) continue;
                 cudaError_t e = cudaFuncSetAttribute(fn, cudaFuncAttributeMaxDynamicSharedMemorySize, 227 * 1024);
                 if (e != cudaSuccess) {
@@ -822,10 +869,12 @@
 int igemm_launch(const IgemmPlan& plan, cudaStream_t stream) {
     if (igemm_init()) return -1;
     const int cz = plan.splits > 1 ? plan.splits : 1;
-    IgemmFn fn = igemm_select(plan.p.BN, plan.pair, (plan.p.epi.flags & IG_SILU) != 0, (plan.p.epi.flags & IG_PAD0) != 0);
+    IgemmFn fn = igemm_select(plan.p.BN, plan.pair, (plan.p.epi.flags & IG_SILU) != 0, (plan.p.epi.flags & IG_PAD0) != 0,
+                              (plan.p.epi.flags & IG_UP2) != 0);
     if (!fn) {
-        b2_set_error("igemm launch: no kernel for BN %d%s%s%s", plan.p.BN, plan.pair ? " (CTA pair)" : "",
-                     (plan.p.epi.flags & IG_SILU) ? " with the SiLU epilogue" : "", (plan.p.epi.flags & IG_PAD0) ? " with tap origin 0" : "");
+        b2_set_error("igemm launch: no kernel for BN %d%s%s%s%s", plan.p.BN, plan.pair ? " (CTA pair)" : "",
+                     (plan.p.epi.flags & IG_SILU) ? " with the SiLU epilogue" : "", (plan.p.epi.flags & IG_PAD0) ? " with tap origin 0" : "",
+                     (plan.p.epi.flags & IG_UP2) ? " for sub-pixel upsampling" : "");
         return -1;
     }
     cudaError_t e = plan.pair ? launch_kc(fn, plan.grid, dim3(IG_THREADS), plan.smem, stream, 2, cz, plan.p)
diff --git a/ai-rtc-agent_b200/csrc/igemm.cuh b/ai-rtc-agent_b200/csrc/igemm.cuh
--- a/ai-rtc-agent_b200/csrc/igemm.cuh
+++ b/ai-rtc-agent_b200/csrc/igemm.cuh
@@ -20,6 +20,7 @@
     IG_SPLITK = 4,
     IG_SILU = 8,
     IG_PAD0 = 16,
+    IG_UP2 = 32,
 };
 
 struct IgEpilogue {
diff --git a/ai-rtc-agent_b200/host/capi.py b/ai-rtc-agent_b200/host/capi.py
--- a/ai-rtc-agent_b200/host/capi.py
+++ b/ai-rtc-agent_b200/host/capi.py
@@ -69,6 +69,7 @@
 IG_GEGLU = 2
 IG_SILU = 8
 IG_PAD0 = 16
+IG_UP2 = 32
 SC_IN_U8, SC_IN_TANH3, SC_OUT_RELU, SC_OUT_SILU, SC_IN_OFFSET = 1, 2, 4, 32, 64
 CONTROL_FRAME, CONTROL_HED = 0, 1
 VAE_TINY, VAE_KL = 0, 1
@@ -91,6 +92,8 @@
         _lib.b2sd_op_igemm.restype = C.c_int
         _lib.b2sd_igemm_plan_dry.argtypes = [C.POINTER(IgemmDesc), C.c_int, C.c_int, C.POINTER(IgemmPlanInfo)]
         _lib.b2sd_igemm_plan_dry.restype = C.c_int
+        _lib.b2sd_fold_up2_weights.argtypes = [C.c_void_p, C.c_int, C.c_int, C.c_void_p]
+        _lib.b2sd_fold_up2_weights.restype = C.c_int
         _lib.b2sd_groupnorm_plan_dry.argtypes = [C.c_int, C.c_int, C.c_int, C.c_int, C.POINTER(C.c_int), C.POINTER(C.c_int), C.POINTER(C.c_int)]
         _lib.b2sd_groupnorm_plan_dry.restype = C.c_int
         _lib.b2sd_igemm_partial_floats.argtypes = [C.c_int, C.c_int64, C.c_int]
diff --git a/ai-rtc-agent_b200/host/ops.py b/ai-rtc-agent_b200/host/ops.py
--- a/ai-rtc-agent_b200/host/ops.py
+++ b/ai-rtc-agent_b200/host/ops.py
@@ -14,6 +14,15 @@
 def pack_conv_weight(w_oihw: torch.Tensor) -> torch.Tensor:
     o, i, kh, kw = w_oihw.shape
     return w_oihw.permute(0, 2, 3, 1).reshape(o, kh * kw * i).contiguous().to(torch.float16)
+
+
+def fold_up2_weight(w_oihw: torch.Tensor) -> torch.Tensor:
+    o, i, kh, kw = w_oihw.shape
+    assert (kh, kw) == (3, 3)
+    w = w_oihw.detach().to("cpu", torch.float16).contiguous()
+    out = torch.empty(4 * o, 4 * i, dtype=torch.float16)
+    capi.check(capi.lib().b2sd_fold_up2_weights(w.data_ptr(), o, i, out.data_ptr()), "b2sd_fold_up2_weights")
+    return out
 
 
 def _view(t: torch.Tensor) -> capi.ActView:
@@ -29,13 +38,13 @@
           stride: int = 1, colbias: Optional[torch.Tensor] = None, res: Optional[torch.Tensor] = None,
           acc_scale: float = 1.0, res_scale: float = 1.0, relu: bool = False, geglu: bool = False, silu: bool = False,
           bn: int = 0, splits: int = 1, n_valid: Optional[int] = None, timeline: Optional[torch.Tensor] = None, swap: bool = False,
-          tconv: bool = False, pair: bool = False, pad0: bool = False,
+          tconv: bool = False, pair: bool = False, pad0: bool = False, up2: bool = False,
           rowstat_out: Optional[torch.Tensor] = None, rowstat_in: Optional[torch.Tensor] = None,
           colsum: Optional[torch.Tensor] = None, ln_c: int = 0, ln_eps: float = 1e-5,
           out2: Optional[torch.Tensor] = None, col2: int = 0) -> torch.Tensor:
     d = _igemm_desc(srcs, w, out, stride=stride, colbias=colbias, res=res, acc_scale=acc_scale, res_scale=res_scale, relu=relu,
                     geglu=geglu, silu=silu, bn=bn, splits=splits, n_valid=n_valid, timeline=timeline, swap=swap, tconv=tconv, pair=pair,
-                    pad0=pad0,
+                    pad0=pad0, up2=up2,
                     rowstat_out=rowstat_out, rowstat_in=rowstat_in, colsum=colsum, ln_c=ln_c, ln_eps=ln_eps, out2=out2, col2=col2)
     capi.check(capi.lib().b2sd_op_igemm(C.byref(d), capi.current_stream_ptr()), "b2sd_op_igemm")
     return out
@@ -49,7 +58,8 @@
 
 
 def _igemm_desc(srcs, w, out, *, stride=1, colbias=None, res=None, acc_scale=1.0, res_scale=1.0, relu=False, geglu=False,
-                silu=False, bn=0, splits=1, n_valid=None, timeline=None, swap=False, tconv=False, pair=False, pad0=False, rowstat_out=None,
+                silu=False, bn=0, splits=1, n_valid=None, timeline=None, swap=False, tconv=False, pair=False, pad0=False, up2=False,
+                rowstat_out=None,
                 rowstat_in=None, colsum=None, ln_c=0, ln_eps=1e-5, out2=None, col2=0) -> capi.IgemmDesc:
     d = capi.IgemmDesc()
     d.nseg = len(srcs)
@@ -77,7 +87,7 @@
         d.res, d.ldr = res.data_ptr(), res.stride(2)
     d.acc_scale, d.res_scale = acc_scale, res_scale
     d.flags = (capi.IG_RELU if relu else 0) | (capi.IG_GEGLU if geglu else 0) | (capi.IG_TCONV if tconv else 0) | (capi.IG_PAIR if pair else 0) \
-        | (capi.IG_SILU if silu else 0) | (capi.IG_PAD0 if pad0 else 0)
+        | (capi.IG_SILU if silu else 0) | (capi.IG_PAD0 if pad0 else 0) | (capi.IG_UP2 if up2 else 0)
     if rowstat_out is not None:
         assert rowstat_out.dtype == torch.int64 and rowstat_out.is_contiguous()
         d.rowstat_out = rowstat_out.data_ptr()
diff --git a/ai-rtc-agent_b200/host/stream.py b/ai-rtc-agent_b200/host/stream.py
--- a/ai-rtc-agent_b200/host/stream.py
+++ b/ai-rtc-agent_b200/host/stream.py
@@ -96,8 +96,6 @@
         self.image_processor = ImageProcessor(8)
         self.prompt_encoder = prompt_encoder
         self.text_encoder = prompt_encoder
-        self.unet = self
-        self.vae = self
         self._handle = C.c_void_p()
         self._prepared = False
         self._lib = capi.lib()
@@ -151,6 +149,14 @@
         capi.check(self._lib.b2sd_export_packed(self._handle, os.fsencode(tmp)), f"b2sd_export_packed({path})")
         os.replace(tmp, path)
 
+    @property
+    def unet(self) -> "StreamDiffusion":
+        return self
+
+    @property
+    def vae(self) -> "StreamDiffusion":
+        return self
+
     def __del__(self):
         try:
             if getattr(self, "_handle", None) and self._handle.value:
diff --git a/include/b200sd.h b/include/b200sd.h
--- a/include/b200sd.h
+++ b/include/b200sd.h
@@ -22,6 +22,7 @@
     B2SD_IG_GEGLU = 2,
     B2SD_IG_SILU = 8,
     B2SD_IG_PAD0 = 16,
+    B2SD_IG_UP2 = 32,
     B2SD_IG_TCONV = 64,
     B2SD_IG_PAIR = 128
 };
@@ -57,6 +58,7 @@
 } b2sd_igemm_desc;
 
 int b2sd_op_igemm(const b2sd_igemm_desc* d, void* stream);
+int b2sd_fold_up2_weights(const void* w_oihw, int cout, int cin, void* out);
 
 typedef struct {
     int mode;
```
